# roahmlab/armour

Hardware: AMD Instinct MI355X
Metric: planning iters/s (eval_g+jac) Kinova 7-DOF, 100 timesteps × 20 obstacles (higher is better)
Workload: dtype f64

## Files before the change

armour_amd/_lib.py:

```python
import ctypes as C
import os

_HERE = os.path.dirname(os.path.abspath(__file__))
KEY128 = os.environ.get("ARMOUR_KEY128", "0") not in ("", "0")
LIB_PATH = os.environ.get("ARMOUR_HIP_LIB") or os.path.join(_HERE, "lib", "libarmour_hip_k128.so" if KEY128 else "libarmour_hip.so")

MAXJ = 9
MAXF = 8 if KEY128 else 7

OK, EINVAL, EDEVICE, ECAPACITY, ESTATE = 0, -1, -2, -3, -4


class ArmourRobot(C.Structure):
    _fields_ = [
        ("num_joints", C.c_int32), ("num_factors", C.c_int32),
        ("axes", C.c_int32 * MAXJ), ("continuous", C.c_int32 * MAXF),
        ("trans", C.c_double * ((MAXJ + 1) * 3)), ("rots", C.c_double * (MAXJ * 3)),
        ("mass", C.c_double * MAXJ), ("mass_uncertainty", C.c_double),
        ("com", C.c_double * (MAXJ * 3)),
        ("inertia", C.c_double * (MAXJ * 9)), ("inertia_uncertainty", C.c_double),
        ("friction", C.c_double * MAXJ), ("damping", C.c_double * MAXJ), ("armature", C.c_double * MAXJ),
        ("state_limits_lb", C.c_double * MAXF), ("state_limits_ub", C.c_double * MAXF),
        ("speed_limits", C.c_double * MAXF), ("torque_limits", C.c_double * MAXF),
        ("gravity", C.c_double),
        ("link_zonotope_center", C.c_double * (MAXJ * 3)), ("link_zonotope_generators", C.c_double * (MAXJ * 3)),
        ("alpha", C.c_double), ("V_m", C.c_double), ("M_max", C.c_double), ("M_min", C.c_double), ("K", C.c_double),
        ("mass_uncertainty_link", C.c_double * MAXJ), ("inertia_uncertainty_link", C.c_double * MAXJ),
    ]


class ArmourParams(C.Structure):
    _fields_ = [
        ("num_time_steps", C.c_int32), ("input_constraints_off", C.c_int32),
        ("duration", C.c_double), ("k_range", C.c_double * MAXF),
        ("simplify_threshold", C.c_double), ("t_plan", C.c_double), ("cost_scale", C.c_double),
        ("collision_violation_threshold", C.c_double), ("torque_violation_threshold", C.c_double),
    ]


class ArmourLimits(C.Structure):
    _fields_ = [
        ("max_batch", C.c_int32), ("max_obstacles", C.c_int32), ("link_monomials", C.c_int32),
        ("torque_monomials", C.c_int32), ("work_monomials", C.c_int32), ("raw_terms", C.c_int32),
    ]


class ArmourSolveOptions(C.Structure):
    _fields_ = [("max_iterations", C.c_int32), ("max_line_search", C.c_int32), ("tolerance", C.c_double),
                ("max_wall_time_s", C.c_double), ("force_host_qp", C.c_double), ("reserved", C.c_double * 3)]


class ArmourSolveResult(C.Structure):
    _fields_ = [("k_opt", C.c_double * MAXF), ("cost", C.c_double), ("max_violation", C.c_double), ("feasible", C.c_int32),
                ("iterations", C.c_int32), ("evaluations", C.c_int32), ("status", C.c_int32), ("time_ms", C.c_double)]


class ArmourTrackOptions(C.Structure):
    _fields_ = [("controller", C.c_int32), ("record_every", C.c_int32), ("steps_per_launch", C.c_int32), ("reserved0", C.c_int32),
                ("Kr", C.c_double * MAXF), ("alpha", C.c_double), ("V_max", C.c_double), ("r_norm_threshold", C.c_double),
                ("model_uncertainty", C.c_double), ("dt", C.c_double), ("t0", C.c_double), ("t1", C.c_double), ("duration", C.c_double),
                ("reserved", C.c_double * 4)]


class ArmourTrackResult(C.Structure):
    _fields_ = [("status", C.c_int32), ("steps", C.c_int32), ("limit_flags", C.c_int32), ("reserved", C.c_int32),
                ("t_end", C.c_double), ("q", C.c_double * MAXF), ("qd", C.c_double * MAXF),
                ("max_pos_error", C.c_double), ("max_vel_error", C.c_double), ("max_V", C.c_double), ("max_robust_input", C.c_double),
                ("max_torque_ratio", C.c_double), ("first_violation_t", C.c_double)]


TRACK_CTL_ROBUST, TRACK_CTL_NOMINAL, TRACK_CTL_NONE = 0, 1, 2
TRACK_LIMIT_TORQUE, TRACK_LIMIT_POSITION, TRACK_LIMIT_SPEED = 1, 2, 4


class ArmourViolation(C.Structure):
    _fields_ = [("l1_violation", C.c_double), ("worst", C.c_double), ("worst_row", C.c_int32), ("n_violated", C.c_int32),
                ("n_outside_slack", C.c_int32), ("feasible", C.c_int32)]


OPT_P1_BUILD = 1
OPT_P1_WORK_MEMORY_MB = 2
OPT_P1_KEEP_WORK_MEMORY = 3
OPT_P1_STEP_WAVES = 101
OPT_P1_STEP_FREE = 102
OPT_P1_STEP_SPLIT_FK = 103
OPT_P1_STEP_AUX3 = 104
OPT_P1_MAX_WAVES_PER_CU = 105
OPT_P1_TWO_PASS = 106
OPT_P1_STEP_PAIRS = 107
OPT_P1_STEP_QUEUE = 109
OPT_P1_STEP_TAIL_CROSS = 108
OPT_P1_STEP_TWO_CU = 123
OPT_P1_STEP_LEAN_BACK = 124
OPT_P1_TV_TAIL_CROSS = 121
OPT_P1_TV_MIN_GROUPS = 110
OPT_P1_TV_WAVES = 111
OPT_P1_TV_FREE = 112
OPT_P1_TV_SPLIT_FK = 113
OPT_P1_TV_DEDICATED = 114
OPT_P1_TV_HELP_SHIFT = 115
OPT_P1_TV_HELPERS = 116
OPT_P1_TV_HELP_MIN = 117
OPT_P1_TV_HELP_N = 118
OPT_P1_TV_AUX3 = 119
OPT_P1_FULL_PLANES = 120
OPT_P1_TV_ROW_WIDTH = 122
OPT_P2_EX = 130
OPT_STEPS_GRAPH_MIN = 131
OPT_PINNED_MODE = 132
OPT_CULL_ROWS = 133
OPT_SOLVE_SUB_TILES = 140
OPT_SOLVE_DEVICE = 141
OPT_SOLVE_CUT_TILES = 142
OPT_SOLVE_BLOCKS = 143
OPT_SOLVE_SUB_BATCH = 144
OPT_SOLVE_ROW_CAP = 145
OPT_SOLVE_HARD_CAP_S = 146
OPT_SOLVE_WAVES_PER_SIMD = 147
OPT_SOLVE_CULL = 148

EXPORTS = [
    "armour_robot_kinova_gen3_no_gripper", "armour_robot_kinova_gen3_gripper", "armour_robot_fetch", "armour_robot_fetch8", "armour_params_default", "armour_create", "armour_destroy",
    "armour_last_error", "armour_device_available", "armour_alloc_pinned", "armour_free_pinned", "armour_set_problems", "armour_set_problems_armtd", "armour_get_sizes",
    "armour_get_bounds", "armour_eval_f", "armour_eval_grad_f", "armour_eval_g_jac",
    "armour_eval_g_jac_device", "armour_eval_g_jac_device_steps", "armour_prepare_steps", "armour_eval_g_jac_device_multi", "armour_desired_trajectory", "armour_robust_controller", "armour_check_feasible", "armour_get_torque_radius",
    "armour_get_link_generators", "armour_get_link_centers", "armour_get_pz", "armour_get_table_sizes",
    "armour_solve_options_default", "armour_solve", "armour_debug_qp", "armour_debug_qp_box", "armour_debug_pz_op",
    "armour_get_hyperplanes", "armour_get_build_ms", "armour_get_build_info", "armour_p2_kernel_name", "armour_debug_load_tables",
    "armour_get_plane_skip", "armour_get_prune_margin", "armour_batch_get_prune_margin", "armour_set_option", "armour_get_option", "armour_controller_set_kernel", "armour_device_memory", "armour_abi_max_factors", "armour_eval_violations_device", "armour_eval_violations", "armour_get_row_relevance", "armour_get_solver_rows",
    "armour_batch_partition", "armour_batch_create", "armour_batch_destroy", "armour_batch_set_option", "armour_batch_set_problems",
    "armour_batch_get_sizes", "armour_batch_get_bounds", "armour_batch_eval_g_jac", "armour_batch_eval_violations", "armour_batch_solve",
    "armour_batch_get_build_ms", "armour_batch_get_build_info",
    "armour_roadmap_create", "armour_roadmap_destroy", "armour_roadmap_get_sizes", "armour_roadmap_check", "armour_roadmap_plan",
    "armour_track_options_default", "armour_track", "armour_track_auto_steps",
    "armour_path_audit", "armour_path_audit_host", "armour_path_audit_items",
]

_lib = None


def _share_hip_runtime_with_torch():
    import importlib.util
    import sys
    if "torch" in sys.modules:
        return
    try:
        spec = importlib.util.find_spec("torch")
    except (ImportError, ValueError):
        spec = None
    if spec is None or not spec.origin:
        return
    cand = os.path.join(os.path.dirname(spec.origin), "lib", "libamdhip64.so")
    if os.path.exists(cand):
        try:
            C.CDLL(cand, mode=C.RTLD_GLOBAL)
        except OSError:
            pass


def load():
    global _lib
    if _lib is not None:
        return _lib
    if not os.path.exists(LIB_PATH):
        raise OSError(
            f"{LIB_PATH} not found: build it with `make -C armour_amd/csrc` (hipcc, gfx950) or "
            "`python -c 'import __graft_entry__ as g; g.build()'`. There is no CPU path.")
    _share_hip_runtime_with_torch()
    L = C.CDLL(LIB_PATH)
    if hasattr(L, "armour_abi_max_factors") and L.armour_abi_max_factors() != MAXF:
        raise RuntimeError(f"{LIB_PATH} is built for {L.armour_abi_max_factors()} factors, this process mirrors its structs for {MAXF} (ARMOUR_KEY128)")
    dp, ip = C.POINTER(C.c_double), C.POINTER(C.c_int32)
    vp = C.c_void_p
    L.armour_robot_kinova_gen3_no_gripper.argtypes = [C.POINTER(ArmourRobot)]
    L.armour_robot_kinova_gen3_no_gripper.restype = None
    L.armour_robot_kinova_gen3_gripper.argtypes = [C.POINTER(ArmourRobot)]
    L.armour_robot_fetch.argtypes = [C.POINTER(ArmourRobot)]
    L.armour_robot_fetch.restype = None
    L.armour_robot_fetch8.argtypes = [C.POINTER(ArmourRobot)]
    L.armour_robot_fetch8.restype = C.c_int
    L.armour_robot_kinova_gen3_gripper.restype = None
    L.armour_params_default.argtypes = [C.POINTER(ArmourParams), C.c_int32]
    L.armour_params_default.restype = None
    L.armour_create.argtypes = [C.POINTER(ArmourRobot), C.POINTER(ArmourParams), C.POINTER(ArmourLimits), C.c_int32, C.POINTER(vp)]
    L.armour_destroy.argtypes = [vp]
    L.armour_destroy.restype = None
    L.armour_last_error.restype = C.c_char_p
    L.armour_alloc_pinned.argtypes = [C.c_uint64, C.POINTER(vp)]
    L.armour_free_pinned.argtypes = [vp]
    L.armour_free_pinned.restype = None
    L.armour_set_problems.argtypes = [vp, C.c_int32, C.c_int32, dp, dp, dp, dp, dp]
    L.armour_set_problems_armtd.argtypes = [vp, C.c_int32, C.c_int32, dp, dp, dp, dp, dp, dp]
    L.armour_get_sizes.argtypes = [vp, ip, ip, ip]
    L.armour_get_bounds.argtypes = [vp, dp, dp, dp, dp]
    L.armour_eval_f.argtypes = [vp, dp, dp]
    L.armour_eval_grad_f.argtypes = [vp, dp, dp]
    L.armour_eval_g_jac.argtypes = [vp, dp, dp, dp]
    L.armour_eval_g_jac_device.argtypes = [vp, vp, vp, vp, vp]
    L.armour_eval_g_jac_device_steps.argtypes = [vp, vp, C.c_int32, vp, vp, vp]
    L.armour_prepare_steps.argtypes = [vp, vp, C.c_int32, vp, vp]
    L.armour_eval_g_jac_device_multi.argtypes = [vp, vp, C.c_int32, vp, vp, vp]
    L.armour_desired_trajectory.argtypes = [C.c_int32, dp, dp, dp, dp, C.c_double, dp, C.c_double, dp, dp, dp]
    L.armour_robust_controller.argtypes = [C.POINTER(ArmourRobot), C.c_double, dp, C.c_double, C.c_double, C.c_double, C.c_int32, dp, dp, dp, dp, dp, dp, dp, dp]
    L.armour_check_feasible.argtypes = [vp, dp, ip]
    L.armour_solve_options_default.argtypes = [C.POINTER(ArmourSolveOptions)]
    L.armour_solve_options_default.restype = None
    L.armour_solve.argtypes = [vp, C.POINTER(ArmourSolveOptions), C.POINTER(ArmourSolveResult)]
    L.armour_debug_qp.argtypes = [C.c_int32, dp, dp, C.c_int32, dp, dp, dp, dp, ip]
    L.armour_debug_qp_box.argtypes = [C.c_int32, dp, dp, C.c_int32, dp, dp, dp, dp, dp, C.c_int32, dp, ip, ip, dp]
    L.armour_debug_pz_op.argtypes = [vp, C.c_int32, C.c_int32, ip, ip, C.POINTER(C.POINTER(C.c_uint64)), C.POINTER(dp), dp, dp, dp, dp,
                                     C.c_int32, C.c_int32, C.POINTER(C.c_uint64), dp, dp]
    L.armour_get_torque_radius.argtypes = [vp, dp]
    L.armour_get_link_generators.argtypes = [vp, dp]
    L.armour_get_link_centers.argtypes = [vp, dp, dp]
    L.armour_get_pz.argtypes = [vp, C.c_int32, C.c_int32, C.c_int32, C.c_int32, dp, C.POINTER(C.c_uint64), dp, C.c_int32]
    L.armour_get_table_sizes.argtypes = [vp, C.POINTER(C.c_int64)]
    L.armour_get_hyperplanes.argtypes = [vp, dp, dp, dp]
    L.armour_get_build_ms.argtypes = [vp, dp]
    L.armour_get_build_info.argtypes = [vp, ip]
    L.armour_p2_kernel_name.restype = C.c_char_p
    L.armour_debug_load_tables.argtypes = [vp, C.c_int32, C.c_int32, dp, dp, dp, dp, ip, dp, C.POINTER(C.c_uint64), dp,
                                           C.c_int32, ip, dp, C.POINTER(C.c_uint64), dp, C.c_int32, dp, dp, dp, dp]
    L.armour_get_plane_skip.argtypes = [vp, C.POINTER(C.c_uint64)]
    L.armour_get_prune_margin.argtypes = [vp, dp]
    L.armour_batch_get_prune_margin.argtypes = [vp, dp]
    L.armour_set_option.argtypes = [vp, C.c_int32, C.c_double]
    L.armour_get_option.argtypes = [vp, C.c_int32, dp]
    L.armour_device_memory.argtypes = [C.c_int32, C.POINTER(C.c_uint64), C.POINTER(C.c_uint64)]
    L.armour_controller_set_kernel.argtypes = [C.c_int32]
    L.armour_eval_violations_device.argtypes = [vp, vp, vp, vp]
    L.armour_eval_violations.argtypes = [vp, dp, C.POINTER(ArmourViolation)]
    L.armour_get_row_relevance.argtypes = [vp, C.POINTER(C.c_uint8), C.POINTER(C.c_int32), C.POINTER(C.c_double)]
    L.armour_get_solver_rows.argtypes = [vp, C.POINTER(C.c_uint8), C.POINTER(C.c_int32), C.POINTER(C.c_int32), C.POINTER(C.c_double)]
    L.armour_batch_partition.argtypes = [C.c_int32, C.c_int32, ip]
    L.armour_batch_create.argtypes = [C.POINTER(ArmourRobot), C.POINTER(ArmourParams), C.POINTER(ArmourLimits), ip, C.c_int32, C.POINTER(vp)]
    L.armour_batch_destroy.argtypes = [vp]
    L.armour_batch_destroy.restype = None
    L.armour_batch_set_option.argtypes = [vp, C.c_int32, C.c_double]
    L.armour_batch_set_problems.argtypes = [vp, C.c_int32, C.c_int32, dp, dp, dp, dp, dp]
    L.armour_batch_get_sizes.argtypes = [vp, ip, ip, ip, ip]
    L.armour_batch_get_bounds.argtypes = [vp, dp, dp, dp, dp]
    L.armour_batch_eval_g_jac.argtypes = [vp, dp, dp, dp]
    L.armour_batch_eval_violations.argtypes = [vp, dp, C.POINTER(ArmourViolation)]
    L.armour_batch_solve.argtypes = [vp, C.POINTER(ArmourSolveOptions), C.POINTER(ArmourSolveResult)]
    L.armour_batch_get_build_ms.argtypes = [vp, dp, dp]
    L.armour_batch_get_build_info.argtypes = [vp, ip]
    u8p = C.POINTER(C.c_uint8)
    L.armour_roadmap_create.argtypes = [C.POINTER(ArmourRobot), C.c_int32, dp, C.c_int32, ip, u8p, C.c_double, C.c_int32, C.POINTER(vp)]
    L.armour_roadmap_destroy.argtypes = [vp]
    L.armour_roadmap_destroy.restype = None
    L.armour_roadmap_get_sizes.argtypes = [vp, ip, ip, C.POINTER(C.c_int64)]
    L.armour_roadmap_check.argtypes = [vp, C.c_int32, C.c_int32, dp, u8p, u8p, dp, dp]
    L.armour_roadmap_plan.argtypes = [vp, C.c_int32, dp, dp, C.c_int32, C.c_int32, dp, ip]
    L.armour_track_options_default.argtypes = [C.POINTER(ArmourRobot), C.POINTER(ArmourTrackOptions)]
    L.armour_track_options_default.restype = None
    L.armour_track.argtypes = [C.POINTER(ArmourRobot), C.POINTER(ArmourTrackOptions), C.c_int32, dp, dp, dp, dp, dp, dp, dp, dp,
                               C.POINTER(ArmourTrackResult), dp, dp]
    L.armour_track_auto_steps.argtypes = [C.c_int32]
    audit = [C.POINTER(ArmourRobot), C.c_int32, C.c_int32, dp, C.c_int32, ip, dp, dp, dp, dp, dp, C.c_double, dp, dp, dp, C.c_double, ip, dp, dp]
    L.armour_path_audit.argtypes = audit + [dp]
    L.armour_path_audit_host.argtypes = audit
    L.armour_path_audit_items.argtypes = [C.POINTER(ArmourRobot), C.c_int32, dp, dp, dp, dp, dp, C.c_double, dp, dp, C.c_double, C.POINTER(C.c_int64)]
    _lib = L
    return L


class ArmourError(RuntimeError):
    def __init__(self, code, msg):
        super().__init__(f"armour error {code}: {msg}")
        self.code = code


def check(rc):
    if rc < 0:
        raise ArmourError(rc, load().armour_last_error().decode())
    return rc
```

armour_amd/csrc/api.hip:

```cpp
#include <algorithm>
#include <cmath>
#include <cstdarg>
#include <chrono>
#include <cstring>
#include <mutex>
#include <new>

#include "../../include/armour_robot_fetch.h"
#include "../../include/armour_robot_kinova.h"
#include "bezier.h"
#include "cacc.h"
#include "common.h"
#include "solver_common.h"

static thread_local char g_err[512] = "";

void armour_set_error(const char* fmt, ...) {
    va_list ap;
    va_start(ap, fmt);
    vsnprintf(g_err, sizeof(g_err), fmt, ap);
    va_end(ap);
}

extern "C" const char* armour_last_error(void) { return g_err; }

extern "C" void armour_robot_kinova_gen3_no_gripper(ArmourRobot* robot) { armour_fill_kinova_gen3_no_gripper(robot); }
extern "C" void armour_robot_kinova_gen3_gripper(ArmourRobot* robot) { armour_fill_kinova_gen3_gripper(robot); }
extern "C" void armour_robot_fetch(ArmourRobot* robot) { armour_fill_fetch(robot); }
extern "C" int armour_robot_fetch8(ArmourRobot* robot) {
#if ARMOUR_MAX_FACTORS >= 8
    if (!robot) { armour_set_error("null argument"); return ARMOUR_EINVAL; }
    armour_fill_fetch8(robot);
    return ARMOUR_OK;
#else
    (void)robot;
    armour_set_error("armour_robot_fetch8: an 8-factor robot needs the 128-bit-key library (libarmour_hip_k128.so: armour_abi_max_factors() == 8)");
    return ARMOUR_EINVAL;
#endif
}
extern "C" void armour_params_default(ArmourParams* params, int32_t T) { armour_fill_default_params(params, T); }

extern "C" int armour_device_available(void) {
    int n = 0;
    if (hipGetDeviceCount(&n) != hipSuccess) return 0;
    return n > 0 ? 1 : 0;
}

namespace {
struct PinnedRange { const char* p; size_t bytes; };
std::mutex g_pinned_mu;
std::vector<PinnedRange> g_pinned;
bool in_pinned(const void* q, size_t bytes) {
    if (!q) return true;
    const char* c = static_cast<const char*>(q);
    std::lock_guard<std::mutex> lk(g_pinned_mu);
    for (const PinnedRange& r : g_pinned)
        if (c >= r.p && c + bytes <= r.p + r.bytes) return true;
    return false;
}
}

extern "C" int armour_alloc_pinned(uint64_t bytes, void** out) {
    if (!out) { armour_set_error("null argument"); return ARMOUR_EINVAL; }
    HIPCHK(hipHostMalloc(out, bytes ? bytes : 1, hipHostMallocDefault));
    std::lock_guard<std::mutex> lk(g_pinned_mu);
    g_pinned.push_back({static_cast<const char*>(*out), (size_t)(bytes ? bytes : 1)});
    return ARMOUR_OK;
}
extern "C" void armour_free_pinned(void* p) {
    if (!p) return;
    {
        std::lock_guard<std::mutex> lk(g_pinned_mu);
        for (size_t i = 0; i < g_pinned.size(); i++)
            if (g_pinned[i].p == p) { g_pinned.erase(g_pinned.begin() + i); break; }
    }
    (void)hipHostFree(p);
}

template <class Tp>
static int dev_alloc(Tp** p, size_t count) {
    if (*p) { (void)hipFree(*p); *p = nullptr; }
    if (count == 0) count = 1;
    HIPCHK(hipMalloc((void**)p, count * sizeof(Tp)));
    return ARMOUR_OK;
}
template <class Tp>
static void dev_free(Tp** p) {
    if (*p) { (void)hipFree(*p); *p = nullptr; }
}

static int ensure_capacity(ArmourPlanner* h, int B, int O) {
    if (B <= h->allocB && O <= h->allocO) return ARMOUR_OK;
    const int nb = B > h->allocB ? B : h->allocB, no = O > h->allocO ? O : h->allocO;
    h->allocB = 0; h->allocO = 0;
    const size_t nl = (size_t)nb * h->J * h->T, nt = (size_t)nb * h->n * h->T;
    int rc;
#define TRY(x) if ((rc = (x)) != ARMOUR_OK) return rc
    TRY(dev_alloc(&h->d_link_count, nl));
    TRY(dev_alloc(&h->d_link_center, nl * 3));
    TRY(dev_alloc(&h->d_link_indep, nl * 3));
    TRY(dev_alloc(&h->d_link_keys, nl * h->lim.link_monomials));
    TRY(dev_alloc(&h->d_link_coeff, nl * h->lim.link_monomials * 3));
    TRY(dev_alloc(&h->d_tq_count, nt));
    TRY(dev_alloc(&h->d_tq_center, nt));
    TRY(dev_alloc(&h->d_tq_indep, nt));
    TRY(dev_alloc(&h->d_tq_keys, nt * h->lim.torque_monomials));
    TRY(dev_alloc(&h->d_tq_coeff, nt * h->lim.torque_monomials));
    TRY(dev_alloc(&h->d_planes, (size_t)nb * armour_planes_per_problem(h->J * h->T * no)));
    TRY(dev_alloc(&h->d_planes_ll, (size_t)nb * armour_planes_ll_per_problem(h->J * h->T)));
    TRY(dev_alloc(&h->d_obs_center, (size_t)nb * 3 * (no > 0 ? no : 1)));
    TRY(dev_alloc(&h->d_plane_skip, (size_t)nb));
    TRY(dev_alloc(&h->d_bez, (size_t)nb * 3 * h->n));
    const size_t mmax = (size_t)h->n * h->T + (size_t)h->J * h->T * no + 4 * h->n;
    TRY(dev_alloc(&h->d_k, (size_t)nb * h->n));
    TRY(dev_alloc(&h->d_g, (size_t)nb * mmax + std::max((size_t)nb * mmax * h->n, (size_t)nb * h->T * h->J * 3)));
    h->d_jac = h->d_g + (size_t)nb * mmax;
    TRY(dev_alloc(&h->d_bounds, (size_t)2 * nb * mmax));
#undef TRY
    h->allocB = nb;
    h->allocO = no;
    return ARMOUR_OK;
}

P2Tables armour_make_tables(const ArmourPlanner* h) {
    P2Tables tb;
    memset(&tb, 0, sizeof(tb));
    tb.B = h->B; tb.T = h->T; tb.J = h->J; tb.n = h->n; tb.O = h->O; tb.Q = h->Q; tb.m = h->m;
    tb.capL = h->lim.link_monomials; tb.capT = h->lim.torque_monomials;
    tb.row0 = h->row0; tb.mode = h->mode;
    tb.link_count = h->d_link_count; tb.link_center = h->d_link_center; tb.link_indep = h->d_link_indep;
    tb.link_keys = h->d_link_keys; tb.link_coeff = h->d_link_coeff;
    tb.tq_count = h->d_tq_count; tb.tq_center = h->d_tq_center; tb.tq_indep = h->d_tq_indep;
    tb.tq_keys = h->d_tq_keys; tb.tq_coeff = h->d_tq_coeff;
    tb.planes = h->d_planes; tb.planes_ll = h->d_planes_ll; tb.ll_shared = h->ll_shared;
    tb.ex_allowed = h->tune(ARMOUR_OPT_P2_EX);
    tb.obs_center = (h->d_from_center && (h->B >= 8 || !h->planes_have_d)) ? h->d_obs_center : nullptr;
    tb.plane_skip = h->d_plane_skip; tb.bez = h->d_bez;
    for (int i = 0; i < ARMOUR_MAX_FACTORS; i++) tb.k_range[i] = h->params.k_range[i];
    tb.duration = h->params.duration;
    return tb;
}

namespace {
struct TuningSpec { int option; double def, lo, hi; };
const TuningSpec kTuning[] = {
    {ARMOUR_OPT_P1_STEP_WAVES, 0, 0, 4}, {ARMOUR_OPT_P1_STEP_FREE, 1, 0, 1}, {ARMOUR_OPT_P1_STEP_SPLIT_FK, -1, -1, 1}, {ARMOUR_OPT_P1_STEP_AUX3, 1, 0, 1},
    {ARMOUR_OPT_P1_MAX_WAVES_PER_CU, 4, 1, 8}, {ARMOUR_OPT_P1_TWO_PASS, 1, 0, 1}, {ARMOUR_OPT_P1_STEP_PAIRS, 1, 0, 2}, {ARMOUR_OPT_P1_STEP_QUEUE, 1, 0, 3}, {ARMOUR_OPT_P1_STEP_TAIL_CROSS, 0, 0, 514}, {ARMOUR_OPT_P1_STEP_TWO_CU, 3, 0, 33}, {ARMOUR_OPT_P1_STEP_LEAN_BACK, 1, 0, 3}, {ARMOUR_OPT_P1_TV_TAIL_CROSS, 111, 0, 514} ,
    {ARMOUR_OPT_P1_TV_MIN_GROUPS, 31, 1, 1e6}, {ARMOUR_OPT_P1_TV_WAVES, 0, 0, 8}, {ARMOUR_OPT_P1_TV_FREE, 1, 0, 1}, {ARMOUR_OPT_P1_TV_SPLIT_FK, -1, -1, 1},
    {ARMOUR_OPT_P1_TV_DEDICATED, 1, 0, 1}, {ARMOUR_OPT_P1_TV_HELP_SHIFT, 0, 0, 3}, {ARMOUR_OPT_P1_TV_HELPERS, 1, 0, 31}, {ARMOUR_OPT_P1_TV_HELP_MIN, 192, 1, 1e6},
    {ARMOUR_OPT_P1_TV_HELP_N, 1, 0, 1}, {ARMOUR_OPT_P1_TV_AUX3, 1, 0, 1}, {ARMOUR_OPT_P1_TV_ROW_WIDTH, 0, 0, 64}, {ARMOUR_OPT_P1_FULL_PLANES, 0, 0, 1},
    {ARMOUR_OPT_P2_EX, 1, 0, 1}, {ARMOUR_OPT_STEPS_GRAPH_MIN, 2, 0, 1e6}, {ARMOUR_OPT_PINNED_MODE, 0, 0, 2}, {ARMOUR_OPT_CULL_ROWS, 0, 0, 1},
    {ARMOUR_OPT_SOLVE_SUB_TILES, 48, 1, 1e6}, {ARMOUR_OPT_SOLVE_DEVICE, 1, 0, 2}, {ARMOUR_OPT_SOLVE_CUT_TILES, 156, 1, 1e6}, {ARMOUR_OPT_SOLVE_BLOCKS, 0, 0, 1e6},
    {ARMOUR_OPT_SOLVE_SUB_BATCH, 0, 0, 1e6}, {ARMOUR_OPT_SOLVE_ROW_CAP, 0, 0, 1e7}, {ARMOUR_OPT_SOLVE_HARD_CAP_S, 0, 0, 1e6}, {ARMOUR_OPT_SOLVE_WAVES_PER_SIMD, 0, 0, 2}, {ARMOUR_OPT_SOLVE_CULL, -1, -1, 1},
};
const TuningSpec* tuning_spec(int option) {
    for (const TuningSpec& t : kTuning) if (t.option == option) return &t;
    return nullptr;
}
}
void armour_tuning_defaults(double* tuning) {
    for (int o = ARMOUR_OPT_FIRST_TUNING; o <= ARMOUR_OPT_LAST_TUNING; o++) tuning[o - ARMOUR_OPT_FIRST_TUNING] = 0.0;
    for (const TuningSpec& t : kTuning) tuning[t.option - ARMOUR_OPT_FIRST_TUNING] = t.def;
}
bool armour_trace_p1() { static const bool on = getenv("ARMOUR_P1_TRACE") != nullptr; return on; }
BuildStamps& armour_build_stamps() { static thread_local BuildStamps s; return s; }
void armour_build_stamp(const char* name) {
    if (!armour_trace_p1()) return;
    BuildStamps& s = armour_build_stamps();
    if (s.n < 12) { s.t[s.n] = std::chrono::duration<double, std::micro>(std::chrono::steady_clock::now().time_since_epoch()).count(); s.name[s.n] = name; s.n++; }
}
static void armour_build_stamps_print(const char* what) {
    if (!armour_trace_p1()) return;
    BuildStamps& s = armour_build_stamps();
    fprintf(stderr, "[%s, host side, us]", what);
    for (int i = 1; i < s.n; i++) fprintf(stderr, " %s %.1f", s.name[i], s.t[i] - s.t[i - 1]);
    if (s.n > 1) fprintf(stderr, " | total %.1f\n", s.t[s.n - 1] - s.t[0]);
}
bool armour_trace_solve() { static const bool on = getenv("ARMOUR_SOLVE_TIMING") != nullptr; return on; }

extern "C" int armour_create(const ArmourRobot* robot, const ArmourParams* params, const ArmourLimits* limits,
                             int32_t device, ArmourPlanner** out) {
    if (!robot || !params || !out) { armour_set_error("armour_create: null argument"); return ARMOUR_EINVAL; }
    if (robot->num_joints < 1 || robot->num_joints > ARMOUR_MAX_JOINTS || robot->num_factors < 1 ||
        robot->num_factors > robot->num_joints || robot->num_factors > ARMOUR_MAX_FACTORS) {
        armour_set_error("armour_create: unsupported robot (joints=%d, factors=%d; max %d joints, %d factors -- the monomial key "
                         "packs 9 bits per factor into 64, RT/PZsparse.h:8-21)", robot->num_joints, robot->num_factors,
                         ARMOUR_MAX_JOINTS, ARMOUR_MAX_FACTORS);
        return ARMOUR_EINVAL;
    }
    for (int i = 0; i < robot->num_joints; i++)
        if ((i < robot->num_factors) != (robot->axes[i] != 0)) {
            armour_set_error("armour_create: the actuated joints must come first and the fixed ones last (RT/Dynamics.cu:103-105)");
            return ARMOUR_EINVAL;
        }
    if (params->num_time_steps < 2 || (params->num_time_steps & 1)) {
        armour_set_error("armour_create: num_time_steps must be even and >= 2 (RT/Parameters.h:16)");
        return ARMOUR_EINVAL;
    }
    int ndev = 0;
    if (hipGetDeviceCount(&ndev) != hipSuccess || ndev <= 0) {
        armour_set_error("armour_create: no HIP device visible -- libarmour_hip has no CPU path");
        return ARMOUR_EDEVICE;
    }
    if (device < 0 || device >= ndev) { armour_set_error("armour_create: device %d out of range (%d visible)", device, ndev); return ARMOUR_EINVAL; }
    HIPCHK(hipSetDevice(device));
    ArmourPlanner* h = new (std::nothrow) ArmourPlanner();
    if (!h) { armour_set_error("out of host memory"); return ARMOUR_EINVAL; }
    h->robot = *robot;
    h->params = *params;
    armour_tuning_defaults(h->tuning);
    ArmourLimits lim;
    memset(&lim, 0, sizeof(lim));
    if (limits) lim = *limits;
    if (lim.max_batch <= 0) lim.max_batch = 1;
    if (lim.max_obstacles <= 0) lim.max_obstacles = 40;
    if (lim.link_monomials <= 0) lim.link_monomials = 32;
    if (lim.torque_monomials <= 0) lim.torque_monomials = 128;
    if (lim.work_monomials <= 0) lim.work_monomials = 1024;
    if (lim.raw_terms <= 0) lim.raw_terms = 4096;
    h->lim = lim;
    h->ub = armour_ultimate_bound(robot);
    h->device = device;
    h->T = params->num_time_steps; h->J = robot->num_joints; h->n = robot->num_factors;
    hipError_t e = hipStreamCreateWithFlags(&h->stream, hipStreamNonBlocking);
    if (e != hipSuccess) { armour_set_error("hipStreamCreate failed: %s", hipGetErrorString(e)); delete h; return ARMOUR_EDEVICE; }
    *out = h;
    return ARMOUR_OK;
}

double* armour_handle_pinned(ArmourPlanner* h, int slot, size_t bytes) {
    if (h->solve_pin[slot] && h->solve_pin_bytes[slot] >= bytes) return static_cast<double*>(h->solve_pin[slot]);
    if (h->solve_pin[slot]) { armour_free_pinned(h->solve_pin[slot]); h->solve_pin[slot] = nullptr; h->solve_pin_bytes[slot] = 0; }
    void* p = nullptr;
    if (armour_alloc_pinned(bytes, &p) != ARMOUR_OK) return nullptr;
    h->solve_pin[slot] = p; h->solve_pin_bytes[slot] = bytes;
    return static_cast<double*>(p);
}

static void drop_step_graphs(ArmourPlanner* h) {
    for (auto& g : h->step_graphs) (void)hipGraphExecDestroy(g.exec);
    h->step_graphs.clear();
}

extern "C" void armour_destroy(ArmourPlanner* h) {
    if (!h) return;
    (void)hipSetDevice(h->device);
    if (h->stream) (void)hipStreamSynchronize(h->stream);
    drop_step_graphs(h);
    for (void* pin : h->solve_pin) armour_free_pinned(pin);
    dev_free(&h->d_bounds); dev_free(&h->d_viol);
    armour_relevance_free(h);
    if (h->d_tr_stage) (void)hipFree(h->d_tr_stage);
    dev_free(&h->solve_dev.ctl); dev_free(&h->solve_dev.blk_word); dev_free(&h->solve_dev.blk_rows); dev_free(&h->solve_dev.qp_rows);
    dev_free(&h->solve_dev.flags);
    dev_free(&h->d_jrs);
    armour_p1_free(h);
    dev_free(&h->d_link_count); dev_free(&h->d_link_center); dev_free(&h->d_link_indep);
    dev_free(&h->d_link_keys); dev_free(&h->d_link_coeff);
    dev_free(&h->d_tq_count); dev_free(&h->d_tq_center); dev_free(&h->d_tq_indep);
    dev_free(&h->d_tq_keys); dev_free(&h->d_tq_coeff);
    dev_free(&h->d_planes); dev_free(&h->d_planes_ll); dev_free(&h->d_obs_center); dev_free(&h->d_plane_skip); dev_free(&h->d_bez);
    dev_free(&h->d_k); dev_free(&h->d_g); h->d_jac = nullptr;
    if (h->stream) (void)hipStreamDestroy(h->stream);
    delete h;
}

static int begin_problem_set(ArmourPlanner* h, int B, int O, const double* q0, const double* qd0, const double* qdd0,
                             const double* q_des, int mode = ARMOUR_MODE_ARMOUR) {
    if (!h || !q0 || !qd0 || !qdd0 || !q_des) { armour_set_error("null argument"); return ARMOUR_EINVAL; }
    if (B < 1 || O < 0) { armour_set_error("bad batch/obstacle count (B=%d, O=%d)", B, O); return ARMOUR_EINVAL; }
    {
        const double* arrs[4] = {q0, qd0, qdd0, q_des};
        for (int a = 0; a < 4; a++)
            for (size_t i = 0; i < (size_t)B * h->n; i++)
                if (!std::isfinite(arrs[a][i])) { armour_set_error("non-finite entry in the initial state / goal arrays (array %d, entry %zu)", a, i); return ARMOUR_EINVAL; }
    }
    HIPCHK(hipSetDevice(h->device));
    h->ready = false;
    h->rel_fresh = false; h->rel2_fresh = false;
    h->bounds_on_device = false; h->bounds_on_host = false;
    h->tables_from_host = false;
    h->stats_fresh = false;
    drop_step_graphs(h);
    int rc = ensure_capacity(h, B, O);
    if (rc != ARMOUR_OK) return rc;
    h->B = B; h->O = O; h->Q = h->J * h->T * O;
    h->mode = mode;
    h->row0 = h->no_torque() ? 0 : h->n * h->T;
    h->m = h->row0 + h->Q + 4 * h->n;
    h->d_jac = h->d_g + (size_t)B * h->m;
    const size_t bn = (size_t)B * h->n;
    h->h_q0.assign(q0, q0 + bn); h->h_qd0.assign(qd0, qd0 + bn);
    h->h_qdes.assign(q_des, q_des + bn);
    if (mode == ARMOUR_MODE_ARMTD) { h->h_qdd0.assign(bn, 0.0); h->h_krange.assign(qdd0, qdd0 + bn); }
    else { h->h_qdd0.assign(qdd0, qdd0 + bn); h->h_krange.clear(); }
    std::vector<double> bz((size_t)B * 3 * h->n);
    const double D = mode == ARMOUR_MODE_ARMTD ? 1.0 : h->params.duration;
    for (int b = 0; b < B; b++)
        for (int i = 0; i < h->n; i++) {
            bz[((size_t)b * 3 + 0) * h->n + i] = q0[b * h->n + i];
            bz[((size_t)b * 3 + 1) * h->n + i] = qd0[b * h->n + i] * D;
            bz[((size_t)b * 3 + 2) * h->n + i] = qdd0[b * h->n + i] * D * D;
        }
    HIPCHK(hipMemcpy(h->d_bez, bz.data(), bz.size() * sizeof(double), hipMemcpyHostToDevice));
    return ARMOUR_OK;
}

int armour_refresh_table_stats(ArmourPlanner* h) {
    if (h->stats_fresh) { h->stats_fresh = false; return ARMOUR_OK; }
    const size_t nl = (size_t)h->B * h->J * h->T, nt = (size_t)h->B * h->n * h->T;
    std::vector<int> lc(nl), tc(nt);
    HIPCHK(hipMemcpy(lc.data(), h->d_link_count, nl * sizeof(int), hipMemcpyDeviceToHost));
    HIPCHK(hipMemcpy(tc.data(), h->d_tq_count, nt * sizeof(int), hipMemcpyDeviceToHost));
    long long sl = 0, st = 0;
    int ml = 0, mt = 0;
    for (int v : lc) { sl += v; if (v > ml) ml = v; }
    for (int v : tc) { st += v; if (v > mt) mt = v; }
    h->sum_link = sl; h->sum_torque = st; h->max_link = ml; h->max_torque = mt;
    h->h_plane_skip.assign((size_t)h->B, 0ull);
    if (h->O > 0) HIPCHK(hipMemcpy(h->h_plane_skip.data(), h->d_plane_skip, (size_t)h->B * sizeof(unsigned long long), hipMemcpyDeviceToHost));
    if (h->O > 0 && armour_trace_p1()) {
        unsigned long long all_and = ~0ull, all_or = 0ull;
        for (unsigned long long v : h->h_plane_skip) { all_and &= v; all_or |= v; }
        fprintf(stderr, "[P1 planes] plane_skip of %d problem(s): AND 0x%09llx OR 0x%09llx\n", h->B, all_and & ((1ull << ARMOUR_NPLANES) - 1ull), all_or & ((1ull << ARMOUR_NPLANES) - 1ull));
    }
    return ARMOUR_OK;
}

extern "C" int armour_set_problems(ArmourPlanner* h, int32_t B, int32_t O, const double* q0, const double* qd0,
                                   const double* qdd0, const double* q_des, const double* obstacles) {
    armour_build_stamps().n = 0;
    armour_build_stamp("start");
    int rc = begin_problem_set(h, B, O, q0, qd0, qdd0, q_des);
    if (rc != ARMOUR_OK) return rc;
    if (O > 0 && !obstacles) { armour_set_error("obstacles is null but O=%d", O); return ARMOUR_EINVAL; }
    for (size_t i = 0; i < (size_t)B * O * 12; i++)
        if (!std::isfinite(obstacles[i])) { armour_set_error("non-finite obstacle entry %zu", i); return ARMOUR_EINVAL; }
    armour_build_stamp("checks+bezier-upload");
    rc = armour_p1_build(h, obstacles);
    if (rc != ARMOUR_OK) return rc;
    armour_build_stamp("copy-out");
    rc = armour_refresh_table_stats(h);
    if (rc != ARMOUR_OK) return rc;
    h->ready = true;
    armour_build_stamp("table-stats");
    armour_build_stamps_print("armour_set_problems");
    return ARMOUR_OK;
}

extern "C" int armour_set_problems_armtd(ArmourPlanner* h, int32_t B, int32_t O, const double* q0, const double* qd0, const double* q_des,
                                         const double* jrs, const double* k_range, const double* obstacles) {
    if (!jrs || !k_range) { armour_set_error("null argument"); return ARMOUR_EINVAL; }
    int rc = begin_problem_set(h, B, O, q0, qd0, k_range, q_des, ARMOUR_MODE_ARMTD);
    if (rc != ARMOUR_OK) return rc;
    if (O > 0 && !obstacles) { armour_set_error("obstacles is null but O=%d", O); return ARMOUR_EINVAL; }
    for (size_t i = 0; i < (size_t)B * O * 12; i++)
        if (!std::isfinite(obstacles[i])) { armour_set_error("non-finite obstacle entry %zu", i); return ARMOUR_EINVAL; }
    for (size_t i = 0; i < (size_t)B * h->n * 6 * h->T; i++)
        if (!std::isfinite(jrs[i])) { armour_set_error("non-finite entry %zu in the offline JRS tables", i); return ARMOUR_EINVAL; }
    const size_t cnt = (size_t)B * h->n * 6 * h->T;
    if (cnt > h->jrs_cap) {
        if ((rc = dev_alloc(&h->d_jrs, cnt)) != ARMOUR_OK) return rc;
        h->jrs_cap = cnt;
    }
    HIPCHK(hipMemcpy(h->d_jrs, jrs, cnt * sizeof(double), hipMemcpyHostToDevice));
    rc = armour_p1_build(h, obstacles);
    if (rc != ARMOUR_OK) return rc;
    rc = armour_refresh_table_stats(h);
    if (rc != ARMOUR_OK) return rc;
    h->ready = true;
    return ARMOUR_OK;
}

extern "C" int armour_debug_load_tables(ArmourPlanner* h, int32_t B, int32_t O, const double* q0, const double* qd0,
                                        const double* qdd0, const double* q_des, const int32_t* link_count,
                                        const double* link_center, const uint64_t* link_keys, const double* link_coeffs,
                                        int32_t cap_l, const int32_t* torque_count, const double* torque_center,
                                        const uint64_t* torque_keys, const double* torque_coeffs, int32_t cap_t,
                                        const double* A, const double* d, const double* delta, const double* torque_radius) {
    int rc = begin_problem_set(h, B, O, q0, qd0, qdd0, q_des);
    if (rc != ARMOUR_OK) return rc;
    h->build_ms = 0; h->build_info[0] = h->build_info[1] = h->build_info[2] = h->build_info[3] = 0;
    h->h_prune_margin.clear();
    const int J = h->J, T = h->T, n = h->n, capL = h->lim.link_monomials, capT = h->lim.torque_monomials;
    const size_t nl = (size_t)B * J * T, nt = (size_t)B * n * T;
    std::vector<double> lc(nl * 3), li(nl * 3), lco(nl * capL * 3, 0.0), tc(nt), ti(nt), tco(nt * capT, 0.0);
    std::vector<uint32_t> lk(nl * capL, 0), tk(nt * capT, 0);
    for (size_t i = 0; i < nl; i++) {
        if (link_count[i] > capL) { armour_set_error("link PZ %zu has %d monomials > capacity %d", i, link_count[i], capL); return ARMOUR_ECAPACITY; }
        for (int e = 0; e < 3; e++) { lc[i * 3 + e] = link_center[(i * 2) * 3 + e]; li[i * 3 + e] = link_center[(i * 2 + 1) * 3 + e]; }
        for (int mo = 0; mo < link_count[i]; mo++) {
            lk[i * capL + mo] = (uint32_t)link_keys[i * cap_l + mo];
            for (int e = 0; e < 3; e++) lco[(i * capL + mo) * 3 + e] = link_coeffs[(i * cap_l + mo) * 3 + e];
        }
    }
    for (size_t i = 0; i < nt; i++) {
        if (torque_count[i] > capT) { armour_set_error("torque PZ %zu has %d monomials > capacity %d", i, torque_count[i], capT); return ARMOUR_ECAPACITY; }
        tc[i] = torque_center[i * 2]; ti[i] = torque_center[i * 2 + 1];
        for (int mo = 0; mo < torque_count[i]; mo++) { tk[i * capT + mo] = (uint32_t)torque_keys[i * cap_t + mo]; tco[i * capT + mo] = torque_coeffs[i * cap_t + mo]; }
    }
    const size_t ppp = armour_planes_per_problem(h->Q);
    std::vector<double> pl((size_t)B * ppp, 0.0);
    for (int b = 0; b < B; b++)
        for (int t = 0; t < T; t++)
            for (int l = 0; l < J; l++)
                for (int o = 0; o < O; o++)
                    for (int p = 0; p < 36; p++) {
                        const size_t src = ((((size_t)b * T + t) * J + l) * O + o) * 36 + p;
                        const int q = (l * T + t) * O + o;
                        double* base = &pl[(size_t)b * ppp];
                        base[armour_plane_index(h->Q, q, p, 0)] = A[src * 3 + 0]; base[armour_plane_index(h->Q, q, p, 1)] = A[src * 3 + 1];
                        base[armour_plane_index(h->Q, q, p, 2)] = A[src * 3 + 2];
                        base[armour_plane_index(h->Q, q, p, 3)] = d[src]; base[armour_plane_index(h->Q, q, p, 4)] = delta[src];
                    }
#define UP(dst, vec) HIPCHK(hipMemcpy(dst, vec.data(), vec.size() * sizeof(vec[0]), hipMemcpyHostToDevice))
    HIPCHK(hipMemcpy(h->d_link_count, link_count, nl * sizeof(int), hipMemcpyHostToDevice));
    HIPCHK(hipMemcpy(h->d_tq_count, torque_count, nt * sizeof(int), hipMemcpyHostToDevice));
    UP(h->d_link_center, lc); UP(h->d_link_indep, li); UP(h->d_link_keys, lk); UP(h->d_link_coeff, lco);
    UP(h->d_tq_center, tc); UP(h->d_tq_indep, ti); UP(h->d_tq_keys, tk); UP(h->d_tq_coeff, tco);
    if (!pl.empty()) UP(h->d_planes, pl);
    {
        const int JT = J * T;
        std::vector<double> pll((size_t)B * armour_planes_ll_per_problem(JT), 0.0);
        bool shared = O > 0;
        for (int b = 0; b < B && O > 0; b++)
            for (int t = 0; t < T; t++)
                for (int l = 0; l < J; l++)
                    for (int p = ARMOUR_FIRST_LL_PLANE; p < 36; p++)
                        for (int o = 0; o < O; o++) {
                            const size_t src = ((((size_t)b * T + t) * J + l) * O + o) * 36 + p, src0 = ((((size_t)b * T + t) * J + l) * O) * 36 + p;
                            for (int cc = 0; cc < 3; cc++) {
                                if (o == 0) pll[(size_t)b * armour_planes_ll_per_problem(JT) + armour_plane_ll_index(JT, l * T + t, p - ARMOUR_FIRST_LL_PLANE, cc)] = A[src * 3 + cc];
                                else if (memcmp(&A[src * 3 + cc], &A[src0 * 3 + cc], sizeof(double)) != 0) shared = false;
                            }
                        }
        UP(h->d_planes_ll, pll);
        h->ll_shared = shared ? 1 : 0;
        h->d_from_center = 0;
        h->planes_lean = 0; h->planes_have_d = 1;
    }
    HIPCHK(hipMemset(h->d_plane_skip, 0, (size_t)B * sizeof(unsigned long long)));
#undef UP
    h->h_torque_radius.assign(torque_radius, torque_radius + (size_t)B * n * T);
    h->h_link_gens.assign((size_t)B * T * J * 18, 0.0);
    rc = armour_refresh_table_stats(h);
    if (rc != ARMOUR_OK) return rc;
    h->tables_from_host = true;
    h->ready = true;
    return ARMOUR_OK;
}

#define NEED_READY(h)                                                                        \
    if (!(h)) { armour_set_error("null handle"); return ARMOUR_EINVAL; }                     \
    if (!(h)->ready) { armour_set_error("no problem set: call armour_set_problems first"); return ARMOUR_ESTATE; }

extern "C" int armour_get_sizes(const ArmourPlanner* h, int32_t* B, int32_t* n, int32_t* m) {
    NEED_READY(h);
    if (B) *B = h->B;
    if (n) *n = h->n;
    if (m) *m = h->m;
    return ARMOUR_OK;
}

extern "C" int armour_get_bounds(ArmourPlanner* h, double* x_l, double* x_u, double* g_l, double* g_u) {
    NEED_READY(h);
    const int T = h->T, n = h->n;
    if (x_l) for (int i = 0; i < n; i++) x_l[i] = -1.0;
    if (x_u) for (int i = 0; i < n; i++) x_u[i] = 1.0;
    if (!g_l || !g_u) return ARMOUR_OK;
    for (int b = 0; b < h->B; b++) {
        double* gl = g_l + (size_t)b * h->m;
        double* gu = g_u + (size_t)b * h->m;
        if (!h->no_torque()) {
            const double* tr = &h->h_torque_radius[(size_t)b * n * T];
            for (int t = 0; t < T; t++)
                for (int j = 0; j < n; j++) {
                    gl[t * n + j] = -h->robot.torque_limits[j] + tr[j * T + t];
                    gu[t * n + j] = h->robot.torque_limits[j] - tr[j * T + t];
                }
        }
        size_t off = (size_t)h->row0;
        for (size_t i = off; i < off + (size_t)h->Q; i++) { gl[i] = -1e19; gu[i] = 0; }
        off += h->Q;
        for (int rep = 0; rep < 2; rep++, off += n)
            for (int i = 0; i < n; i++) { gl[off + i] = h->robot.state_limits_lb[i] + h->ub.qe; gu[off + i] = h->robot.state_limits_ub[i] - h->ub.qe; }
        for (int rep = 0; rep < 2; rep++, off += n)
            for (int i = 0; i < n; i++) { gl[off + i] = -h->robot.speed_limits[i] + h->ub.qde; gu[off + i] = h->robot.speed_limits[i] - h->ub.qde; }
    }
    return ARMOUR_OK;
}

int armour_checked_collision_rows(const ArmourPlanner* h) {
    return h->mode == ARMOUR_MODE_ARMTD ? (h->n - 1 < h->J ? h->n - 1 : h->J) * h->T * h->O : h->Q;
}

static void plan_coeffs(const ArmourPlanner* h, size_t ix, double c[3]) {
    const double D = h->params.duration;
    const bool armtd = h->mode == ARMOUR_MODE_ARMTD;
    c[0] = h->h_q0[ix];
    c[1] = armtd ? h->h_qd0[ix] : h->h_qd0[ix] * D;
    c[2] = armtd ? h->h_krange[ix] : h->h_qdd0[ix] * D * D;
}

extern "C" int armour_eval_f(ArmourPlanner* h, const double* k, double* f) {
    NEED_READY(h);
    const int n = h->n;
    for (int b = 0; b < h->B; b++) {
        double obj = 0;
        for (int pass = 0; pass < 2; pass++)
            for (int i = 0; i < n; i++) {
                if ((h->robot.continuous[i] != 0) != (pass == 0)) continue;
                const size_t ix = (size_t)b * n + i;
                double c[3];
                plan_coeffs(h, ix, c);
                const double qp = slv::plan_point(h->mode, c[0], c[1], c[2], h->params.k_range[i], k[ix], h->params.t_plan);
                const double e = h->robot.continuous[i] ? slv::wrap_to_pi(h->h_qdes[ix] - qp) : (h->h_qdes[ix] - qp);
                obj += e * e;
            }
        f[b] = obj * h->params.cost_scale;
    }
    return ARMOUR_OK;
}

extern "C" int armour_eval_grad_f(ArmourPlanner* h, const double* k, double* grad_f) {
    NEED_READY(h);
    const int n = h->n;
    const double tp = h->params.t_plan;
    for (int b = 0; b < h->B; b++)
        for (int i = 0; i < n; i++) {
            const size_t ix = (size_t)b * n + i;
            double c[3];
            plan_coeffs(h, ix, c);
            const double qp = slv::plan_point(h->mode, c[0], c[1], c[2], h->params.k_range[i], k[ix], tp);
            const double dk = slv::plan_dk(h->mode, c[2], h->params.k_range[i], tp);
            const double e = h->robot.continuous[i] ? slv::wrap_to_pi(qp - h->h_qdes[ix]) : (qp - h->h_qdes[ix]);
            grad_f[ix] = 2 * e * dk * h->params.cost_scale;
        }
    return ARMOUR_OK;
}

extern "C" int armour_desired_trajectory(int32_t n, const double* q0, const double* qd0, const double* qdd0, const double* k_range,
                                         double duration, const double* k, double t, double* q, double* qd, double* qdd) {
    if (n < 1 || !q0 || !qd0 || !qdd0 || !k_range || !k || !(duration > 0)) { armour_set_error("bad argument"); return ARMOUR_EINVAL; }
    const double D = duration, s = t / D;
    for (int i = 0; i < n; i++) {
        const double a = qd0[i] * D, b = qdd0[i] * D * D, ka = k_range[i] * k[i];
        if (q) q[i] = bez::q_des(q0[i], a, b, ka, s);
        if (qd) qd[i] = bez::qd_des(q0[i], a, b, ka, s) / D;
        if (qdd) qdd[i] = bez::qdd_des(q0[i], a, b, ka, s) / (D * D);
    }
    return ARMOUR_OK;
}

extern "C" int armour_eval_g_jac_device(ArmourPlanner* h, const double* d_k, double* d_g, double* d_jac, void* stream) {
    NEED_READY(h);
    if (!d_k) { armour_set_error("d_k is null"); return ARMOUR_EINVAL; }
    const P2Tables tb = armour_make_tables(h);
    return armour_p2_launch(tb, h->max_link, h->max_torque, h->h_plane_skip.data(), d_k, d_g, d_jac, stream ? (hipStream_t)stream : h->stream);
}

static int enqueue_steps(ArmourPlanner* h, const double* d_k, int steps, double* d_g, double* d_jac, hipStream_t st) {
    const P2Tables tb = armour_make_tables(h);
    const size_t stride = (size_t)h->B * h->n;
    for (int s = 0; s < steps; s++) {
        int rc = armour_p2_launch(tb, h->max_link, h->max_torque, h->h_plane_skip.data(), d_k + (size_t)s * stride, d_g, d_jac, st);
        if (rc != ARMOUR_OK) return rc;
    }
    return ARMOUR_OK;
}

static int steps_graph(ArmourPlanner* h, const double* d_k, int steps, double* d_g, double* d_jac, hipGraphExec_t* out) {
    h->graph_clock++;
    for (auto& g : h->step_graphs)
        if (g.d_k == d_k && g.steps == steps && g.d_g == d_g && g.d_jac == d_jac) { g.last_use = h->graph_clock; *out = g.exec; return ARMOUR_OK; }
    HIPCHK(hipSetDevice(h->device));
    HIPCHK(hipStreamSynchronize(h->stream));
    hipGraph_t graph = nullptr;
    HIPCHK(hipStreamBeginCapture(h->stream, hipStreamCaptureModeThreadLocal));
    const int rc = enqueue_steps(h, d_k, steps, d_g, d_jac, h->stream);
    const hipError_t e = hipStreamEndCapture(h->stream, &graph);
    if (rc != ARMOUR_OK) { if (graph) (void)hipGraphDestroy(graph); return rc; }
    if (e != hipSuccess) { armour_set_error("hipStreamEndCapture failed: %s", hipGetErrorString(e)); return ARMOUR_EDEVICE; }
    hipGraphExec_t exec = nullptr;
    const hipError_t ei = hipGraphInstantiate(&exec, graph, nullptr, nullptr, 0);
    (void)hipGraphDestroy(graph);
    if (ei != hipSuccess) { armour_set_error("hipGraphInstantiate failed: %s", hipGetErrorString(ei)); return ARMOUR_EDEVICE; }
    if (h->step_graphs.size() >= 4) {
        size_t lru = 0;
        for (size_t i = 1; i < h->step_graphs.size(); i++) if (h->step_graphs[i].last_use < h->step_graphs[lru].last_use) lru = i;
        (void)hipGraphExecDestroy(h->step_graphs[lru].exec);
        h->step_graphs.erase(h->step_graphs.begin() + lru);
    }
    h->step_graphs.push_back({d_k, steps, d_g, d_jac, exec, h->graph_clock});
    *out = exec;
    return ARMOUR_OK;
}

static bool steps_use_graph(const ArmourPlanner* h, int steps) {
    const int min_steps = h->tune(ARMOUR_OPT_STEPS_GRAPH_MIN);
    return min_steps > 0 && steps >= min_steps;
}

extern "C" int armour_prepare_steps(ArmourPlanner* h, const double* d_k, int32_t steps, double* d_g, double* d_jac) {
    NEED_READY(h);
    if (!d_k || steps < 0) { armour_set_error("bad argument"); return ARMOUR_EINVAL; }
    if (!steps_use_graph(h, steps)) return ARMOUR_OK;
    hipGraphExec_t exec;
    return steps_graph(h, d_k, steps, d_g, d_jac, &exec);
}

extern "C" int armour_eval_g_jac_device_steps(ArmourPlanner* h, const double* d_k, int32_t steps, double* d_g, double* d_jac,
                                              void* stream) {
    NEED_READY(h);
    if (!d_k || steps < 0) { armour_set_error("bad argument"); return ARMOUR_EINVAL; }
    if (steps == 0 || (!d_g && !d_jac)) return ARMOUR_OK;
    const hipStream_t st = stream ? (hipStream_t)stream : h->stream;
    if (steps_use_graph(h, steps))
        for (auto& g : h->step_graphs)
            if (g.d_k == d_k && g.steps == steps && g.d_g == d_g && g.d_jac == d_jac) {
                g.last_use = ++h->graph_clock;
                HIPCHK(hipGraphLaunch(g.exec, st));
                return ARMOUR_OK;
            }
    return enqueue_steps(h, d_k, steps, d_g, d_jac, st);
}

extern "C" int armour_eval_g_jac_device_multi(ArmourPlanner* h, const double* d_k, int32_t points, double* d_g, double* d_jac,
                                              void* stream) {
    NEED_READY(h);
    if (!d_k || points < 0) { armour_set_error("bad argument"); return ARMOUR_EINVAL; }
    if (points == 0) return ARMOUR_OK;
    const P2Tables tb = armour_make_tables(h);
    const long long bn = (long long)h->B * h->n, bm = (long long)h->B * h->m;
    return armour_p2_launch(tb, h->max_link, h->max_torque, h->h_plane_skip.data(), d_k, d_g, d_jac, stream ? (hipStream_t)stream : h->stream,
                            points, bn, bm, bm * h->n);
}

int armour_spin_on_stream(hipStream_t st) {
    for (;;) {
        const hipError_t q = hipStreamQuery(st);
        if (q == hipSuccess) return ARMOUR_OK;
        if (q != hipErrorNotReady) { armour_set_error("hipStreamQuery failed: %s", hipGetErrorString(q)); return ARMOUR_EDEVICE; }
    }
}

extern "C" int armour_eval_g_jac(ArmourPlanner* h, const double* k, double* g, double* jac) {
    NEED_READY(h);
    if (!k) { armour_set_error("k is null"); return ARMOUR_EINVAL; }
    HIPCHK(hipSetDevice(h->device));
    const size_t bn = (size_t)h->B * h->n, bm = (size_t)h->B * h->m;
    const P2Tables tb = armour_make_tables(h);
    const int pinned_mode = h->tune(ARMOUR_OPT_PINNED_MODE);
    const bool all_pinned = in_pinned(k, bn * sizeof(double)) && in_pinned(g, bm * sizeof(double)) && in_pinned(jac, bm * h->n * sizeof(double));
    if (all_pinned && pinned_mode == 1) {
        int rc = armour_p2_launch(tb, h->max_link, h->max_torque, h->h_plane_skip.data(), k, g, jac, h->stream);
        if (rc != ARMOUR_OK) return rc;
        return armour_spin_on_stream(h->stream);
    }
    const double* k_dev = h->d_k;
    if (all_pinned && pinned_mode == 2) k_dev = k;
    else HIPCHK(hipMemcpyAsync(h->d_k, k, bn * sizeof(double), hipMemcpyHostToDevice, h->stream));
    int rc = armour_p2_launch(tb, h->max_link, h->max_torque, h->h_plane_skip.data(), k_dev, g ? h->d_g : nullptr, jac ? h->d_jac : nullptr, h->stream);
    if (rc != ARMOUR_OK) return rc;
    if (g && jac && jac == g + bm) {
        HIPCHK(hipMemcpyAsync(g, h->d_g, bm * (1 + (size_t)h->n) * sizeof(double), hipMemcpyDeviceToHost, h->stream));
        return armour_spin_on_stream(h->stream);
    }
    if (g) HIPCHK(hipMemcpyAsync(g, h->d_g, bm * sizeof(double), hipMemcpyDeviceToHost, h->stream));
    if (jac) HIPCHK(hipMemcpyAsync(jac, h->d_jac, bm * h->n * sizeof(double), hipMemcpyDeviceToHost, h->stream));
    return armour_spin_on_stream(h->stream);
}

extern "C" int armour_check_feasible(ArmourPlanner* h, const double* g, int32_t* feasible) {
    NEED_READY(h);
    const int T = h->T, n = h->n;
    const double tt = h->params.torque_violation_threshold, ct = h->params.collision_violation_threshold;
    for (int b = 0; b < h->B; b++) {
        const double* gb = g + (size_t)b * h->m;
        bool ok = true;
        if (!h->no_torque()) {
            const double* tr = &h->h_torque_radius[(size_t)b * n * T];
            for (int t = 0; t < T && ok; t++)
                for (int j = 0; j < n; j++) {
                    const double v = gb[t * n + j];
                    if (v < -h->robot.torque_limits[j] + tr[j * T + t] - tt || v > h->robot.torque_limits[j] - tr[j * T + t] + tt) { ok = false; break; }
                }
        }
        size_t off = (size_t)h->row0;
        const size_t n_checked = (size_t)armour_checked_collision_rows(h);
        for (size_t i = 0; i < n_checked && ok; i++)
            if (gb[off + i] > ct) ok = false;
        off += h->Q;
        for (int rep = 0; rep < 2 && ok; rep++, off += n)
            for (int i = 0; i < n; i++)
                if (gb[off + i] < h->robot.state_limits_lb[i] + h->ub.qe || gb[off + i] > h->robot.state_limits_ub[i] - h->ub.qe) { ok = false; break; }
        for (int rep = 0; rep < 2 && ok; rep++, off += n)
            for (int i = 0; i < n; i++)
                if (gb[off + i] < -h->robot.speed_limits[i] + h->ub.qde || gb[off + i] > h->robot.speed_limits[i] - h->ub.qde) { ok = false; break; }
        feasible[b] = ok ? 1 : 0;
    }
    return ARMOUR_OK;
}

namespace {
struct BoundsArgs {
    int n, T, m, row0, Q, no_torque;
    double torque_limits[ARMOUR_MAX_FACTORS], lb[ARMOUR_MAX_FACTORS], ub[ARMOUR_MAX_FACTORS], speed[ARMOUR_MAX_FACTORS];
    double qe, qde;
    const double* tr;
    double* lo; double* hi;
};
__global__ __launch_bounds__(256) void armour_bounds_kernel(BoundsArgs a) {
    const int b = blockIdx.y, r = blockIdx.x * 256 + threadIdx.x;
    if (r >= a.m) return;
    double l, u;
    if (r < a.row0) {
        const int t = r / a.n, j = r - t * a.n;
        const double tr = a.tr[((size_t)b * a.n + j) * a.T + t];
        l = -a.torque_limits[j] + tr; u = a.torque_limits[j] - tr;
    } else if (r < a.row0 + a.Q) { l = -1e19; u = 0; }
    else {
        const int e = r - a.row0 - a.Q, rep = e / a.n, i = e - rep * a.n;
        if (rep < 2) { l = a.lb[i] + a.qe; u = a.ub[i] - a.qe; }
        else { l = -a.speed[i] + a.qde; u = a.speed[i] - a.qde; }
    }
    a.lo[(size_t)b * a.m + r] = l;
    a.hi[(size_t)b * a.m + r] = u;
}
}

int armour_bounds_launch(ArmourPlanner* h, const double* d_tr) {
    const size_t bm = (size_t)h->B * h->m;
    BoundsArgs a;
    a.n = h->n; a.T = h->T; a.m = h->m; a.row0 = h->row0; a.Q = h->Q; a.no_torque = h->no_torque() ? 1 : 0;
    for (int j = 0; j < ARMOUR_MAX_FACTORS; j++) {
        a.torque_limits[j] = h->robot.torque_limits[j]; a.lb[j] = h->robot.state_limits_lb[j]; a.ub[j] = h->robot.state_limits_ub[j]; a.speed[j] = h->robot.speed_limits[j];
    }
    a.qe = h->ub.qe; a.qde = h->ub.qde;
    a.lo = h->d_bounds; a.hi = h->d_bounds + bm;
    a.tr = d_tr;
    hipLaunchKernelGGL(armour_bounds_kernel, dim3((h->m + 255) / 256, h->B), dim3(256), 0, h->stream, a);
    HIPCHK(hipGetLastError());
    h->bounds_on_device = true;
    return ARMOUR_OK;
}

int armour_upload_bounds(ArmourPlanner* h) {
    if (h->bounds_on_device) return ARMOUR_OK;
    const double* d_tr = nullptr;
    if (!h->no_torque()) {
        const size_t ntr = (size_t)h->B * h->n * h->T;
        if (h->tr_stage_cap < ntr) {
            if (h->d_tr_stage) (void)hipFree(h->d_tr_stage);
            h->d_tr_stage = nullptr; h->tr_stage_cap = 0;
            HIPCHK(hipMalloc((void**)&h->d_tr_stage, ntr * sizeof(double)));
            h->tr_stage_cap = ntr;
        }
        HIPCHK(hipMemcpyAsync(h->d_tr_stage, h->h_torque_radius.data(), ntr * sizeof(double), hipMemcpyHostToDevice, h->stream));
        d_tr = h->d_tr_stage;
    }
    const int rc = armour_bounds_launch(h, d_tr);
    if (rc != ARMOUR_OK) return rc;
    HIPCHK(hipStreamSynchronize(h->stream));
    return ARMOUR_OK;
}

extern "C" int armour_set_option(ArmourPlanner* h, int32_t option, double value) {
    if (!h) { armour_set_error("null handle"); return ARMOUR_EINVAL; }
    if (option == ARMOUR_OPT_P1_BUILD && (value == 0.0 || value == 1.0 || value == 2.0)) { h->opt_p1_build = (int)value; return ARMOUR_OK; }
    if (option == ARMOUR_OPT_P1_WORK_MEMORY_MB && value >= 0.0 && value <= 1e9) { h->opt_p1_work_mb = value; return ARMOUR_OK; }
    if (option == ARMOUR_OPT_P1_KEEP_WORK_MEMORY && (value == 0.0 || value == 1.0)) { h->opt_p1_keep_work = (int)value; return ARMOUR_OK; }
    if (const TuningSpec* t = tuning_spec(option)) {
        bool ok = value >= t->lo && value <= t->hi && (option == ARMOUR_OPT_SOLVE_HARD_CAP_S || value == (double)(long long)value);
        if (ok && (option == ARMOUR_OPT_P1_STEP_TAIL_CROSS || option == ARMOUR_OPT_P1_TV_TAIL_CROSS)) {
            const int v = (int)value, lo2 = v % 100, hi2 = v / 100;
            ok = (lo2 <= 4 || (lo2 >= 10 && lo2 <= 14)) && hi2 <= 5;
        }
        if (ok && option == ARMOUR_OPT_P1_TV_ROW_WIDTH) ok = value == 0.0 || value == 50.0 || value == 64.0;
        if (ok && option == ARMOUR_OPT_P1_STEP_TWO_CU) { const int lv = (int)value % 10; ok = lv <= 3 && (value < 10.0 || lv >= 1); if (ok) h->p1_two_cu_off = false; }
        if (ok) {
            h->tuning[option - ARMOUR_OPT_FIRST_TUNING] = value;
            h->p1_step_cap_hint = 0; h->p1_tv_shape_hint = 0;
            return ARMOUR_OK;
        }
    }
    armour_set_error("armour_set_option: unknown option %d or bad value %g", option, value);
    return ARMOUR_EINVAL;
}

extern "C" int armour_abi_max_factors(void) { return ARMOUR_MAX_FACTORS; }

extern "C" int armour_device_memory(int32_t device, uint64_t* free_bytes, uint64_t* total_bytes) {
    int ndev = 0;
    if (hipGetDeviceCount(&ndev) != hipSuccess || device < 0 || device >= ndev) { (void)hipGetLastError(); armour_set_error("armour_device_memory: no such device %d", device); return ARMOUR_EDEVICE; }
    HIPCHK(hipSetDevice(device));
    size_t f = 0, t = 0;
    HIPCHK(hipMemGetInfo(&f, &t));
    if (free_bytes) *free_bytes = f;
    if (total_bytes) *total_bytes = t;
    return ARMOUR_OK;
}

extern "C" int armour_get_option(ArmourPlanner* h, int32_t option, double* value) {
    if (!h || !value) { armour_set_error("null argument"); return ARMOUR_EINVAL; }
    if (option == ARMOUR_OPT_P1_BUILD) { *value = h->opt_p1_build; return ARMOUR_OK; }
    if (option == ARMOUR_OPT_P1_WORK_MEMORY_MB) { *value = h->opt_p1_work_mb; return ARMOUR_OK; }
    if (option == ARMOUR_OPT_P1_KEEP_WORK_MEMORY) { *value = h->opt_p1_keep_work; return ARMOUR_OK; }
    if (tuning_spec(option)) { *value = h->tuning[option - ARMOUR_OPT_FIRST_TUNING]; return ARMOUR_OK; }
    armour_set_error("armour_get_option: unknown option %d", option);
    return ARMOUR_EINVAL;
}

namespace {
struct ViolArgs {
    int m, row0, Q, n_checked;
    double torque_slack, collision_slack;
    const double* g; const double* lo; const double* hi;
    ArmourViolation* out;
};
__global__ __launch_bounds__(256) void armour_violation_kernel(ViolArgs a) {
    __shared__ double s_l1[256], s_w[256];
    __shared__ int s_row[256], s_nv[256], s_no[256];
    const int b = blockIdx.x, tid = threadIdx.x;
    const double* g = a.g + (size_t)b * a.m;
    const double* lo = a.lo + (size_t)b * a.m;
    const double* hi = a.hi + (size_t)b * a.m;
    double l1 = 0.0, worst = 0.0;
    int wrow = -1, nv = 0, no = 0;
    for (int r = tid; r < a.m; r += 256) {
        const double v = g[r], l = lo[r], u = hi[r];
        const double viol = fmax(0.0, fmax(l - v, v - u));
        l1 += viol;
        if (viol > 0.0) nv++;
        if (viol > worst) { worst = viol; wrow = r; }
        bool outside;
        if (r < a.row0) outside = v < l - a.torque_slack || v > u + a.torque_slack;
        else if (r < a.row0 + a.Q) outside = (r - a.row0) < a.n_checked && v > a.collision_slack;
        else outside = v < l || v > u;
        if (outside) no++;
    }
    s_l1[tid] = l1; s_w[tid] = worst; s_row[tid] = wrow; s_nv[tid] = nv; s_no[tid] = no;
    __syncthreads();
    for (int s = 128; s > 0; s >>= 1) {
        if (tid < s) {
            s_l1[tid] += s_l1[tid + s]; s_nv[tid] += s_nv[tid + s]; s_no[tid] += s_no[tid + s];
            const double ow = s_w[tid + s];
            const int orow = s_row[tid + s];
            if (ow > s_w[tid] || (ow == s_w[tid] && orow >= 0 && (s_row[tid] < 0 || orow < s_row[tid]))) { s_w[tid] = ow; s_row[tid] = orow; }
        }
        __syncthreads();
    }
    if (tid == 0) {
        ArmourViolation o;
        o.l1_violation = s_l1[0]; o.worst = s_w[0]; o.worst_row = s_row[0]; o.n_violated = s_nv[0]; o.n_outside_slack = s_no[0];
        o.feasible = s_no[0] == 0 ? 1 : 0;
        a.out[b] = o;
    }
}
}

static int eval_violations_device_impl(ArmourPlanner* h, const double* d_k, ArmourViolation* d_out, void* stream, bool allow_cull) {
    NEED_READY(h);
    if (!d_k || !d_out) { armour_set_error("null argument"); return ARMOUR_EINVAL; }
    HIPCHK(hipSetDevice(h->device));
    int rc = armour_upload_bounds(h);
    if (rc != ARMOUR_OK) return rc;
    const hipStream_t st = stream ? (hipStream_t)stream : h->stream;
    if (allow_cull && h->tune(ARMOUR_OPT_CULL_ROWS)) return armour_eval_violations_culled(h, d_k, d_out, st);
    const P2Tables tb = armour_make_tables(h);
    rc = armour_p2_launch(tb, h->max_link, h->max_torque, h->h_plane_skip.data(), d_k, h->d_g, nullptr, st);
    if (rc != ARMOUR_OK) return rc;
    ViolArgs a;
    a.m = h->m; a.row0 = h->row0; a.Q = h->Q; a.n_checked = armour_checked_collision_rows(h);
    a.torque_slack = h->params.torque_violation_threshold; a.collision_slack = h->params.collision_violation_threshold;
    a.g = h->d_g; a.lo = h->d_bounds; a.hi = h->d_bounds + (size_t)h->B * h->m; a.out = d_out;
    hipLaunchKernelGGL(armour_violation_kernel, dim3(h->B), dim3(256), 0, st, a);
    HIPCHK(hipGetLastError());
    return ARMOUR_OK;
}

extern "C" int armour_eval_violations_device(ArmourPlanner* h, const double* d_k, ArmourViolation* d_out, void* stream) {
    return eval_violations_device_impl(h, d_k, d_out, stream, true);
}

extern "C" int armour_eval_violations(ArmourPlanner* h, const double* k, ArmourViolation* out) {
    NEED_READY(h);
    if (!k || !out) { armour_set_error("null argument"); return ARMOUR_EINVAL; }
    HIPCHK(hipSetDevice(h->device));
    const size_t bn = (size_t)h->B * h->n;
    if ((size_t)h->B > h->viol_cap) {
        dev_free(&h->d_viol); h->viol_cap = 0;
        int rc = dev_alloc(&h->d_viol, (size_t)h->B);
        if (rc != ARMOUR_OK) return rc;
        h->viol_cap = (size_t)h->B;
    }
    double* hk = armour_handle_pinned(h, 6, bn * sizeof(double));
    ArmourViolation* hv = reinterpret_cast<ArmourViolation*>(armour_handle_pinned(h, 7, (size_t)h->B * sizeof(ArmourViolation)));
    if (!hk || !hv) return ARMOUR_EDEVICE;
    memcpy(hk, k, bn * sizeof(double));
    HIPCHK(hipMemcpyAsync(h->d_k, hk, bn * sizeof(double), hipMemcpyHostToDevice, h->stream));
    bool in_box = true;
    for (size_t i = 0; i < bn && in_box; i++) in_box = fabs(k[i]) <= 1.0;
    int rc = eval_violations_device_impl(h, h->d_k, h->d_viol, h->stream, in_box);
    if (rc != ARMOUR_OK) return rc;
    HIPCHK(hipMemcpyAsync(hv, h->d_viol, (size_t)h->B * sizeof(ArmourViolation), hipMemcpyDeviceToHost, h->stream));
    rc = armour_spin_on_stream(h->stream);
    if (rc != ARMOUR_OK) return rc;
    memcpy(out, hv, (size_t)h->B * sizeof(ArmourViolation));
    return ARMOUR_OK;
}

extern "C" int armour_get_torque_radius(ArmourPlanner* h, double* out) {
    NEED_READY(h);
    memcpy(out, h->h_torque_radius.data(), h->h_torque_radius.size() * sizeof(double));
    return ARMOUR_OK;
}

extern "C" int armour_get_link_generators(ArmourPlanner* h, double* out) {
    NEED_READY(h);
    memcpy(out, h->h_link_gens.data(), h->h_link_gens.size() * sizeof(double));
    return ARMOUR_OK;
}

extern "C" int armour_get_link_centers(ArmourPlanner* h, const double* k, double* centers) {
    NEED_READY(h);
    HIPCHK(hipSetDevice(h->device));
    const size_t bn = (size_t)h->B * h->n, cnt = (size_t)h->B * h->T * h->J * 3;
    HIPCHK(hipMemcpyAsync(h->d_k, k, bn * sizeof(double), hipMemcpyHostToDevice, h->stream));
    const P2Tables tb = armour_make_tables(h);
    int rc = armour_p2_slice_links_launch(tb, h->d_k, h->d_jac, h->stream);
    if (rc != ARMOUR_OK) return rc;
    HIPCHK(hipMemcpyAsync(centers, h->d_jac, cnt * sizeof(double), hipMemcpyDeviceToHost, h->stream));
    HIPCHK(hipStreamSynchronize(h->stream));
    return ARMOUR_OK;
}

extern "C" int armour_get_pz(ArmourPlanner* h, int32_t b, int32_t which, int32_t i, int32_t t, double* center,
                             uint64_t* keys, double* coeffs, int32_t capacity) {
    NEED_READY(h);
    if (b < 0 || b >= h->B || t < 0 || t >= h->T || which < 0 || which > 1 || i < 0 || i >= (which == 0 ? h->J : h->n)) {
        armour_set_error("armour_get_pz: index out of range");
        return ARMOUR_EINVAL;
    }
    if (which == 1 && h->no_torque()) {
        if (center) center[0] = center[1] = 0.0;
        return 0;
    }
    HIPCHK(hipSetDevice(h->device));
    HIPCHK(hipStreamSynchronize(h->stream));
    const int sz = which == 0 ? 3 : 1;
    const int cap = which == 0 ? h->lim.link_monomials : h->lim.torque_monomials;
    const size_t idx = which == 0 ? ((size_t)b * h->J + i) * h->T + t : ((size_t)b * h->n + i) * h->T + t;
    int cnt = 0;
    HIPCHK(hipMemcpy(&cnt, (which == 0 ? h->d_link_count : h->d_tq_count) + idx, sizeof(int), hipMemcpyDeviceToHost));
    if (center) {
        HIPCHK(hipMemcpy(center, (which == 0 ? h->d_link_center : h->d_tq_center) + idx * sz, sz * sizeof(double), hipMemcpyDeviceToHost));
        HIPCHK(hipMemcpy(center + sz, (which == 0 ? h->d_link_indep : h->d_tq_indep) + idx * sz, sz * sizeof(double), hipMemcpyDeviceToHost));
    }
    if (keys && coeffs) {
        if (capacity < cnt) { armour_set_error("armour_get_pz: capacity %d < count %d", capacity, cnt); return ARMOUR_EINVAL; }
        std::vector<uint32_t> k32(cnt > 0 ? cnt : 1);
        if (cnt > 0) {
            HIPCHK(hipMemcpy(k32.data(), (which == 0 ? h->d_link_keys : h->d_tq_keys) + idx * cap, cnt * sizeof(uint32_t), hipMemcpyDeviceToHost));
            HIPCHK(hipMemcpy(coeffs, (which == 0 ? h->d_link_coeff : h->d_tq_coeff) + idx * cap * sz, (size_t)cnt * sz * sizeof(double), hipMemcpyDeviceToHost));
        }
        for (int mo = 0; mo < cnt; mo++) keys[mo] = k32[mo];
    }
    return cnt;
}

extern "C" int armour_get_table_sizes(ArmourPlanner* h, int64_t* out4) {
    NEED_READY(h);
    out4[0] = h->sum_link; out4[1] = h->sum_torque; out4[2] = h->max_link; out4[3] = h->max_torque;
    return ARMOUR_OK;
}

extern "C" int armour_get_hyperplanes(ArmourPlanner* h, double* A, double* d, double* delta) {
    NEED_READY(h);
    HIPCHK(hipSetDevice(h->device));
    HIPCHK(hipStreamSynchronize(h->stream));
    const int B = h->B, T = h->T, J = h->J, O = h->O;
    const size_t ppp = armour_planes_per_problem(h->Q);
    std::vector<double> pl(h->Q > 0 ? (size_t)B * ppp : 0);
    if (pl.empty()) return ARMOUR_OK;
    if (h->planes_lean) {
        double* d_full = nullptr;
        HIPCHK(hipMalloc((void**)&d_full, pl.size() * sizeof(double)));
        int rc = armour_p1_full_planes(h, d_full);
        if (rc == ARMOUR_OK && hipMemcpy(pl.data(), d_full, pl.size() * sizeof(double), hipMemcpyDeviceToHost) != hipSuccess) { armour_set_error("copy of the half-space table failed"); rc = ARMOUR_EDEVICE; }
        (void)hipFree(d_full);
        if (rc != ARMOUR_OK) return rc;
    } else
    HIPCHK(hipMemcpy(pl.data(), h->d_planes, pl.size() * sizeof(double), hipMemcpyDeviceToHost));
    for (int b = 0; b < B; b++)
        for (int t = 0; t < T; t++)
            for (int l = 0; l < J; l++)
                for (int o = 0; o < O; o++)
                    for (int p = 0; p < 36; p++) {
                        const size_t dst = ((((size_t)b * T + t) * J + l) * O + o) * 36 + p;
                        const int q = (l * T + t) * O + o;
                        const double* base = &pl[(size_t)b * ppp];
                        if (A) { A[dst * 3 + 0] = base[armour_plane_index(h->Q, q, p, 0)]; A[dst * 3 + 1] = base[armour_plane_index(h->Q, q, p, 1)]; A[dst * 3 + 2] = base[armour_plane_index(h->Q, q, p, 2)]; }
                        if (d) d[dst] = base[armour_plane_index(h->Q, q, p, 3)];
                        if (delta) delta[dst] = base[armour_plane_index(h->Q, q, p, 4)];
                    }
    return ARMOUR_OK;
}

extern "C" int armour_debug_pz_op(ArmourPlanner* h, int32_t op, int32_t nops, const int32_t* sz, const int32_t* cnt, const uint64_t* const* keys,
                                  const double* const* coef, const double* cen, const double* ind, const double* ind2, const double* consts,
                                  int32_t r, int32_t out_cap, uint64_t* out_keys, double* out_coef, double* out_misc) {
    if (!h || nops < 1 || nops > 3 || op < 0 || op > 11) { armour_set_error("armour_debug_pz_op: bad argument"); return ARMOUR_EINVAL; }
    for (int o = 0; o < nops; o++)
        if ((sz[o] != 1 && sz[o] != 3 && sz[o] != 9) || cnt[o] < 0 || cnt[o] > h->lim.work_monomials || (sz[o] == 9 && o == 1 && cnt[o] > 8)) {
            armour_set_error("armour_debug_pz_op: bad operand"); return ARMOUR_EINVAL;
        }
    return armour_p1_debug_pz_op(h, op, nops, sz, cnt, keys, coef, cen, ind, ind2, consts, r, out_cap, out_keys, out_coef, out_misc);
}

extern "C" int armour_get_plane_skip(ArmourPlanner* h, uint64_t* plane_skip) {
    NEED_READY(h);
    if (!plane_skip) { armour_set_error("null argument"); return ARMOUR_EINVAL; }
    for (int b = 0; b < h->B; b++) plane_skip[b] = (uint64_t)h->h_plane_skip[b] & ((1ull << ARMOUR_NPLANES) - 1ull);
    return ARMOUR_OK;
}

extern "C" int armour_get_prune_margin(ArmourPlanner* h, double* margin) {
    NEED_READY(h);
    if (!margin) { armour_set_error("null argument"); return ARMOUR_EINVAL; }
    if ((int)h->h_prune_margin.size() != h->B) { armour_set_error("no reach-set build on this handle (tables loaded by armour_debug_load_tables carry no prune margin)"); return ARMOUR_ESTATE; }
    for (int b = 0; b < h->B; b++) margin[b] = h->h_prune_margin[(size_t)b];
    return ARMOUR_OK;
}

extern "C" int armour_get_build_ms(ArmourPlanner* h, double* ms) {
    NEED_READY(h);
    *ms = h->build_ms;
    return ARMOUR_OK;
}

extern "C" int armour_get_build_info(ArmourPlanner* h, int32_t* out4) {
    NEED_READY(h);
    if (!out4) { armour_set_error("null argument"); return ARMOUR_EINVAL; }
    for (int i = 0; i < 4; i++) out4[i] = h->build_info[i];
    return ARMOUR_OK;
}
```

armour_amd/csrc/common.h:

```cpp
#pragma once

#include <hip/hip_runtime.h>

#include <cstdint>
#include <cstdio>
#include <string>
#include <vector>

#include "../../include/armour_hip.h"

#define ARMOUR_NPLANES 36
#define ARMOUR_PLANE_COMPONENTS 5

void armour_set_error(const char* fmt, ...);

#define ARMOUR_FIRST_LL_PLANE 21
#define ARMOUR_N_LL_PLANES 15
__host__ __device__ inline int armour_row_stride(int Q) { return (Q + 15) & ~15; }
__host__ __device__ inline size_t armour_planes_ab_offset(int Q) { (void)Q; return 0; }
__host__ __device__ inline size_t armour_planes_cd_offset(int Q) { return (size_t)2 * ARMOUR_NPLANES * armour_row_stride(Q); }
__host__ __device__ inline size_t armour_planes_dll_offset(int Q) { return (size_t)4 * ARMOUR_NPLANES * armour_row_stride(Q); }
__host__ __device__ inline size_t armour_planes_d_offset(int Q) { return (size_t)(4 * ARMOUR_NPLANES + 16) * armour_row_stride(Q); }
__host__ __device__ inline size_t armour_planes_per_problem(int Q) { return (size_t)(5 * ARMOUR_NPLANES + 16) * armour_row_stride(Q); }
__host__ __device__ inline size_t armour_plane_index(int Q, int q, int p, int c) {
    const size_t Qs = (size_t)armour_row_stride(Q);
    if (c < 2) return ((size_t)p * Qs + q) * 2 + c;
    if (c == 2) return armour_planes_cd_offset(Q) + ((size_t)p * Qs + q) * 2;
    if (c == 3) return armour_planes_d_offset(Q) + (size_t)p * Qs + q;
    if (p < ARMOUR_FIRST_LL_PLANE) return armour_planes_cd_offset(Q) + ((size_t)p * Qs + q) * 2 + 1;
    return armour_planes_dll_offset(Q) + ((size_t)((p - ARMOUR_FIRST_LL_PLANE) >> 1) * Qs + q) * 2 + ((p - ARMOUR_FIRST_LL_PLANE) & 1);
}
#define ARMOUR_RECOMPUTE_D_ROWS 32768
#define ARMOUR_LL_RECORD 48
__host__ __device__ inline size_t armour_planes_ll_per_problem(int JT) { return (size_t)ARMOUR_LL_RECORD * (size_t)JT; }
__host__ __device__ inline size_t armour_plane_ll_index(int JT, int lt, int pll, int c) { (void)JT; return (size_t)lt * ARMOUR_LL_RECORD + (size_t)pll * 3 + c; }

#define HIPCHK(expr)                                                                                     \
    do {                                                                                                 \
        hipError_t e__ = (expr);                                                                         \
        if (e__ != hipSuccess) {                                                                         \
            armour_set_error("%s failed: %s (%s:%d)", #expr, hipGetErrorString(e__), __FILE__, __LINE__); \
            return ARMOUR_EDEVICE;                                                                       \
        }                                                                                                \
    } while (0)

template <class Tp>
inline int grow(Tp** p, size_t* cap, size_t need, bool* fresh = nullptr) {
    if (need <= *cap && *p) return ARMOUR_OK;
    if (*p) (void)hipFree(*p);
    *p = nullptr;
    HIPCHK(hipMalloc((void**)p, (need ? need : 1) * sizeof(Tp)));
    *cap = need;
    if (fresh) *fresh = true;
    return ARMOUR_OK;
}

int armour_spin_on_stream(hipStream_t st);

struct P2Tables {
    int B, T, J, n, O, Q, m;
    int capL, capT;
    int row0;
    const int* link_count;
    const double* link_center;
    const double* link_indep;
    const uint32_t* link_keys;
    const double* link_coeff;
    const int* tq_count;
    const double* tq_center;
    const double* tq_indep;
    const uint32_t* tq_keys;
    const double* tq_coeff;
    const double* planes;
    const double* obs_center;
    const double* planes_ll;
    int ll_shared;
    int ex_allowed;
    int mode;
    const unsigned long long* plane_skip;
    const double* bez;
    double k_range[ARMOUR_MAX_FACTORS];
    double duration;
};

#define ARMOUR_MODE_ARMOUR 0
#define ARMOUR_MODE_ARMTD 1

struct SolveDeviceWork {
    unsigned char* ctl = nullptr; size_t ctl_cap = 0;
    unsigned char* blk_word = nullptr; size_t word_cap = 0;
    int words_clean = 0;
    unsigned char* blk_rows = nullptr; size_t blk_rows_cap = 0;
    unsigned char* qp_rows = nullptr; size_t qp_rows_cap = 0;
    unsigned char* flags = nullptr; size_t flags_cap = 0;
};

struct ArmourPlanner {
    ArmourRobot robot;
    ArmourParams params;
    ArmourLimits lim;
    ArmourUltimateBound ub;
    int device = 0;
    hipStream_t stream = nullptr;
    int T = 0, J = 0, n = 0;
    int B = 0, O = 0, Q = 0, m = 0;
    bool ready = false;
    int mode = ARMOUR_MODE_ARMOUR;
    bool no_torque() const { return mode == ARMOUR_MODE_ARMTD || params.input_constraints_off != 0; }
    int row0 = 0;
    std::vector<double> h_krange;
    double* d_jrs = nullptr;
    size_t jrs_cap = 0;
    void* solve_pin[10] = {nullptr, nullptr, nullptr, nullptr, nullptr, nullptr, nullptr, nullptr, nullptr, nullptr};
    size_t solve_pin_bytes[10] = {0, 0, 0, 0, 0, 0, 0, 0, 0, 0};
    bool stats_fresh = false;
    int opt_p1_build = 0;
    double opt_p1_work_mb = 0;
    int opt_p1_keep_work = 1;
    double tuning[ARMOUR_OPT_LAST_TUNING - ARMOUR_OPT_FIRST_TUNING + 1];
    int tune(int option) const { return (int)tuning[option - ARMOUR_OPT_FIRST_TUNING]; }
    double tune_f(int option) const { return tuning[option - ARMOUR_OPT_FIRST_TUNING]; }
    ArmourViolation* d_viol = nullptr; size_t viol_cap = 0;
    unsigned char* d_rel = nullptr; size_t rel_cap = 0;
    int* d_rel_rows = nullptr; size_t rel_rows_cap = 0;
    int* d_rel_count = nullptr; size_t rel_count_cap = 0;
    double* d_rel_packed = nullptr; size_t rel_packed_cap = 0;
    long long* d_rel_pack_off = nullptr; size_t rel_pack_off_cap = 0;
    int* d_rel_rows_res = nullptr; size_t rel_rows_res_cap = 0;
    std::vector<int> h_rel_count;
    unsigned char* d_rel2 = nullptr; size_t rel2_cap = 0;
    int* d_rel2_rows = nullptr; size_t rel2_rows_cap = 0;
    int* d_rel2_count = nullptr; size_t rel2_count_cap = 0;
    double* d_rel2_packed = nullptr; size_t rel2_packed_cap = 0;
    long long* d_rel2_pack_off = nullptr; size_t rel2_pack_off_cap = 0;
    int* d_rel2_tq_tiles = nullptr; size_t rel2_tq_tiles_cap = 0;
    std::vector<int> h_rel2_count, h_rel2_tq_count;
    bool rel2_fresh = false;
    double rel2_ms = 0;
    int rel2_max_count = 0, rel2_tq_cap = 0;
    bool rel_fresh = false;
    double rel_ms = 0;
    int rel_max_count = 0;
    SolveDeviceWork solve_dev;
    double* d_bounds = nullptr;
    bool bounds_on_device = false, bounds_on_host = false;
    bool tables_from_host = false;
    std::vector<double> h_gl, h_gu;
    std::vector<double> h_q0, h_qd0, h_qdd0, h_qdes;
    std::vector<double> h_torque_radius;
    double* d_tr_stage = nullptr; size_t tr_stage_cap = 0;
    std::vector<double> h_link_gens;
    std::vector<unsigned long long> h_plane_skip;
    std::vector<double> h_prune_margin;
    int allocB = 0, allocO = 0;
    int* d_link_count = nullptr;
    double* d_link_center = nullptr;
    double* d_link_indep = nullptr;
    uint32_t* d_link_keys = nullptr;
    double* d_link_coeff = nullptr;
    int* d_tq_count = nullptr;
    double* d_tq_center = nullptr;
    double* d_tq_indep = nullptr;
    uint32_t* d_tq_keys = nullptr;
    double* d_tq_coeff = nullptr;
    double* d_planes = nullptr;
    double* d_obs_center = nullptr;
    int d_from_center = 0;
    int planes_lean = 0;
    int planes_have_d = 1;
    double planes_ms = 0;
    double* d_planes_ll = nullptr;
    int ll_shared = 0;
    unsigned long long* d_plane_skip = nullptr;
    double* d_bez = nullptr;
    double* d_k = nullptr;
    double* d_g = nullptr;
    double* d_jac = nullptr;
    double build_ms = 0;
    int p1_step_cap_hint = 0, p1_tv_shape_hint = 0;
    bool p1_two_cu_off = false;
    int p1_hint_B = 0, p1_hint_T = 0, p1_hint_O = 0, p1_hint_builds = 0;
    int build_info[4] = {0, 0, 0, 0};
    int max_link = 0, max_torque = 0;
    long long sum_link = 0, sum_torque = 0;
    void* p1 = nullptr;
    struct StepsGraph { const double* d_k; int steps; double* d_g; double* d_jac; hipGraphExec_t exec; unsigned long long last_use; };
    std::vector<StepsGraph> step_graphs;
    unsigned long long graph_clock = 0;
};

void armour_tuning_defaults(double* tuning);
bool armour_trace_p1();
bool armour_trace_solve();

int armour_p2_launch(const P2Tables& tb, int max_link, int max_torque, const unsigned long long* h_skip, const double* d_k, double* d_g, double* d_jac, hipStream_t stream,
                     int steps = 1, long long k_stride = 0, long long g_stride = 0, long long j_stride = 0, bool skip_collision_blocks = false);
int armour_relevance_build(ArmourPlanner* h, bool for_solver);
void armour_relevance_free(ArmourPlanner* h);
int armour_eval_violations_culled(ArmourPlanner* h, const double* d_k, ArmourViolation* d_out, hipStream_t st);
int armour_refresh_table_stats(ArmourPlanner* h);
int armour_checked_collision_rows(const ArmourPlanner* h);
double* armour_handle_pinned(ArmourPlanner* h, int slot, size_t bytes);
int armour_p2_slice_links_launch(const P2Tables& tb, const double* d_k, double* d_centers, hipStream_t stream);
P2Tables armour_make_tables(const ArmourPlanner* h);
int armour_upload_bounds(ArmourPlanner* h);
struct BuildStamps { double t[12]; const char* name[12]; int n; };
BuildStamps& armour_build_stamps();
void armour_build_stamp(const char* name);
int armour_bounds_launch(ArmourPlanner* h, const double* d_torque_radius);

int armour_p1_build(ArmourPlanner* h, const double* obstacles);
void armour_p1_free(ArmourPlanner* h);
int armour_p1_full_planes(ArmourPlanner* h, double* d_full);

inline int armour_p1_auto_kernel(int B, int T, int min_groups, bool fk_only) {
    return (long long)B * T >= 50ll * (fk_only ? min_groups * 5 / 3 : min_groups) ? ARMOUR_P1_KERNEL_TIME_VECTORISED : ARMOUR_P1_KERNEL_PER_STEP;
}

int armour_p1_debug_pz_op(ArmourPlanner* h, int op, int nops, const int* sz, const int* cnt, const uint64_t* const* keys,
                          const double* const* coef, const double* cen, const double* ind, const double* ind2, const double* consts,
                          int r, int out_cap, uint64_t* out_keys, double* out_coef, double* out_misc);
```

armour_amd/csrc/p2_eval.hip:

```cpp
#include "p2_tiles.h"

using namespace p2;

namespace {

template <bool WANT_G, bool WANT_J, bool MULTI, bool DFC, bool LL, int PPW, bool EX>
__global__ __launch_bounds__(P2_BLOCK) __attribute__((amdgpu_waves_per_eu(P2_WPE(DFC, MULTI)))) void armour_p2_eval_kernel(P2Tables tb, const double* __restrict__ k_all,
                                                                  double* __restrict__ g_all, double* __restrict__ jac_all,
                                                                  P2Launch lp) {
    extern __shared__ __attribute__((aligned(16))) unsigned char smem_raw[];
    const int b = blockIdx.y, role = blockIdx.x + lp.role0;
    const int n = tb.n, m = tb.m;
    const double* k0 = k_all + (size_t)b * n;
    double* g0 = WANT_G ? g_all + (size_t)b * m : nullptr;
    double* jac0 = WANT_J ? jac_all + (size_t)b * m * n : nullptr;
    const double k_first = ((int)threadIdx.x < n) ? k0[threadIdx.x] : 0.0;
#ifdef P2_ABLATE
    if ((P2_ABLATE & 1) && role < lp.nbc) return;
    if ((P2_ABLATE & 2) && role >= lp.nbc && role < lp.nbc + lp.nbt) return;
    if ((P2_ABLATE & 4) && role >= lp.nbc + lp.nbt) return;
#endif
    if (role < lp.nbc) collision_block<WANT_G, WANT_J, MULTI, DFC, LL, PPW, EX>(tb, lp, b, role, k0, k_first, g0, jac0, smem_raw);
    else if (role < lp.nbc + lp.nbt) torque_block<WANT_G, WANT_J, MULTI, DFC, LL, PPW, EX>(tb, lp, b, role, k0, k_first, g0, jac0, smem_raw);
    else limit_block<WANT_G, WANT_J, MULTI, DFC, LL, PPW, EX>(tb, lp, b, role, k0, k_first, g0, jac0, smem_raw);
}

__global__ void armour_p2_slice_links_kernel(P2Tables tb, const double* __restrict__ k_all, double* __restrict__ centers) {
    __shared__ KPow kp;
    const int b = blockIdx.y;
    fill_kpow(kp, threadIdx.x < (unsigned)tb.n ? k_all[(size_t)b * tb.n + threadIdx.x] : 0.0, tb.n);
    __syncthreads();
    const int task = blockIdx.x * blockDim.x + threadIdx.x;
    const int JT = tb.J * tb.T;
    if (task >= JT * 3) return;
    const int lt = task / 3, e = task - lt * 3;
    const size_t idx = (size_t)b * JT + lt;
    const int cnt = tb.link_count[idx];
    double cen = tb.link_center[idx * 3 + e];
    for (int mo = 0; mo < cnt; mo++)
        cen += mono_value(kp, tb.link_keys[idx * tb.capL + mo], tb.link_coeff[(idx * tb.capL + mo) * 3 + e], tb.n);
    const int l = lt / tb.T, t = lt - l * tb.T;
    centers[(((size_t)b * tb.T + t) * tb.J + l) * 3 + e] = interval_center(cen, tb.link_indep[idx * 3 + e]);
}

}

const char* armour_p2_kernel_name(void) { return "armour_p2_eval_kernel"; }

bool armour_p2_ex_layout_ok(unsigned long long skip) {
    unsigned long long live = ~skip & ((1ull << ARMOUR_NPLANES) - 1ull);
    if (__builtin_popcountll(live) != 24) return false;
    int pl[24];
    for (int i = 0; i < 24; i++) { pl[i] = __builtin_ctzll(live); live &= live - 1ull; }
    if (pl[11] >= ARMOUR_FIRST_LL_PLANE || pl[12] < ARMOUR_FIRST_LL_PLANE) return false;
    for (int w = 2; w < 4; w++) {
        const int p0 = pl[6 * w];
        if ((p0 - ARMOUR_FIRST_LL_PLANE) & 1) return false;
        for (int i = 1; i < 6; i++) if (pl[6 * w + i] != p0 + i) return false;
    }
    return true;
}

int armour_p2_plan(const P2Tables& tb, int max_link, int max_torque, const unsigned long long* h_skip, int steps, long long k_stride,
                   long long g_stride, long long j_stride, P2Launch* lp_out, size_t* smem_out, bool* dfc_out, bool* six_out, bool* exact_out) {
    P2Launch lp;
    lp.role0 = 0;
    lp.nbc = (tb.Q + P2_ROWS - 1) / P2_ROWS;
    lp.nbt = tb.row0 == 0 ? 0 : (tb.n * tb.T + P2_TQ_ROWS - 1) / P2_TQ_ROWS;
    lp.max_pairs = tb.O > 0 ? (P2_ROWS - 1) / tb.O + 2 : 1;
    lp.strideL = max_link > 0 ? max_link : 1;
    lp.strideT = max_torque > 0 ? max_torque : 1;
    lp.skip_by_value = (tb.B == 1 && h_skip) ? 1 : 0;
    lp.skip0 = lp.skip_by_value ? h_skip[0] : 0ull;
    lp.steps = steps; lp.k_stride = k_stride; lp.g_stride = g_stride; lp.j_stride = j_stride;
    lp.magic_O = div_magic(tb.O > 0 ? tb.O : 1); lp.magic_pp3 = div_magic(3 * lp.strideL);
    if (tb.Q >= (1 << 20)) { armour_set_error("more than 2^20 collision rows per problem"); return ARMOUR_ECAPACITY; }
    if (lp.strideL * 3 > P2_BLOCK * P2_TASK_ROUNDS) { armour_set_error("link PZ with %d monomials exceeds the P2 kernel's %d", lp.strideL, P2_BLOCK * P2_TASK_ROUNDS / 3); return ARMOUR_ECAPACITY; }
    lp.pair_chunk = std::max(1, std::min(std::min(lp.max_pairs, P2_BLOCK / P2_SL), (P2_BLOCK * P2_TASK_ROUNDS) / (lp.strideL * 3)));
    if (lp.strideT > 32 * P2_TQ_ROUNDS) { armour_set_error("torque PZ with %d monomials exceeds the P2 kernel's %d", lp.strideT, 32 * P2_TQ_ROUNDS); return ARMOUR_ECAPACITY; }
    const size_t col = ((size_t)lp.max_pairs * P2_SL + (size_t)lp.pair_chunk * lp.strideL * P2_SL + 4 * 64 * 4 + 64 * ARMOUR_MAX_FACTORS) * sizeof(double) + 4 * 64 * sizeof(int);
    const size_t tq = (size_t)P2_TQ_ROWS * lp.strideT * P2_TQW * sizeof(double);
    const size_t lim = (size_t)2 * ARMOUR_MAX_FACTORS * 8 * sizeof(double);
    const size_t smem = 2 * sizeof(KPow) + std::max(std::max(col, tq), lim);
    if (smem > 64 * 1024) { armour_set_error("P2 kernel needs %zu B of LDS (link/torque monomial counts too large)", smem); return ARMOUR_ECAPACITY; }
    const bool dfc = tb.obs_center != nullptr && tb.ll_shared;
    bool six = h_skip != nullptr;
    for (int b = 0; six && b < tb.B; b++) six = __builtin_popcountll(~h_skip[b] & ((1ull << ARMOUR_NPLANES) - 1ull)) <= 24;
    bool exact = six && tb.ex_allowed && lp.max_pairs <= lp.pair_chunk;
    for (int b = 0; exact && b < tb.B; b++) exact = armour_p2_ex_layout_ok(h_skip[b]);
    *lp_out = lp; *smem_out = smem; *dfc_out = dfc; *six_out = six; *exact_out = exact;
    return ARMOUR_OK;
}

int armour_p2_launch(const P2Tables& tb, int max_link, int max_torque, const unsigned long long* h_skip, const double* d_k, double* d_g, double* d_jac,
                     hipStream_t stream, int steps, long long k_stride, long long g_stride, long long j_stride, bool skip_collision_blocks) {
    if (!d_g && !d_jac) return ARMOUR_OK;
    P2Launch lp;
    size_t smem = 0;
    bool dfc, six, exact;
    const int rc = armour_p2_plan(tb, max_link, max_torque, h_skip, steps, k_stride, g_stride, j_stride, &lp, &smem, &dfc, &six, &exact);
    if (rc != ARMOUR_OK) return rc;
    if (skip_collision_blocks) lp.role0 = lp.nbc;
    dim3 grid(lp.nbc + lp.nbt + 1 - lp.role0, tb.B), block(P2_BLOCK);
#define P2_LAUNCH_M(G, J, M)                                                                                                                      \
    do {                                                                                                                                          \
        if (dfc && exact && !(M)) hipLaunchKernelGGL((armour_p2_eval_kernel<G, J, false, true, true, 6, true>), grid, block, smem, stream, tb, d_k, d_g, d_jac, lp);      \
        else if (dfc && six) hipLaunchKernelGGL((armour_p2_eval_kernel<G, J, M, true, true, 6, false>), grid, block, smem, stream, tb, d_k, d_g, d_jac, lp);                \
        else if (dfc) hipLaunchKernelGGL((armour_p2_eval_kernel<G, J, M, true, true, 9, false>), grid, block, smem, stream, tb, d_k, d_g, d_jac, lp);              \
        else if (tb.ll_shared && exact && !(M)) hipLaunchKernelGGL((armour_p2_eval_kernel<G, J, false, false, true, 6, true>), grid, block, smem, stream, tb, d_k, d_g, d_jac, lp); \
        else if (tb.ll_shared && six) hipLaunchKernelGGL((armour_p2_eval_kernel<G, J, M, false, true, 6, false>), grid, block, smem, stream, tb, d_k, d_g, d_jac, lp); \
        else if (tb.ll_shared) hipLaunchKernelGGL((armour_p2_eval_kernel<G, J, M, false, true, 9, false>), grid, block, smem, stream, tb, d_k, d_g, d_jac, lp); \
        else hipLaunchKernelGGL((armour_p2_eval_kernel<G, J, M, false, false, 9, false>), grid, block, smem, stream, tb, d_k, d_g, d_jac, lp);             \
    } while (0)
#define P2_LAUNCH(G, J)                                                                                                     \
    do {                                                                                                                    \
        if (steps > 1) P2_LAUNCH_M(G, J, true); else P2_LAUNCH_M(G, J, false);                                                                         \
    } while (0)
    if (d_g && d_jac) P2_LAUNCH(true, true);
    else if (d_g) P2_LAUNCH(true, false);
    else P2_LAUNCH(false, true);
#undef P2_LAUNCH
#undef P2_LAUNCH_M
    HIPCHK(hipGetLastError());
    return ARMOUR_OK;
}

int armour_p2_slice_links_launch(const P2Tables& tb, const double* d_k, double* d_centers, hipStream_t stream) {
    const int tasks = tb.J * tb.T * 3;
    dim3 grid((tasks + 255) / 256, tb.B), block(256);
    hipLaunchKernelGGL(armour_p2_slice_links_kernel, grid, block, 0, stream, tb, d_k, d_centers);
    HIPCHK(hipGetLastError());
    return ARMOUR_OK;
}
```

armour_amd/csrc/p2_tiles.h:

```cpp
#pragma once
#include <algorithm>
#include <cstdlib>

#include "bezier.h"
#include "cacc.h"
#include "common.h"

#define P2_BLOCK 256
#define P2_ROWS 64
#define P2_PPW 9
#define P2_TASK_ROUNDS 2
#define P2_TQ_ROWS 8
#define P2_TQ_ROUNDS 4
#define P2_SL (3 * (1 + ARMOUR_MAX_FACTORS))
#define P2_TQW (1 + ARMOUR_MAX_FACTORS)

#define P2_WPE(DFC, MULTI) ((DFC) && !(MULTI) ? 3 : 1)

namespace p2 {


#ifdef P2_TIMELINE
#define P2_STAMP(i) do { unsigned long long t__; asm volatile("s_memrealtime %0\n\ts_waitcnt lgkmcnt(0)" : "=s"(t__) :: "memory"); stamp[i] = t__; } while (0)
#else
#define P2_STAMP(i)
#endif

struct KPow {
    double pw[ARMOUR_MAX_FACTORS][4];
    double df[ARMOUR_MAX_FACTORS][4];
};

__device__ inline void fill_kpow(KPow& kp, double x, int n) {
    const int j = threadIdx.x;
    if (j < n) {
        kp.pw[j][0] = 1.0; kp.pw[j][1] = x; kp.pw[j][2] = x * x; kp.pw[j][3] = x * x * x;
        kp.df[j][0] = 0.0; kp.df[j][1] = 1.0; kp.df[j][2] = 2.0 * x; kp.df[j][3] = 3.0 * (x * x);
    }
}

__device__ __forceinline__ void lds_barrier() {
    __builtin_amdgcn_sched_barrier(0);
    asm volatile("s_waitcnt lgkmcnt(0)\n\ts_barrier" ::: "memory");
    __builtin_amdgcn_sched_barrier(0);
}

__device__ inline double mono_value(const KPow& kp, uint32_t key, double c, int n) {
    double f[ARMOUR_MAX_FACTORS];
#pragma unroll
    for (int j = 0; j < ARMOUR_MAX_FACTORS; j++) f[j] = (j < n) ? kp.pw[j][(key >> (2 * j)) & 3u] : 1.0;
    double v = c;
#pragma unroll
    for (int j = 0; j < ARMOUR_MAX_FACTORS; j++) v *= f[j];
    return v;
}
__device__ inline double mono_grad(const KPow& kp, uint32_t key, double c, int n, int kk) {
    double f[ARMOUR_MAX_FACTORS];
#pragma unroll
    for (int j = 0; j < ARMOUR_MAX_FACTORS; j++) {
        const uint32_t d = (key >> (2 * j)) & 3u;
        f[j] = (j < n) ? (j == kk ? kp.df[j][d] : kp.pw[j][d]) : 1.0;
    }
    double v = c;
#pragma unroll
    for (int j = 0; j < ARMOUR_MAX_FACTORS; j++) v *= f[j];
    return v;
}
template <bool WANT_J>
__device__ inline void mono_all(const KPow& kp, uint32_t key, double c, int n, double* o) {
    double pw[ARMOUR_MAX_FACTORS], df[ARMOUR_MAX_FACTORS];
#pragma unroll
    for (int j = 0; j < ARMOUR_MAX_FACTORS; j++) {
        const uint32_t d = (key >> (2 * j)) & 3u;
        pw[j] = (j < n) ? kp.pw[j][d] : 1.0;
        df[j] = (j < n) ? kp.df[j][d] : 0.0;
    }
    double v = c;
#pragma unroll
    for (int j = 0; j < ARMOUR_MAX_FACTORS; j++) v *= pw[j];
    o[0] = v;
    if (WANT_J) {
#pragma unroll
        for (int kk = 0; kk < ARMOUR_MAX_FACTORS; kk++) {
            double g = c;
#pragma unroll
            for (int j = 0; j < ARMOUR_MAX_FACTORS; j++) g *= (j == kk) ? df[j] : pw[j];
            o[1 + kk] = g;
        }
    }
}
__device__ inline double interval_center(double c, double r) {
    const double lo = c - r, hi = c + r;
    return (lo + hi) * 0.5;
}

__host__ __device__ inline unsigned long long div_magic(int d) { return ((1ull << 40) + (unsigned long long)d - 1ull) / (unsigned long long)d; }
__device__ inline int fast_div(int x, unsigned long long m) { return (int)(((unsigned long long)(unsigned)x * m) >> 40); }

typedef double v2d __attribute__((ext_vector_type(2)));

struct P2Launch {
    int nbc, nbt;
    int role0;
    int max_pairs;
    int strideL;
    int strideT;
    int pair_chunk;
    int skip_by_value;
    unsigned long long skip0;
    int steps;
    long long k_stride, g_stride, j_stride;
    unsigned long long magic_O, magic_pp3;
};

struct PassRegs {
    uint32_t tkey[P2_TASK_ROUNDS];
    double tco[P2_TASK_ROUNDS];
    int tcnt[P2_TASK_ROUNDS], tdst[P2_TASK_ROUNDS];
    double rc_cen, rc_ind;
    int rc_cnt;
};

__device__ inline void load_pass(const P2Tables& tb, const P2Launch& lp, int b, int lt_first, int p0, int pc, PassRegs& pr) {
    const int tid = threadIdx.x;
    const int per_pair = lp.strideL * P2_SL, per_pair3 = lp.strideL * 3;
    const int ntask = pc * per_pair3;
#pragma unroll
    for (int r = 0; r < P2_TASK_ROUNDS; r++) {
        const int task = tid + r * P2_BLOCK;
        pr.tcnt[r] = -1; pr.tdst[r] = 0; pr.tkey[r] = 0; pr.tco[r] = 0.0;
        if (task < ntask) {
            const int pi = fast_div(task, lp.magic_pp3), rem = task - pi * per_pair3, mo = rem / 3, e = rem - mo * 3;
            const size_t idx = (size_t)b * tb.J * tb.T + (lt_first + p0 + pi);
            pr.tcnt[r] = tb.link_count[idx] - mo;
            pr.tdst[r] = pi * per_pair + mo * P2_SL + e;
            if (mo < tb.capL) {
                pr.tkey[r] = tb.link_keys[idx * tb.capL + mo];
                pr.tco[r] = tb.link_coeff[(idx * tb.capL + mo) * 3 + e];
            }
        }
    }
    pr.rc_cen = 0.0; pr.rc_ind = 0.0; pr.rc_cnt = 0;
    if (tid < pc * P2_SL) {
        const int pi = tid / P2_SL, c = tid - pi * P2_SL, e = c % 3;
        const size_t idx = (size_t)b * tb.J * tb.T + (lt_first + p0 + pi);
        pr.rc_cnt = min(tb.link_count[idx], lp.strideL);
        if (c < 3) { pr.rc_cen = tb.link_center[idx * 3 + e]; pr.rc_ind = tb.link_indep[idx * 3 + e]; }
    }
}

__device__ inline void load_pass_uncond(const P2Tables& tb, const P2Launch& lp, int b, int lt_first, int pc, PassRegs& pr) {
    const int tid = threadIdx.x;
    const int per_pair = lp.strideL * P2_SL, per_pair3 = lp.strideL * 3;
    const int ntask = pc * per_pair3;
    const size_t idx0 = (size_t)b * tb.J * tb.T + lt_first;
#pragma unroll
    for (int r = 0; r < P2_TASK_ROUNDS; r++) {
        const int task = tid + r * P2_BLOCK;
        const bool valid = task < ntask;
        const int tk = valid ? task : 0;
        const int pi = fast_div(tk, lp.magic_pp3), rem = tk - pi * per_pair3, mo = rem / 3, e = rem - mo * 3;
        const size_t idx = idx0 + pi;
        const int moc = min(mo, tb.capL - 1);
        const int cnt = tb.link_count[idx];
        pr.tkey[r] = tb.link_keys[idx * tb.capL + moc];
        pr.tco[r] = tb.link_coeff[(idx * tb.capL + moc) * 3 + e];
        pr.tcnt[r] = cnt - (valid ? mo : (1 << 20));
        pr.tdst[r] = pi * per_pair + mo * P2_SL + e;
    }
    const int tc = tid < pc * P2_SL ? tid : 0;
    const int pi = tc / P2_SL, c = tc - pi * P2_SL, e = c % 3;
    const size_t idx = idx0 + pi;
    pr.rc_cnt = min(tb.link_count[idx], lp.strideL);
    pr.rc_cen = tb.link_center[idx * 3 + e];
    pr.rc_ind = tb.link_indep[idx * 3 + e];
}

template <bool WANT_G, bool WANT_J, bool MULTI, bool DFC, bool LL, int PPW, bool EX>
__device__ __forceinline__ void collision_block(const P2Tables& tb, const P2Launch& lp, const int b, const int role, const double* __restrict__ k0,
                                   const double k_first, double* __restrict__ g0_in, double* __restrict__ jac0_in, unsigned char* smem_raw) {
    KPow* kp2 = reinterpret_cast<KPow*>(smem_raw);
    double* lds = reinterpret_cast<double*>(smem_raw + 2 * sizeof(KPow));
    const int n = tb.n, T = tb.T, O = tb.O, Q = tb.Q, m = tb.m;
    const int tid = threadIdx.x, lane = tid & 63;
    const int wv = __builtin_amdgcn_readfirstlane(tid >> 6);
    double* g0 = WANT_G ? g0_in : nullptr;
    double* jac0 = WANT_J ? jac0_in : nullptr;
    const int nsteps = MULTI ? lp.steps : 1;
    double k_next = k_first;
    (void)lane; (void)wv; (void)T; (void)O; (void)Q; (void)m; (void)kp2; (void)lds; (void)g0; (void)jac0; (void)nsteps; (void)k_next;
#ifdef P2_TIMELINE
    unsigned long long stamp[8] = {0, 0, 0, 0, 0, 0, 0, 0};
#endif
    P2_STAMP(0);
#ifdef P2_TIMELINE
    const unsigned long long cyc0 = __builtin_amdgcn_s_memtime();
#endif
    double* sx = lds;
    double* terms = sx + (size_t)lp.max_pairs * P2_SL;
    double* part = terms + (size_t)lp.pair_chunk * lp.strideL * P2_SL;
    int* pneg = reinterpret_cast<int*>(part + 4 * 64 * 4);
    double* stage = part + 4 * 64 * 4 + 4 * 64 / 2;

    const int q_begin = role * P2_ROWS;
    const int q_end = min(Q, q_begin + P2_ROWS);
    const int q = min(q_begin + lane, q_end - 1);
    const size_t Qs = (size_t)armour_row_stride(Q);
    const double* pl0 = tb.planes + (size_t)b * armour_planes_per_problem(Q);
    const v2d* plAB = reinterpret_cast<const v2d*>(pl0) + q;
    const v2d* plCD = reinterpret_cast<const v2d*>(pl0 + armour_planes_cd_offset(Q)) + q;
    const v2d* plLL = reinterpret_cast<const v2d*>(pl0 + armour_planes_dll_offset(Q)) + q;
    const double* plD = pl0 + armour_planes_d_offset(Q) + q;
    const int JT = tb.J * T;
    const int q_lt = fast_div(q, lp.magic_O), q_o = q - q_lt * O;
    const double* pll = tb.planes_ll + (size_t)b * armour_planes_ll_per_problem(JT) + (size_t)q_lt * ARMOUR_LL_RECORD;
    unsigned long long live = ~(lp.skip_by_value ? lp.skip0 : tb.plane_skip[b]) & ((1ull << ARMOUR_NPLANES) - 1ull);
    const bool plane0_live = (live & 1ull) != 0;
    const int na = __popcll(live), base = na >> 2, rem = na & 3;
    const int my_cnt = base + (wv < rem ? 1 : 0), my_start = wv * base + min(wv, rem);
    for (int s = 0; s < my_start; s++) live &= live - 1ull;
    double a0[PPW], a1[PPW], a2[PPW], dd[PPW], dl[PPW];
    const int lt_first = q_begin / O;
    const int npairs = (q_end - 1) / O - lt_first + 1;
    const bool single_pass = npairs <= lp.pair_chunk;
    PassRegs pr;
    if (EX) load_pass_uncond(tb, lp, b, lt_first, npairs, pr);
    v2d raw[EX ? 12 : 1];
    bool ll_wave = false;
    if (EX) {
        static_assert(!EX || PPW == 6, "the EX kernels hold six planes per wave");
        ll_wave = wv >= 2;
        const v2d* ra[12];
        const double* da[6];
        if (ll_wave) {
            const int pll0 = __builtin_ctzll(live) - ARMOUR_FIRST_LL_PLANE;
            const v2d* nrm = reinterpret_cast<const v2d*>(pll + (size_t)pll0 * 3);
#pragma unroll
            for (int j = 0; j < 9; j++) ra[j] = nrm + j;
#pragma unroll
            for (int j = 0; j < 3; j++) ra[9 + j] = plLL + (size_t)((pll0 >> 1) + j) * Qs;
#pragma unroll
            for (int i = 0; i < 6; i++) da[i] = plD + (size_t)(ARMOUR_FIRST_LL_PLANE + pll0 + i) * Qs;
        } else {
#pragma unroll
            for (int i = 0; i < 6; i++) {
                const size_t o = (size_t)__builtin_ctzll(live) * Qs;
                live &= live - 1ull;
                ra[2 * i] = plAB + o; ra[2 * i + 1] = plCD + o; da[i] = plD + o;
            }
        }
#pragma unroll
        for (int j = 0; j < 12; j++) raw[j] = *ra[j];
#pragma unroll
        for (int i = 0; i < 6; i++) { dd[i] = 0.0; if (!DFC) dd[i] = *da[i]; }
    } else {
#pragma unroll
    for (int i = 0; i < PPW; i++) {
        a0[i] = 0.0; a1[i] = 0.0; a2[i] = 0.0; dd[i] = 0.0; dl[i] = 0.0;
        if (i < my_cnt) {
            const int pidx = __builtin_ctzll(live);
            const size_t o = (size_t)pidx * Qs;
            live &= live - 1ull;
            if (LL && pidx >= ARMOUR_FIRST_LL_PLANE) {
                const double* al = pll + (size_t)(pidx - ARMOUR_FIRST_LL_PLANE) * 3;
                a0[i] = al[0]; a1[i] = al[1]; a2[i] = al[2];
                dl[i] = pl0[armour_plane_index(Q, q, pidx, 4)];
            } else {
                const v2d ab = plAB[o], cd = plCD[o];
                a0[i] = ab.x; a1[i] = ab.y; a2[i] = cd.x; dl[i] = cd.y;
                if (!LL && pidx >= ARMOUR_FIRST_LL_PLANE) dl[i] = pl0[armour_plane_index(Q, q, pidx, 4)];
            }
            if (!DFC) dd[i] = plD[o];
        }
#if defined(P2_ABLATE) && (P2_ABLATE & 8)
        a0[i] = 1.0 + i; a1[i] = 0.5; a2[i] = 0.25; dd[i] = 0.1; dl[i] = 0.2;
#endif
    }
    }
    double oc0 = 0.0, oc1 = 0.0, oc2 = 0.0;
    if (DFC) {
        const double* oc = tb.obs_center + (size_t)b * 3 * O + q_o;
        oc0 = oc[0]; oc1 = oc[O]; oc2 = oc[2 * (size_t)O];
    }
    P2_STAMP(1);
    const int per_pair = lp.strideL * P2_SL;
    if (MULTI && single_pass) load_pass(tb, lp, b, lt_first, 0, npairs, pr);
    const double* xs = sx + (q_lt - lt_first) * P2_SL;
    for (int s = 0; s < nsteps; s++) {
        KPow& kp = kp2[s & 1];
        const double k_cur = k_next;
        if (tid < n && s + 1 < nsteps) k_next = k0[(size_t)(s + 1) * lp.k_stride + tid];
        fill_kpow(kp, k_cur, n);
        double* g = WANT_G ? g0 + (size_t)s * lp.g_stride : nullptr;
        double* jac = WANT_J ? jac0 + (size_t)s * lp.j_stride : nullptr;
        for (int p0 = 0; p0 < npairs; p0 += lp.pair_chunk) {
            const int pc = min(lp.pair_chunk, npairs - p0);
            if (!EX && (!MULTI || !single_pass)) load_pass(tb, lp, b, lt_first, p0, pc, pr);
            if (EX) lds_barrier(); else __syncthreads();
            P2_STAMP(2);
#pragma unroll
            for (int r = 0; r < P2_TASK_ROUNDS; r++) {
                if (pr.tcnt[r] > 0) {
                    double o8[P2_TQW];
                    mono_all<WANT_J>(kp, pr.tkey[r], pr.tco[r], n, o8);
                    double* dst = terms + pr.tdst[r];
                    dst[0] = o8[0];
                    if (WANT_J) {
#pragma unroll
                        for (int kk = 0; kk < ARMOUR_MAX_FACTORS; kk++) dst[3 + kk * 3] = o8[1 + kk];
                    }
                }
            }
            if (EX) lds_barrier(); else __syncthreads();
            P2_STAMP(3);
            if (tid < pc * P2_SL) {
                const int pi = tid / P2_SL, c = tid - pi * P2_SL, out = c / 3, e2 = c - out * 3;
                double acc = (!EX || out == 0) ? pr.rc_cen : 0.0;
                const double* tp = terms + (size_t)pi * per_pair + c;
#pragma unroll 4
                for (int mo = 0; mo < pr.rc_cnt; mo++) acc += tp[mo * P2_SL];
                if (out == 0) acc = interval_center(acc, pr.rc_ind);
                sx[(p0 + pi) * P2_SL + (out == 0 ? e2 : 3 + (out - 1) * 3 + e2)] = acc;
            }
            if (EX) lds_barrier(); else __syncthreads();
        }
        P2_STAMP(4);
        const double x0 = xs[0], x1 = xs[1], x2 = xs[2];
        if (EX) {
            if (ll_wave) {
#pragma unroll
                for (int i = 0; i < 6; i++) {
                    const int e = 3 * i;
                    a0[i] = (e & 1) ? raw[e >> 1].y : raw[e >> 1].x;
                    a1[i] = ((e + 1) & 1) ? raw[(e + 1) >> 1].y : raw[(e + 1) >> 1].x;
                    a2[i] = ((e + 2) & 1) ? raw[(e + 2) >> 1].y : raw[(e + 2) >> 1].x;
                    dl[i] = (i & 1) ? raw[9 + (i >> 1)].y : raw[9 + (i >> 1)].x;
                }
            } else {
#pragma unroll
                for (int i = 0; i < 6; i++) { a0[i] = raw[2 * i].x; a1[i] = raw[2 * i].y; a2[i] = raw[2 * i + 1].x; dl[i] = raw[2 * i + 1].y; }
            }
        }
        if (DFC) {
#pragma unroll
            for (int i = 0; i < PPW; i++) dd[i] = a0[i] * oc0 + a1[i] * oc1 + a2[i] * oc2;
        }
        double max_elt = -100000000.0;
        int best = (wv == 0 && plane0_live) ? 0 : -2;
#pragma unroll
        for (int i = 0; i < PPW; i++) {
            const bool nz = (a0[i] != 0.0) | (a1[i] != 0.0) | (a2[i] != 0.0);
            const double dot = a0[i] * x0 + a1[i] * x1 + a2[i] * x2;
            const double pos_res = nz ? dot - (dd[i] + dl[i]) : -100000000.0;
            const double neg_res = nz ? -dot - (-dd[i] + dl[i]) : -100000000.0;
            const bool c1 = pos_res > max_elt;
            max_elt = c1 ? pos_res : max_elt; best = c1 ? 2 * i : best;
            const bool c2 = neg_res > max_elt;
            max_elt = c2 ? neg_res : max_elt; best = c2 ? 2 * i + 1 : best;
        }
        {
            double mA0 = 0.0, mA1 = 0.0, mA2 = 0.0;
            const int bs = best >> 1;
#pragma unroll
            for (int i = 0; i < PPW; i++) {
                const bool hit = bs == i;
                mA0 = hit ? a0[i] : mA0; mA1 = hit ? a1[i] : mA1; mA2 = hit ? a2[i] : mA2;
            }
            double* my = part + ((size_t)wv * 64 + lane) * 4;
            my[0] = max_elt; my[1] = mA0; my[2] = mA1; my[3] = mA2;
            pneg[wv * 64 + lane] = best & 1;
        }
        __syncthreads();
        P2_STAMP(5);
        {
            const double* c0 = part + (size_t)lane * 4;
            double m_elt = c0[0], mA0 = c0[1], mA1 = c0[2], mA2 = c0[3];
            int neg = pneg[lane];
#pragma unroll
            for (int w2 = 1; w2 < 4; w2++) {
                const double* o = part + ((size_t)w2 * 64 + lane) * 4;
                const double oe = o[0], o1 = o[1], o2 = o[2], o3 = o[3];
                const int on = pneg[w2 * 64 + lane];
                const bool c = oe > m_elt;
                m_elt = c ? oe : m_elt; mA0 = c ? o1 : mA0; mA1 = c ? o2 : mA1; mA2 = c ? o3 : mA2; neg = c ? on : neg;
            }
#if defined(P2_ABLATE) && (P2_ABLATE & 32)
            if (WANT_G && wv == 0 && m_elt == 12345.678) g[(size_t)tb.row0 + q_begin + lane] = -m_elt;
#else
            if (WANT_G && wv == 0 && q_begin + lane < q_end) g[(size_t)tb.row0 + q_begin + lane] = -m_elt;
#endif
            if (WANT_J) {
#pragma unroll
                for (int h = 0; h < 2; h++) {
                    const int kk = wv + 4 * h;
                    if (kk < n) {
                        const double* dx = xs + 3 + kk * 3;
                        const double dot = mA0 * dx[0] + mA1 * dx[1] + mA2 * dx[2];
                        stage[lane * n + kk] = neg ? dot : -dot;
                    }
                }
            }
        }
        if (WANT_J) {
            __syncthreads();
            const int total = (q_end - q_begin) * n;
            double* jrow = jac + ((size_t)tb.row0 + q_begin) * n;
#if defined(P2_ABLATE) && (P2_ABLATE & 32)
            for (int i = tid; i < total; i += P2_BLOCK) if (stage[i] == 12345.678) jrow[i] = stage[i];
#else
            for (int i = tid; i < total; i += P2_BLOCK) jrow[i] = stage[i];
#endif
        }
    }
#ifdef P2_TIMELINE
    P2_STAMP(6);
    stamp[7] = __builtin_amdgcn_s_memtime() - cyc0;
    if (tid == 0 && (role == 0 || role == lp.nbc / 2 || role == lp.nbc - 1)) {
        const int slot = role == 0 ? 0 : role == lp.nbc - 1 ? 2 : 1;
        for (int i2 = 0; i2 < 8; i2++) g0_in[(size_t)tb.row0 + Q + slot * 8 + i2] = (double)(stamp[i2] & 0xffffffffffffull);
    }
#endif
}

template <bool WANT_G, bool WANT_J, bool MULTI, bool DFC, bool LL, int PPW, bool EX>
__device__ __forceinline__ void torque_block(const P2Tables& tb, const P2Launch& lp, const int b, const int role, const double* __restrict__ k0,
                                   const double k_first, double* __restrict__ g0_in, double* __restrict__ jac0_in, unsigned char* smem_raw) {
    KPow* kp2 = reinterpret_cast<KPow*>(smem_raw);
    double* lds = reinterpret_cast<double*>(smem_raw + 2 * sizeof(KPow));
    const int n = tb.n, T = tb.T, O = tb.O, Q = tb.Q, m = tb.m;
    const int tid = threadIdx.x, lane = tid & 63;
    const int wv = __builtin_amdgcn_readfirstlane(tid >> 6);
    double* g0 = WANT_G ? g0_in : nullptr;
    double* jac0 = WANT_J ? jac0_in : nullptr;
    const int nsteps = MULTI ? lp.steps : 1;
    double k_next = k_first;
    (void)lane; (void)wv; (void)T; (void)O; (void)Q; (void)m; (void)kp2; (void)lds; (void)g0; (void)jac0; (void)nsteps; (void)k_next;
    double* terms = lds;
    const int r = tid >> 5, ml = tid & 31;
    const int row = (role - lp.nbc) * P2_TQ_ROWS + r;
    const bool live = row < n * T;
    int t = 0, j = 0, cnt = 0;
    size_t idx = 0;
    uint32_t tkey[P2_TQ_ROUNDS];
    double tco[P2_TQ_ROUNDS];
    double cen0 = 0.0, ind0 = 0.0;
    if (live) {
        t = row / n; j = row - t * n;
        idx = ((size_t)b * n + j) * T + t;
        cnt = min(tb.tq_count[idx], lp.strideT);
        if (ml == 0) { cen0 = tb.tq_center[idx]; ind0 = tb.tq_indep[idx]; }
#pragma unroll
        for (int rr = 0; rr < P2_TQ_ROUNDS; rr++) {
            const int mo = ml + rr * 32;
            tkey[rr] = 0; tco[rr] = 0.0;
            if (mo < lp.strideT && mo < tb.capT) { tkey[rr] = tb.tq_keys[idx * tb.capT + mo]; tco[rr] = tb.tq_coeff[idx * tb.capT + mo]; }
        }
    }
    for (int s = 0; s < nsteps; s++) {
        KPow& kp = kp2[s & 1];
        const double k_cur = k_next;
        if (tid < n && s + 1 < nsteps) k_next = k0[(size_t)(s + 1) * lp.k_stride + tid];
        fill_kpow(kp, k_cur, n);
        double* g = WANT_G ? g0 + (size_t)s * lp.g_stride : nullptr;
        double* jac = WANT_J ? jac0 + (size_t)s * lp.j_stride : nullptr;
        __syncthreads();
        if (live) {
#pragma unroll
            for (int rr = 0; rr < P2_TQ_ROUNDS; rr++) {
                const int mo = ml + rr * 32;
                if (mo < cnt) {
                    double* tp = terms + ((size_t)r * lp.strideT + mo) * P2_TQW;
                    double o8[P2_TQW];
                    mono_all<WANT_J>(kp, tkey[rr], tco[rr], n, o8);
                    tp[0] = o8[0];
                    if (WANT_J) {
#pragma unroll
                        for (int kk = 0; kk < ARMOUR_MAX_FACTORS; kk++) tp[1 + kk] = o8[1 + kk];
                    }
                }
            }
        }
        __syncthreads();
        if (live && ml <= n) {
            const double* tp = terms + (size_t)r * lp.strideT * P2_TQW + ml;
            if (ml == 0) {
                if (WANT_G) {
                    double cen = cen0;
#pragma unroll 4
                    for (int mo = 0; mo < cnt; mo++) cen += tp[mo * P2_TQW];
                    g[row] = interval_center(cen, ind0);
                }
            } else if (WANT_J) {
                double gr = 0.0;
#pragma unroll 4
                for (int mo = 0; mo < cnt; mo++) gr += tp[mo * P2_TQW];
                jac[(size_t)row * n + (ml - 1)] = gr;
            }
        }
    }
}

template <bool WANT_G, bool WANT_J, bool MULTI, bool DFC, bool LL, int PPW, bool EX>
__device__ __forceinline__ void limit_block(const P2Tables& tb, const P2Launch& lp, const int b, const int role, const double* __restrict__ k0,
                                   const double k_first, double* __restrict__ g0_in, double* __restrict__ jac0_in, unsigned char* smem_raw) {
    KPow* kp2 = reinterpret_cast<KPow*>(smem_raw);
    double* lds = reinterpret_cast<double*>(smem_raw + 2 * sizeof(KPow));
    const int n = tb.n, T = tb.T, O = tb.O, Q = tb.Q, m = tb.m;
    const int tid = threadIdx.x, lane = tid & 63;
    const int wv = __builtin_amdgcn_readfirstlane(tid >> 6);
    double* g0 = WANT_G ? g0_in : nullptr;
    double* jac0 = WANT_J ? jac0_in : nullptr;
    const int nsteps = MULTI ? lp.steps : 1;
    double k_next = k_first;
    (void)lane; (void)wv; (void)T; (void)O; (void)Q; (void)m; (void)kp2; (void)lds; (void)g0; (void)jac0; (void)nsteps; (void)k_next;
    double* pv = lds;
    const int jv = tid >> 3, piece = tid & 7;
    const double* bz = tb.bez + (size_t)b * 3 * n;
    if (tb.mode == ARMOUR_MODE_ARMTD) {
        for (int s = 0; s < nsteps; s++) {
            const double* k = k0 + (size_t)s * lp.k_stride;
            double* g = WANT_G ? g0 + (size_t)s * lp.g_stride : nullptr;
            double* jac = WANT_J ? jac0 + (size_t)s * lp.j_stride : nullptr;
            if (tid < n) {
                const cacc::Extrema e = cacc::joint_extrema(bz[tid], bz[n + tid], bz[2 * n + tid] * k[tid]);
                const cacc::Cand c4[4] = {e.q_min, e.q_max, e.qd_min, e.qd_max};
                const size_t off = (size_t)tb.row0 + Q;
                for (int r = 0; r < 4; r++) {
                    const size_t row = off + (size_t)r * n + tid;
                    if (WANT_G) g[row] = c4[r].v;
                    if (WANT_J) for (int c = 0; c < n; c++) jac[row * n + c] = (c == tid) ? c4[r].d : 0.0;
                }
            }
        }
        return;
    }
    for (int s = 0; s < nsteps; s++) {
        const double* k = k0 + (size_t)s * lp.k_stride;
        double* g = WANT_G ? g0 + (size_t)s * lp.g_stride : nullptr;
        double* jac = WANT_J ? jac0 + (size_t)s * lp.j_stride : nullptr;
        if (jv < 2 * n && piece < 6) {
            const int i = jv % n;
            const bool vel = jv >= n;
            const double q0 = bz[i], a = bz[n + i], bb = bz[2 * n + i], ka = tb.k_range[i] * k[i];
            double e2, e3, v;
            if (!vel) bez::q_stationary(a, bb, ka, &e2, &e3); else bez::qd_stationary(a, bb, ka, &e2, &e3);
            if (piece < 4) {
                const double tt = piece == 0 ? 0.0 : piece == 1 ? e2 : piece == 2 ? e3 : 1.0;
                v = vel ? bez::qd_des(q0, a, bb, ka, tt) : bez::q_des(q0, a, bb, ka, tt);
            } else {
                const int sg = piece == 4 ? +1 : -1;
                v = vel ? bez::qd_extremum_dk(q0, a, bb, ka, sg) : bez::q_extremum_dk(q0, a, bb, ka, sg);
            }
            pv[jv * 8 + piece] = v;
            if (piece == 1) pv[jv * 8 + 6] = e2;
            if (piece == 2) pv[jv * 8 + 7] = e3;
        }
        __syncthreads();
        if (tid < 2 * n) {
            const int i = tid % n;
            const bool vel = tid >= n;
            const double* v = pv + tid * 8;
            const double v1 = v[0], v2 = v[1], v3 = v[2], v4 = v[3], e2 = v[6], e3 = v[7];
            double mn, mx;
            int mnId, mxId;
            if (v1 < v4) { mn = v1; mnId = 1; mx = v4; mxId = 4; } else { mn = v4; mnId = 4; mx = v1; mxId = 1; }
            if (0 <= e2 && e2 <= 1) { if (v2 < mn) { mn = v2; mnId = 2; } if (mx < v2) { mx = v2; mxId = 2; } }
            if (0 <= e3 && e3 <= 1) { if (v3 < mn) { mn = v3; mnId = 3; } if (mx < v3) { mx = v3; mxId = 3; } }
            const double sc = vel ? tb.k_range[i] / tb.duration : tb.k_range[i];
            const double dmn = (mnId == 1 ? 0.0 : mnId == 2 ? v[4] : mnId == 3 ? v[5] : 1.0) * sc;
            const double dmx = (mxId == 1 ? 0.0 : mxId == 2 ? v[4] : mxId == 3 ? v[5] : 1.0) * sc;
            const size_t off = (size_t)tb.row0 + Q;
            const size_t r_mn = off + (vel ? 2 * n : 0) + i, r_mx = r_mn + n;
            if (WANT_G) { g[r_mn] = vel ? mn / tb.duration : mn; g[r_mx] = vel ? mx / tb.duration : mx; }
            if (WANT_J) {
                for (int c = 0; c < n; c++) {
                    jac[r_mn * n + c] = (c == i) ? dmn : 0.0;
                    jac[r_mx * n + c] = (c == i) ? dmx : 0.0;
                }
            }
        }
        __syncthreads();
    }
}

}
```

armour_amd/csrc/solver_device.hip:

```cpp
#include <algorithm>
#include <atomic>
#include <cmath>
#include <cstring>

#include "bezier.h"
#include "cacc.h"
#include "common.h"
#include "p2_tiles.h"
#include "solver_common.h"
#include "solver_device.h"

using namespace p2;
using namespace slv;

namespace {

enum { CMD_EVAL = 1, CMD_DONE = 4 };
enum { ST_AFTER_FIRST = 0, ST_AFTER_TRIAL = 1, ST_AFTER_RELIN = 2, ST_AFTER_VERDICT = 3 };
constexpr double kInf = 1e300;
#define WAVE_LDS_SYNC() do { __builtin_amdgcn_fence(__ATOMIC_SEQ_CST, "wavefront"); __builtin_amdgcn_wave_barrier(); } while (0)

__device__ inline unsigned ld_coh(const unsigned* p) { return __hip_atomic_load(p, __ATOMIC_RELAXED, __HIP_MEMORY_SCOPE_AGENT); }
__device__ inline int ld_coh(const int* p) { return __hip_atomic_load(p, __ATOMIC_RELAXED, __HIP_MEMORY_SCOPE_AGENT); }
__device__ inline long long ld_coh(const long long* p) { return __hip_atomic_load(p, __ATOMIC_RELAXED, __HIP_MEMORY_SCOPE_AGENT); }
// ... 614 lines not shown

template <int WPS>
__device__ __forceinline__ int leader_step(const SolveArgs& a, Leader& L, QpShared& QS, int b, long long viol_fx, int bad, SolveRow* cand,
                                  unsigned char* flags_g, double* x_pub, double* lds_stage) {
    const int n = a.tb.n, tid = threadIdx.x;
    const double viol = viol_from_fixed(viol_fx);
#define LSTAMP(k) do { if (a.stamps && tid == 0 && first) a.stamps[(size_t)b * 64 + 32 + (k)] = wall_clock64() - L.t_start; } while (0)
    const bool first = L.stage == ST_AFTER_FIRST;
    const double* pt = first ? L.x : L.xt;
    if (tid < n) {
        const bool cont = (a.continuous_mask >> tid) & 1;
        const double qp = plan_point(a, L.bz, tid, pt[tid]);
        const double eg = cont ? wrap_to_pi(qp - L.qdes[tid]) : (qp - L.qdes[tid]);
        L.np[tid] = 2 * eg * plan_dk(a, L.bz, tid) * a.cost_scale;
        const double e = cont ? wrap_to_pi(L.qdes[tid] - qp) : (L.qdes[tid] - qp);
        L.z[tid] = e * e;
    }
    __syncthreads();
    if (tid == 0) {
        const double fpt = cost_sum(a, L.z);
        L.stop = 0;
        if (first) {
            L.f = fpt; L.evals = 1; L.viol = viol; L.bad = bad; L.status = 0;
            for (int j = 0; j < n; j++) L.gradf[j] = L.np[j];
        } else {
            L.evals++;
            const double phi = fpt + L.mu * viol;
            if (phi <= L.phi0 + 1e-4 * L.alpha * L.dphi || L.ls == a.max_ls) {
                if (L.ls == a.max_ls && phi > L.phi0) { L.status = 4; L.stop = 1; }
                else {
                    for (int j = 0; j < n; j++) { L.x[j] = L.xt[j]; L.gradf[j] = L.np[j]; }
                    L.f = fpt; L.viol = viol; L.bad = bad; L.iters++; L.it++;
                    L.evals++;
                }
            } else {
                L.alpha *= 0.5;
                L.ls++;
                for (int j = 0; j < n; j++) L.xt[j] = L.x[j] + L.alpha * L.d[j];
                L.stop = 3;
            }
        }
        L.stage = ST_AFTER_TRIAL;
        if (L.stop == 0) {
            if (L.it >= a.max_iter) { L.status = 2; L.stop = 1; }
            else if (a.budget_ticks >= 0 && wall_clock64() - L.t_start >= a.budget_ticks) { L.status = 5; L.stop = 1; }
        }
    }
    __syncthreads();
    LSTAMP(0);
    if (L.stop == 0) {
        bool finish = false;
        if (!gather_candidates(a, L, b, cand)) {
            if (tid == 0) L.status = -1;
            finish = true;
        }
        if (!finish) {
            LSTAMP(1);
            if (tid == 0) {
                QS.first_ok = 4;
                for (int j = 0; j < NV; j++) L.invHd[j] = 1.0 / L.Hd[j];
            }
            const double* staged = nullptr;
            if (L.ncand > 64 * (WPS == 1 ? 4 : 2) - 2 * n && L.ncand <= a.lds_rows) {
                for (int i = tid; i < L.ncand; i += 256) {
                    const SolveRow& r = cand[i];
#pragma unroll
                    for (int j = 0; j < NV; j++) lds_stage[(size_t)j * a.lds_rows + i] = r.a[j];
                    lds_stage[(size_t)NV * a.lds_rows + i] = r.v;
                }
                staged = lds_stage;
            }
            __syncthreads();
            solve_qp_wave<WPS>(a, L, QS, cand, staged, flags_g);
            __syncthreads();
            if (tid == 0) {
                int k = 0;
                while (k < 3 && !QS.w[k].feasible) k++;
                const QpWave& W = QS.w[k];
                for (int j = 0; j < NV; j++) L.qx[j] = W.qx[j];
                L.max_mult = W.max_mult; L.feasible = W.feasible; L.sigma = attempt_sigma(k); L.qp_iter = W.qp_iter;
                if (a.stamps) {
                    for (int e = 0; e < 4; e++) {
                        a.stamps[(size_t)b * 64 + 44 + e] += QS.w[e].qp_iter;
                        if (QS.w[e].feasible && QS.w[e].qp_iter > a.stamps[(size_t)b * 64 + 48]) a.stamps[(size_t)b * 64 + 48] = QS.w[e].qp_iter;
                        if (QS.w[e].qp_iter > 60 && !QS.w[e].feasible) a.stamps[(size_t)b * 64 + 49] += 1;
                    }
                }
            }
            __syncthreads();
            LSTAMP(2);
            if (tid == 0 && a.stamps) { if (L.it == 0) { a.stamps[(size_t)b * 64 + 40] = L.qp_iter; a.stamps[(size_t)b * 64 + 41] = L.ncand; } a.stamps[(size_t)b * 64 + 42] += L.qp_iter; a.stamps[(size_t)b * 64 + 43] += 1; }
            if (tid == 0) {
                if (!L.feasible) { L.status = 3; L.stop = 1; }
                else {
                    double dn = 0, gd = 0;
                    for (int j = 0; j < n; j++) { L.d[j] = L.qx[j]; dn = fmax(dn, fabs(L.qx[j])); gd += L.gradf[j] * L.qx[j]; }
                    if (dn <= a.tol * 1e-2 || (dn <= a.tol && L.viol <= a.tol)) { L.status = 1; L.stop = 1; }
                    else {
                        L.mu = fmax(L.mu, 1.5 * L.max_mult + 1e-3);
                        L.phi0 = L.f + L.mu * L.viol;
                        L.dphi = gd - L.mu * (1.0 - L.sigma) * L.viol;
                        if (L.dphi > -1e-14) L.dphi = -1e-14;
                        L.alpha = 1.0;
                        L.ls = 0;
                        for (int j = 0; j < n; j++) L.xt[j] = L.x[j] + L.alpha * L.d[j];
                        L.stop = 3;
                    }
                }
            }
        }
        __syncthreads();
        if (finish && tid == 0) L.stop = 1;
        __syncthreads();
    }
    int next;
    if (L.stop == 3) {
        const int outside = a.culled && tid < n && !(fabs(L.xt[tid]) <= 1.0 + 1e-6) ? 1 : 0;
        if (__syncthreads_or(outside)) {
            if (tid == 0) a.out[b].status = -1;
            __syncthreads();
            return CMD_DONE;
        }
        if (tid < n) st_coh(x_pub + tid, L.xt[tid]);
        next = CMD_EVAL;
    } else {
        if (tid == 0) {
            ArmourSolveResult& r = a.out[b];
            if (L.status == -1) r.status = -1;
            else {
                for (int j = 0; j < NV; j++) r.k_opt[j] = j < n ? L.x[j] : 0.0;
                r.cost = L.f;
                r.max_violation = L.viol;
                r.feasible = L.bad == 0 ? 1 : 0;
                r.iterations = L.iters;
                r.evaluations = L.evals + 1;
                r.status = L.status;
                r.time_ms = (double)(wall_clock64() - L.t_start);
            }
        }
        next = CMD_DONE;
    }
    __syncthreads();
    return next;
}

template <bool LL, int PPW, int WPS>
__global__ __launch_bounds__(P2_BLOCK) __attribute__((amdgpu_waves_per_eu(WPS, WPS))) void armour_solve_kernel(const SolveArgs* __restrict__ args) {
    const SolveArgs& a = *args;
    extern __shared__ __attribute__((aligned(16))) unsigned char smem_raw[];
    __shared__ ScanShared scan_sh;
    __shared__ Leader L;
    __shared__ QpShared QS;
    __shared__ int s_cmd;
    __shared__ double s_x[NV];
    const int tid = threadIdx.x;
    const int b_local = blockIdx.x / a.nb, jb = blockIdx.x - b_local * a.nb;
    const int b = a.b0 + b_local;
    const bool leader = jb == 0;
    const int n = a.tb.n, m = a.tb.m;
    SolveCtl* c = a.ctl + b;
    TileSet ts = {0, 0, 0, 0};
    int my_tiles = a.n_tiles;
    if (a.culled) { ts = problem_tiles(a, b); my_tiles = ts.ntq + ts.nsp + 1; }
    const int t0 = (int)(((long long)jb * my_tiles) / a.nb), t1 = (int)(((long long)(jb + 1) * my_tiles) / a.nb);
    int role = 0, r0 = 0, r1 = 0, rdummy;
    if (!a.culled) {
        tile_info(a, t0, role, r0, rdummy);
        tile_info(a, t1 - 1, role, rdummy, r1);
    }
    SolveRow* my_rows = a.blk_rows + ((size_t)(b - a.b0) * a.nb + jb) * a.cap_blk;
    SolveRow* cand = a.qp_rows + (size_t)(b - a.b0) * a.cap_rows;
    unsigned char* flags_g = a.flags + (size_t)(b - a.b0) * 8 * (a.cap_rows + 2 * NV);
    double* g = a.g + (size_t)b * m;
    double* jac = a.jac + (size_t)b * m * n;
    if (leader && tid < 3 * NV) L.bz[tid] = tid < 3 * n ? a.tb.bez[(size_t)b * 3 * n + tid] : 0.0;
    if (leader && tid >= 32 && tid < 32 + NV) L.qdes[tid - 32] = tid - 32 < n ? a.q_des[(size_t)b * n + tid - 32] : 0.0;
    __syncthreads();
    if (leader && tid == 0) {
        L.t_start = wall_clock64();
        for (int j = 0; j < NV; j++) {
            L.x[j] = 0.0;
            double Hd = 1e-12;
            if (j < n) {
                const double dk = plan_dk(a, L.bz, j);
                Hd = hess_diag(a.cost_scale, dk);
            }
            L.Hd[j] = Hd;
        }
        L.mu = 1.0; L.it = 0; L.iters = 0; L.evals = 0; L.status = 0; L.stage = ST_AFTER_FIRST; L.ncand = 0; L.sigma = 0.0;
    }
    const double* my_x = s_x;
    unsigned phase = 0;
    const long long t_block = wall_clock64();
    for (;;) {
        if (tid == 0) {
            unsigned w;
            unsigned spins = 0;
            while (((w = ld_coh(&c->go)) >> 3) < phase) {
                __builtin_amdgcn_s_sleep(2);
                if ((++spins & 1023u) == 0 && wall_clock64() - t_block > a.hard_ticks) { w = (unsigned)CMD_DONE; break; }
            }
            asm volatile("" ::: "memory");
            s_cmd = (int)(w & 7u);
        }
        __syncthreads();
        const int cmd = s_cmd;
        if (cmd == CMD_DONE) {
            if (tid == 0) st_coh(&a.blk_word[(size_t)(b - a.b0) * a.nb + jb].flag, 0u);
            break;
        }
        if (tid < NV) s_x[tid] = tid < n ? ld_coh(&c->x[tid]) : 0.0;
        __syncthreads();
        const double kf = tid < n ? s_x[tid] : 0.0;
        for (int t = t0; t < t1; t++) {
            if (a.culled) {
                if (t < ts.ntq + ts.nsp) {
                    KPow& kp = *reinterpret_cast<KPow*>(smem_raw);
                    fill_kpow(kp, kf, n);
                    __syncthreads();
                    if (t < ts.ntq) {
                        const int i = t * P2_BLOCK + tid;
                        if (i < ts.cntq) sparse_torque_row(a.tb, b, a.tq_tiles[(size_t)b * a.tq_cap + i], a.lp.strideT, kp, g, jac);
                    } else {
                        const int i = (t - ts.ntq) * P2_BLOCK + tid;
                        if (i < ts.cnt2) sparse_collision_row<true>(a.tb, a.sl, b, i, kp, g, jac);
                    }
                    __syncthreads();
                    continue;
                }
                role = a.lp.nbc + a.lp.nbt;
            } else {
                int tr0, tr1;
                tile_info(a, t, role, tr0, tr1);
            }
            if (role < a.lp.nbc) {
                if constexpr (LL) {
                    if (a.tb.obs_center) collision_block<true, true, false, true, LL, PPW, false>(a.tb, a.lp, b, role, my_x, kf, g, jac, smem_raw);
                    else collision_block<true, true, false, false, LL, PPW, false>(a.tb, a.lp, b, role, my_x, kf, g, jac, smem_raw);
                } else collision_block<true, true, false, false, LL, PPW, false>(a.tb, a.lp, b, role, my_x, kf, g, jac, smem_raw);
            }
            else if (role < a.lp.nbc + a.lp.nbt) torque_block<true, true, false, false, LL, PPW, false>(a.tb, a.lp, b, role, my_x, kf, g, jac, smem_raw);
            else limit_block<true, true, false, false, LL, PPW, false>(a.tb, a.lp, b, role, my_x, kf, g, jac, smem_raw);
            __syncthreads();
        }
        __builtin_amdgcn_fence(__ATOMIC_SEQ_CST, "workgroup");
        __syncthreads();
        long long vfx = 0;
        int cnt = 0, bad = 0;
        if (a.culled) scan_tiles(a, b, ts, t0, t1, my_rows, a.cap_blk, scan_sh, vfx, cnt, bad);
        else scan_rows<3>(a, b, r0, r1, my_rows, a.cap_blk, scan_sh, vfx, cnt, bad);
        BlockWord* mine = a.blk_word + (size_t)(b - a.b0) * a.nb + jb;
        if (tid == 0) { st_coh(&mine->viol, vfx); st_coh(&mine->bad, bad); st_coh(&mine->count, cnt); }
        wait_my_memory_ops();
        __syncthreads();
        phase++;
        if (tid == 0) st_coh(&mine->flag, phase);
        if (!leader) continue;
        bool group_lost = false;
        for (unsigned spins = 0;; spins++) {
            int all = 1;
#pragma unroll
            for (int e = 0; e < 4; e++) { const int j2 = tid * 4 + e; if (j2 < a.nb && ld_coh(&a.blk_word[(size_t)(b - a.b0) * a.nb + j2].flag) < phase) all = 0; }
            if (__syncthreads_and(all)) break;
            if ((spins & 255u) == 255u && __syncthreads_or(wall_clock64() - t_block > a.hard_ticks ? 1 : 0)) { group_lost = true; break; }
        }
        asm volatile("" ::: "memory");
        if (group_lost) {
            if (tid == 0) {
                a.out[b].status = -1;
                wait_my_memory_ops();
                st_coh(&c->go, phase * 8u + (unsigned)CMD_DONE);
                st_coh(&a.blk_word[(size_t)(b - a.b0) * a.nb + jb].flag, 0u);
            }
            break;
        }
        long long viol_fx = 0;
        int nbad = 0;
        {
            long long v = 0;
            int bd = 0;
#pragma unroll
            for (int e = 0; e < 4; e++) { const int j2 = tid * 4 + e; if (j2 < a.nb) { v += ld_coh(&a.blk_word[(size_t)(b - a.b0) * a.nb + j2].viol); bd += ld_coh(&a.blk_word[(size_t)(b - a.b0) * a.nb + j2].bad); } }
            block_sum(v, bd, scan_sh.red, scan_sh.redi);
            viol_fx = v; nbad = bd;
            __syncthreads();
        }
        if (a.stamps && tid == 0 && phase <= 16) a.stamps[(size_t)b * 64 + 2 * (phase - 1)] = wall_clock64() - L.t_start;
        const int next = leader_step<WPS>(a, L, QS, b, viol_fx, nbad, cand, flags_g, c->x, reinterpret_cast<double*>(smem_raw));
        if (a.stamps && tid == 0 && phase <= 16) a.stamps[(size_t)b * 64 + 2 * (phase - 1) + 1] = wall_clock64() - L.t_start;
        wait_my_memory_ops();
        __syncthreads();
        if (tid == 0) st_coh(&c->go, phase * 8u + (unsigned)next);
        __syncthreads();
    }
}

}

int armour_solve_device_capacity(const P2Tables& tb, int max_link, int max_torque, const unsigned long long* h_skip, int device, int b_launch, int waves_per_simd, SolvePlan* plan,
                                 int n_tiles_override) {
    P2Launch lp;
    size_t smem = 0;
    bool dfc, six, exact;
    int rc = armour_p2_plan(tb, max_link, max_torque, h_skip, 1, 0, 0, 0, &lp, &smem, &dfc, &six, &exact);
    if (rc != ARMOUR_OK) return rc;
    plan->lp = lp; plan->smem = smem; plan->six = six;
    plan->n_tiles = n_tiles_override > 0 ? n_tiles_override : lp.nbt + lp.nbc + 1;
    int coop = 0;
    HIPCHK(hipDeviceGetAttribute(&coop, hipDeviceAttributeCooperativeLaunch, device));
    if (!coop) { plan->capacity = 0; return ARMOUR_OK; }
    hipDeviceProp_t prop;
    HIPCHK(hipGetDeviceProperties(&prop, device));
    const void* fn1 = !tb.ll_shared ? (const void*)armour_solve_kernel<false, 9, 1> : six ? (const void*)armour_solve_kernel<true, 6, 1> : (const void*)armour_solve_kernel<true, 9, 1>;
    const void* fn2 = !tb.ll_shared ? (const void*)armour_solve_kernel<false, 9, 2> : six ? (const void*)armour_solve_kernel<true, 6, 2> : (const void*)armour_solve_kernel<true, 9, 2>;
    const int wps_env = waves_per_simd;
    const size_t smem1 = std::max(smem, (size_t)96 * 1024), smem2 = std::max(smem, (size_t)40 * 1024);
    int per_cu = 0;
    {
        static std::atomic<unsigned long long> set1[3], set2[3];
        const int which = !tb.ll_shared ? 0 : six ? 1 : 2;
        const unsigned long long bit = 1ull << (device & 63);
        if (smem1 > 96 * 1024 || !(set1[which].load() & bit)) { HIPCHK(hipFuncSetAttribute(fn1, hipFuncAttributeMaxDynamicSharedMemorySize, (int)smem1)); set1[which].fetch_or(bit); }
        if (smem2 > 40 * 1024 || !(set2[which].load() & bit)) { HIPCHK(hipFuncSetAttribute(fn2, hipFuncAttributeMaxDynamicSharedMemorySize, (int)smem2)); set2[which].fetch_or(bit); }
    }
    HIPCHK(hipOccupancyMaxActiveBlocksPerMultiprocessor(&per_cu, fn1, P2_BLOCK, smem1));
    const int cap1 = per_cu * prop.multiProcessorCount;
    const int blocks1 = cap1 / std::max(1, b_launch);
    const bool one = wps_env ? wps_env == 1 : (blocks1 >= 1 && (n_tiles_override > 0 || (plan->n_tiles + blocks1 - 1) / blocks1 <= 24));
    const void* fn = one ? fn1 : fn2;
    plan->fn = fn;
    plan->smem = one ? smem1 : smem2;
    if (!one) HIPCHK(hipOccupancyMaxActiveBlocksPerMultiprocessor(&per_cu, fn, P2_BLOCK, smem2));
    plan->capacity = per_cu * prop.multiProcessorCount;
    int rate_khz = 0;
    HIPCHK(hipDeviceGetAttribute(&rate_khz, hipDeviceAttributeWallClockRate, device));
    plan->ticks_per_ms = rate_khz > 0 ? (double)rate_khz : 100000.0;
    return ARMOUR_OK;
}

int armour_solve_device_launch(const SolveArgs* d_args, int nb, const SolvePlan& plan, int B, hipStream_t stream) {
    const SolveArgs* p = d_args;
    void* params[1] = {&p};
    HIPCHK(hipLaunchCooperativeKernel(plan.fn, dim3((unsigned)B * (unsigned)nb), dim3(P2_BLOCK), params, (unsigned)plan.smem, stream));
    return ARMOUR_OK;
}
```

armour_amd/planner.py:

```python
import ctypes as C

import numpy as np

from . import _lib
from ._lib import ArmourLimits, ArmourParams, ArmourRobot, check


def _dp(a):
    return None if a is None else a.ctypes.data_as(C.POINTER(C.c_double))


def kinova_robot():
    r = ArmourRobot()
    _lib.load().armour_robot_kinova_gen3_no_gripper(C.byref(r))
    return r


def kinova_gripper_robot():
    r = ArmourRobot()
    _lib.load().armour_robot_kinova_gen3_gripper(C.byref(r))
    return r


def fetch_robot(payload_mass_uncertainty=0.0):
    r = ArmourRobot()
    _lib.load().armour_robot_fetch(C.byref(r))
    if payload_mass_uncertainty:
        r.mass_uncertainty_link[r.num_joints - 1] = payload_mass_uncertainty
        r.inertia_uncertainty_link[r.num_joints - 1] = payload_mass_uncertainty
    return r


def fetch8_robot(payload_mass_uncertainty=0.0):
    r = ArmourRobot()
    check(_lib.load().armour_robot_fetch8(C.byref(r)))
    if payload_mass_uncertainty:
        r.mass_uncertainty_link[r.num_joints - 1] = payload_mass_uncertainty
        r.inertia_uncertainty_link[r.num_joints - 1] = payload_mass_uncertainty
    return r


def default_params(T=128):
    p = ArmourParams()
    _lib.load().armour_params_default(C.byref(p), T)
    return p


def desired_trajectory(q0, qd0, qdd0, k, t, k_range=None, duration=1.0, t_plan=0.5, previous=None):
    q0 = np.ascontiguousarray(q0, dtype=np.float64).ravel()
    qd0 = np.ascontiguousarray(qd0, dtype=np.float64).ravel()
    qdd0 = np.ascontiguousarray(qdd0, dtype=np.float64).ravel()
    n = q0.size
    if k is None or np.any(np.isnan(np.asarray(k, dtype=np.float64))):
        if t <= t_plan and np.linalg.norm(qd0) > 1e-8 and previous is not None:
            return previous(t + t_plan)
        return q0.copy(), np.zeros(n), np.zeros(n)
    L = _lib.load()
    kr = np.full(n, np.pi / 48) if k_range is None else np.ascontiguousarray(k_range, dtype=np.float64).ravel()
    kk = np.ascontiguousarray(k, dtype=np.float64).ravel()
    q, qd, qdd = np.zeros(n), np.zeros(n), np.zeros(n)
    check(L.armour_desired_trajectory(n, _dp(q0), _dp(qd0), _dp(qdd0), _dp(kr), float(duration), _dp(kk), float(t), _dp(q), _dp(qd), _dp(qdd)))
    return q, qd, qdd


def _violation_dict(v):
    return dict(l1_violation=v.l1_violation, worst=v.worst, worst_row=v.worst_row, n_violated=v.n_violated,
                n_outside_slack=v.n_outside_slack, feasible=bool(v.feasible))


def _solve_options(L, max_iterations, tolerance, max_wall_time_s, host_qp, device_qp=False):
    opt = _lib.ArmourSolveOptions()
    L.armour_solve_options_default(C.byref(opt))
    if max_iterations is not None:
        opt.max_iterations = max_iterations
    if tolerance is not None:
        opt.tolerance = tolerance
    if max_wall_time_s is not None:
        opt.max_wall_time_s = max_wall_time_s
    if host_qp:
        opt.force_host_qp = 1.0
    elif device_qp:
        opt.force_host_qp = -1.0
    return opt


def _solve_dicts(res, n):
    return [dict(k_opt=np.array(r.k_opt[:n]), cost=r.cost, max_violation=r.max_violation, feasible=bool(r.feasible),
                 iterations=r.iterations, evaluations=r.evaluations, status=r.status, time_ms=r.time_ms) for r in res]


def batch_partition(B, n_slots):
    first = (C.c_int32 * (n_slots + 1))()
    check(_lib.load().armour_batch_partition(B, n_slots, first))
    return list(first)


class ArmourBatchNLP:

    def __init__(self, devices, robot=None, params=None, T=128, limits=None):
        self.L = _lib.load()
        self.robot = robot if robot is not None else kinova_robot()
        self.params = params if params is not None else default_params(T)
        self.T, self.J, self.n = self.params.num_time_steps, self.robot.num_joints, self.robot.num_factors
        self.limits = limits if limits is not None else ArmourLimits()
        self.devices = list(devices)
        dv = (C.c_int32 * len(self.devices))(*self.devices)
        h = C.c_void_p()
        check(self.L.armour_batch_create(C.byref(self.robot), C.byref(self.params), C.byref(self.limits), dv, len(self.devices), C.byref(h)))
        self.h = h
        self.B = self.O = self.m = 0

    def close(self):
        if getattr(self, "h", None):
            self.L.armour_batch_destroy(self.h)
            self.h = None

    def __del__(self):
        try:
            self.close()
        except Exception:
            pass

    def set_option(self, option, value):
        check(self.L.armour_batch_set_option(self.h, option, float(value)))
        return self

    def set_parameters(self, q0, qd0, qdd0, q_des, obstacles):
        q0, qd0, qdd0, q_des = [np.ascontiguousarray(np.atleast_2d(np.asarray(a, dtype=np.float64))) for a in (q0, qd0, qdd0, q_des)]
        B = q0.shape[0]
        obs = np.asarray(obstacles, dtype=np.float64)
        obs = np.ascontiguousarray(obs.reshape(B, -1, 12)) if obs.size else np.zeros((B, 0, 12))
        O = obs.shape[1]
        check(self.L.armour_batch_set_problems(self.h, B, O, _dp(q0), _dp(qd0), _dp(qdd0), _dp(q_des), _dp(obs) if O else None))
        b, n, m, g = C.c_int32(), C.c_int32(), C.c_int32(), C.c_int32()
        check(self.L.armour_batch_get_sizes(self.h, C.byref(b), C.byref(n), C.byref(m), C.byref(g)))
        self.B, self.O, self.m = b.value, O, m.value
        return self

    def _k(self, x):
        return np.ascontiguousarray(np.asarray(x, dtype=np.float64).reshape(self.B, self.n))

    def get_bounds_info(self):
        xl, xu = np.zeros(self.n), np.zeros(self.n)
        gl, gu = np.zeros((self.B, self.m)), np.zeros((self.B, self.m))
        check(self.L.armour_batch_get_bounds(self.h, _dp(xl), _dp(xu), _dp(gl), _dp(gu)))
        return xl, xu, gl, gu

    def eval_g_jac(self, x):
        g, jac = np.zeros((self.B, self.m)), np.zeros((self.B, self.m, self.n))
        check(self.L.armour_batch_eval_g_jac(self.h, _dp(self._k(x)), _dp(g), _dp(jac)))
        return g, jac

    def eval_violations(self, x):
        out = (_lib.ArmourViolation * self.B)()
        check(self.L.armour_batch_eval_violations(self.h, _dp(self._k(x)), out))
        return [_violation_dict(v) for v in out]

    def solve(self, max_iterations=None, tolerance=None, max_wall_time_s=None, host_qp=False, device_qp=False):
        opt = _solve_options(self.L, max_iterations, tolerance, max_wall_time_s, host_qp, device_qp)
        res = (_lib.ArmourSolveResult * self.B)()
        check(self.L.armour_batch_solve(self.h, C.byref(opt), res))
        return _solve_dicts(res, self.n)

    @property
    def build_ms(self):
        v = C.c_double()
        per = (C.c_double * len(self.devices))()
        check(self.L.armour_batch_get_build_ms(self.h, C.byref(v), per))
        return v.value

    def prune_margin(self):
        out = np.zeros(self.B)
        check(self.L.armour_batch_get_prune_margin(self.h, _dp(out)))
        return out

    def build_info(self):
        out = (C.c_int32 * (4 * len(self.devices)))()
        check(self.L.armour_batch_get_build_info(self.h, out))
        kn = {0: None, 1: "per_step", 2: "time_vectorised"}
        return [None if out[4 * d] == 0 else {"kernel": kn[out[4 * d]], "waves": out[4 * d + 1], "sort_entries": out[4 * d + 2], "launches": out[4 * d + 3]}
                for d in range(len(self.devices))]


class ArmourNLP:

    def __init__(self, robot=None, params=None, T=128, device=0, limits=None):
        self.L = _lib.load()
        self.robot = robot if robot is not None else kinova_robot()
        self.params = params if params is not None else default_params(T)
        self.T = self.params.num_time_steps
        self.J = self.robot.num_joints
        self.n = self.robot.num_factors
        self.limits = limits if limits is not None else ArmourLimits()
        h = C.c_void_p()
        check(self.L.armour_create(C.byref(self.robot), C.byref(self.params), C.byref(self.limits), device, C.byref(h)))
        self.h = h
        self.B = 0
        self.O = 0
        self.m = 0

    def _pinned(self, name, shape):
        cache = self.__dict__.setdefault("_pin", {})
        ent = cache.get(name)
        if ent is None or ent[1].shape != tuple(shape):
            if ent is not None:
                self.L.armour_free_pinned(ent[0])
            nbytes = int(np.prod(shape)) * 8
            ptr = C.c_void_p()
            check(self.L.armour_alloc_pinned(nbytes, C.byref(ptr)))
            arr = np.ctypeslib.as_array((C.c_double * (nbytes // 8)).from_address(ptr.value)).reshape(shape)
            ent = (ptr, arr)
            cache[name] = ent
        return ent[1]

    def close(self):
        for ptr, _ in self.__dict__.get("_pin", {}).values():
            self.L.armour_free_pinned(ptr)
        self.__dict__["_pin"] = {}
        if getattr(self, "h", None):
            self.L.armour_destroy(self.h)
            self.h = None

    def __del__(self):
        try:
            self.close()
        except Exception:
            pass

    def set_parameters(self, q0, qd0, qdd0, q_des, obstacles):
        q0, qd0, qdd0, q_des = [np.ascontiguousarray(np.atleast_2d(np.asarray(a, dtype=np.float64))) for a in (q0, qd0, qdd0, q_des)]
        obs = np.asarray(obstacles, dtype=np.float64)
        B = q0.shape[0]
        obs = np.ascontiguousarray(obs.reshape(B, -1, 12)) if obs.size else np.zeros((B, 0, 12))
        O = obs.shape[1]
        for a in (q0, qd0, qdd0, q_des):
            if a.shape != (B, self.n):
                raise ValueError(f"expected shape ({B},{self.n}), got {a.shape}")
        self._obs = obs
        check(self.L.armour_set_problems(self.h, B, O, _dp(q0), _dp(qd0), _dp(qdd0), _dp(q_des), _dp(obs) if O else None))
        self.problem = dict(q0=q0.copy(), qd0=qd0.copy(), qdd0=qdd0.copy(), q_des=q_des.copy())
        self._after_set(B, O)
        return self

    def set_parameters_armtd(self, q0, qd0, q_des, jrs, k_range, obstacles):
        q0, qd0, q_des, k_range = [np.ascontiguousarray(np.atleast_2d(np.asarray(a, dtype=np.float64))) for a in (q0, qd0, q_des, k_range)]
        B = q0.shape[0]
        jrs = np.ascontiguousarray(np.asarray(jrs, dtype=np.float64).reshape(B, self.n, 6, self.T))
        obs = np.asarray(obstacles, dtype=np.float64)
        obs = np.ascontiguousarray(obs.reshape(B, -1, 12)) if obs.size else np.zeros((B, 0, 12))
        O = obs.shape[1]
        for a in (q0, qd0, q_des, k_range):
            if a.shape != (B, self.n):
                raise ValueError(f"expected shape ({B},{self.n}), got {a.shape}")
        self._obs = obs
        self.problem = None
        check(self.L.armour_set_problems_armtd(self.h, B, O, _dp(q0), _dp(qd0), _dp(q_des), _dp(jrs), _dp(k_range), _dp(obs) if O else None))
        self._after_set(B, O)
        return self

    def _after_set(self, B, O):
        b, n, m = C.c_int32(), C.c_int32(), C.c_int32()
        check(self.L.armour_get_sizes(self.h, C.byref(b), C.byref(n), C.byref(m)))
        self.B, self.O, self.m = b.value, O, m.value

    def debug_load_tables(self, q0, qd0, qdd0, q_des, tables):
        q0, qd0, qdd0, q_des = [np.ascontiguousarray(np.atleast_2d(np.asarray(a, dtype=np.float64))) for a in (q0, qd0, qdd0, q_des)]
        t = {k: np.ascontiguousarray(v) for k, v in tables.items()}
        B, O = q0.shape[0], t["A"].shape[3]
        u64 = C.POINTER(C.c_uint64)
        i32 = C.POINTER(C.c_int32)
        check(self.L.armour_debug_load_tables(
            self.h, B, O, _dp(q0), _dp(qd0), _dp(qdd0), _dp(q_des),
            t["link_count"].ctypes.data_as(i32), _dp(t["link_center"]), t["link_keys"].ctypes.data_as(u64), _dp(t["link_coeffs"]), t["link_keys"].shape[-1],
            t["torque_count"].ctypes.data_as(i32), _dp(t["torque_center"]), t["torque_keys"].ctypes.data_as(u64), _dp(t["torque_coeffs"]), t["torque_keys"].shape[-1],
            _dp(t["A"]), _dp(t["d"]), _dp(t["delta"]), _dp(t["torque_radius"])))
        self._after_set(B, O)
        return self

    def get_nlp_info(self):
        return self.n, self.m, self.m * self.n

    def get_bounds_info(self):
        xl, xu = np.zeros(self.n), np.zeros(self.n)
        gl, gu = np.zeros((self.B, self.m)), np.zeros((self.B, self.m))
        check(self.L.armour_get_bounds(self.h, _dp(xl), _dp(xu), _dp(gl), _dp(gu)))
        return xl, xu, gl, gu

    def get_starting_point(self):
        return np.zeros((self.B, self.n))

    def _k(self, x):
        k = np.ascontiguousarray(np.asarray(x, dtype=np.float64).reshape(self.B, self.n))
        return k

    def eval_f(self, x):
        f = np.zeros(self.B)
        check(self.L.armour_eval_f(self.h, _dp(self._k(x)), _dp(f)))
        return f

    def eval_grad_f(self, x):
        gf = np.zeros((self.B, self.n))
        check(self.L.armour_eval_grad_f(self.h, _dp(self._k(x)), _dp(gf)))
        return gf

    def eval_g(self, x):
        g = np.zeros((self.B, self.m))
        check(self.L.armour_eval_g_jac(self.h, _dp(self._k(x)), _dp(g), None))
        return g

    def eval_jac_g(self, x):
        jac = np.zeros((self.B, self.m, self.n))
        check(self.L.armour_eval_g_jac(self.h, _dp(self._k(x)), None, _dp(jac)))
        return jac

    def eval_g_jac(self, x, pinned=False, out=None):
        if out is not None:
            k, (g, jac) = self._k(x), out
            assert g.dtype == np.float64 and jac.dtype == np.float64 and g.flags.c_contiguous and jac.flags.c_contiguous
            assert g.size == self.B * self.m and jac.size == self.B * self.m * self.n
        elif pinned:
            k = self._pinned("k", (self.B, self.n)); k[...] = np.asarray(x, dtype=np.float64).reshape(self.B, self.n)
            gj = self._pinned("gjac", (self.B * self.m * (1 + self.n),))
            g, jac = gj[:self.B * self.m].reshape(self.B, self.m), gj[self.B * self.m:].reshape(self.B, self.m, self.n)
        else:
            k, g, jac = self._k(x), np.zeros((self.B, self.m)), np.zeros((self.B, self.m, self.n))
        check(self.L.armour_eval_g_jac(self.h, _dp(k), _dp(g), _dp(jac)))
        return g, jac

    def eval_g_jac_device(self, d_k, d_g, d_jac, stream=0):
        check(self.L.armour_eval_g_jac_device(self.h, d_k, d_g, d_jac, stream))

    def eval_g_jac_device_steps(self, d_k, steps, d_g, d_jac, stream=0):
        check(self.L.armour_eval_g_jac_device_steps(self.h, d_k, steps, d_g, d_jac, stream))

    def prepare_steps(self, d_k, steps, d_g, d_jac):
        check(self.L.armour_prepare_steps(self.h, d_k, steps, d_g, d_jac))

    def eval_g_jac_device_multi(self, d_k, points, d_g, d_jac, stream=0):
        check(self.L.armour_eval_g_jac_device_multi(self.h, d_k, points, d_g, d_jac, stream))

    def finalize_solution(self, g):
        g = np.ascontiguousarray(np.asarray(g, dtype=np.float64).reshape(self.B, self.m))
        feas = np.zeros(self.B, dtype=np.int32)
        check(self.L.armour_check_feasible(self.h, _dp(g), feas.ctypes.data_as(C.POINTER(C.c_int32))))
        return feas.astype(bool)

    def set_option(self, option, value):
        check(self.L.armour_set_option(self.h, option, float(value)))
        return self

    def get_option(self, option):
        v = C.c_double()
        check(self.L.armour_get_option(self.h, option, C.byref(v)))
        return v.value

    def eval_violations(self, x):
        out = (_lib.ArmourViolation * self.B)()
        check(self.L.armour_eval_violations(self.h, _dp(self._k(x)), out))
        return [_violation_dict(v) for v in out]

    def row_relevance(self):
        rel = np.zeros((self.B, self.m), dtype=np.uint8)
        cnt = np.zeros(self.B, dtype=np.int32)
        ms = C.c_double()
        check(self.L.armour_get_row_relevance(self.h, rel.ctypes.data_as(C.POINTER(C.c_uint8)), cnt.ctypes.data_as(C.POINTER(C.c_int32)), C.byref(ms)))
        return rel.astype(bool), cnt, ms.value

    def solver_rows(self):
        mask = np.zeros((self.B, self.m), dtype=np.uint8)
        cnt, tq = np.zeros(self.B, dtype=np.int32), np.zeros(self.B, dtype=np.int32)
        ms = C.c_double()
        i32 = C.POINTER(C.c_int32)
        check(self.L.armour_get_solver_rows(self.h, mask.ctypes.data_as(C.POINTER(C.c_uint8)), cnt.ctypes.data_as(i32), tq.ctypes.data_as(i32), C.byref(ms)))
        return mask.astype(bool), cnt, tq, ms.value

    def eval_violations_device(self, d_k, d_out, stream=0):
        check(self.L.armour_eval_violations_device(self.h, d_k, d_out, stream))

    def solve(self, max_iterations=None, tolerance=None, max_wall_time_s=None, host_qp=False, device_qp=False):
        opt = _solve_options(self.L, max_iterations, tolerance, max_wall_time_s, host_qp, device_qp)
        res = (_lib.ArmourSolveResult * self.B)()
        check(self.L.armour_solve(self.h, C.byref(opt), res))
        return [dict(k_opt=np.array(r.k_opt[:self.n]), cost=r.cost, max_violation=r.max_violation, feasible=bool(r.feasible),
                     iterations=r.iterations, evaluations=r.evaluations, status=r.status, time_ms=r.time_ms) for r in res]

    def eval_constraint(self, k, b=0):
        x = np.zeros((self.B, self.n))
        x[b] = k
        g, jac = self.eval_g_jac(x)
        _, _, gl, gu = self.get_bounds_info()
        g, jac, gl, gu = g[b], jac[b], gl[b], gu[b]
        two_sided = gl > -1e18
        h = np.concatenate([g - gu, (gl - g)[two_sided]])
        grad_h = np.concatenate([jac, -jac[two_sided]], axis=0).T
        return h, np.zeros(0), grad_h, np.zeros((self.n, 0))

    def debug_pz_op(self, op, operands, consts=None, r=0, out_cap=4096):
        n = len(operands)
        i32 = C.c_int32 * n
        sz = i32(*[o["sz"] for o in operands])
        cnt = i32(*[len(o["keys"]) for o in operands])
        ks = [np.ascontiguousarray(o["keys"], dtype=np.uint64) if len(o["keys"]) else np.zeros(1, np.uint64) for o in operands]
        cs = [np.ascontiguousarray(o["coef"], dtype=np.float64).reshape(-1) if len(o["keys"]) else np.zeros(1) for o in operands]
        kp = (C.POINTER(C.c_uint64) * n)(*[k.ctypes.data_as(C.POINTER(C.c_uint64)) for k in ks])
        cp = (C.POINTER(C.c_double) * n)(*[_dp(c) for c in cs])
        cen, ind, ind2 = np.zeros((n, 9)), np.zeros((n, 9)), np.zeros((n, 9))
        for i, o in enumerate(operands):
            cen[i, :o["sz"]] = o["cen"]; ind[i, :o["sz"]] = o["ind"]; ind2[i, :o["sz"]] = o.get("ind2", o["ind"])
        cst = np.zeros(4) if consts is None else np.ascontiguousarray(np.concatenate([np.asarray(consts, dtype=np.float64), np.zeros(4)])[:4])
        ok, oc, misc = np.zeros(out_cap, np.uint64), np.zeros(out_cap * 9), np.zeros(64)
        check(self.L.armour_debug_pz_op(self.h, op, n, sz, cnt, kp, cp, _dp(cen), _dp(ind), _dp(ind2), _dp(cst), r, out_cap,
                                        ok.ctypes.data_as(C.POINTER(C.c_uint64)), _dp(oc), _dp(misc)))
        m, osz = int(misc[0]), int(misc[1])
        return dict(keys=ok[:m].copy(), coef=oc[:m * osz].reshape(m, osz).copy(), cen=misc[3:3 + osz].copy(), ind=misc[12:12 + osz].copy(),
                    ind2=misc[21:21 + osz].copy(), flags=int(misc[2]), cycles=float(misc[30]), raw_terms=int(misc[31]), prof=misc[32:60].copy(),
                    margin_sq=float(misc[60]), thr_sq=float(misc[61]))

    def torque_radius(self):
        out = np.zeros((self.B, self.n, self.T))
        check(self.L.armour_get_torque_radius(self.h, _dp(out)))
        return out

    def link_generators(self):
        out = np.zeros((self.B, self.T, self.J, 3, 6))
        check(self.L.armour_get_link_generators(self.h, _dp(out)))
        return out

    def link_centers(self, x):
        out = np.zeros((self.B, self.T, self.J, 3))
        check(self.L.armour_get_link_centers(self.h, _dp(self._k(x)), _dp(out)))
        return out

    def pz(self, which, i, t, b=0):
        w = {"link": 0, "torque": 1}[which]
        sz = 3 if w == 0 else 1
        cap = 4096
        cen = np.zeros(2 * sz)
        keys = np.zeros(cap, dtype=np.uint64)
        co = np.zeros((cap, sz))
        cnt = check(self.L.armour_get_pz(self.h, b, w, i, t, _dp(cen), keys.ctypes.data_as(C.POINTER(C.c_uint64)), _dp(co), cap))
        return cen[:sz], cen[sz:], keys[:cnt], co[:cnt]

    def polyzonotope(self, which, i, t, b=0):
        from . import cora
        c, ind, keys, co = self.pz(which, i, t, b=b)
        return cora.to_polyzonotope(c, ind, keys, co, self.n)

    def table_sizes(self):
        out = (C.c_int64 * 4)()
        check(self.L.armour_get_table_sizes(self.h, out))
        return dict(sum_link=out[0], sum_torque=out[1], max_link=out[2], max_torque=out[3])

    def hyperplanes(self):
        A = np.zeros((self.B, self.T, self.J, self.O, 36, 3))
        d = np.zeros((self.B, self.T, self.J, self.O, 36))
        delta = np.zeros((self.B, self.T, self.J, self.O, 36))
        check(self.L.armour_get_hyperplanes(self.h, _dp(A), _dp(d), _dp(delta)))
        return A, d, delta

    @property
    def build_ms(self):
        v = C.c_double()
        check(self.L.armour_get_build_ms(self.h, C.byref(v)))
        return v.value

    def build_info(self):
        out = (C.c_int32 * 4)()
        check(self.L.armour_get_build_info(self.h, out))
        return {"kernel": {0: None, 1: "per_step", 2: "time_vectorised"}[out[0]], "waves": out[1], "sort_entries": out[2], "launches": out[3]}

    def plane_skip(self):
        out = np.zeros(self.B, dtype=np.uint64)
        check(self.L.armour_get_plane_skip(self.h, out.ctypes.data_as(C.POINTER(C.c_uint64))))
        return out

    def prune_margin(self):
        out = np.zeros(self.B)
        check(self.L.armour_get_prune_margin(self.h, _dp(out)))
        return out

    def effective_bytes(self):
        ts = self.table_sizes()
        JT, Q, nT = self.J * self.T, self.J * self.T * self.O, self.n * self.T
        Qs = (Q + 15) // 16 * 16
        dfc = self.B >= 8 or self.B * Q >= 32768
        line = lambda nbytes: (nbytes + 127) // 128 * 128
        total = 0
        for sk in self.plane_skip():
            live = [p for p in range(36) if not (int(sk) >> p) & 1]
            lo, hi = sum(1 for p in live if p < 21), sum(1 for p in live if p >= 21)
            hi_pairs = len({(p - 21) >> 1 for p in live if p >= 21})
            per_row = 32 * lo + 16 * hi_pairs + (0 if dfc else 8 * (lo + hi))
            total += Qs * per_row + (JT * 384 if hi else 0) + (line(24 * self.O) if dfc else 0)
        total += 32 * ts["sum_link"] + 16 * ts["sum_torque"] + self.B * (JT * 52 + nT * 20)
        total += self.B * (line(8 * self.m * (1 + self.n)) + line(8 * self.n))
        return total

    def algorithmic_bytes(self):
        ts = self.table_sizes()
        return (1440 * self.T * self.J * self.O * self.B + 32 * ts["sum_link"] + 16 * ts["sum_torque"]
                + 8 * self.m * (1 + self.n) * self.B)
```

include/armour_hip.h:

```cpp
#ifndef ARMOUR_HIP_H
#define ARMOUR_HIP_H

#include <stdint.h>
#include "armour_types.h"

#ifdef __cplusplus
extern "C" {
#endif

#define ARMOUR_OK 0
#define ARMOUR_EINVAL (-1)
#define ARMOUR_EDEVICE (-2)
#define ARMOUR_ECAPACITY (-3)
#define ARMOUR_ESTATE (-4)

typedef struct ArmourPlanner ArmourPlanner;

typedef struct ArmourLimits {
    int32_t max_batch;
    int32_t max_obstacles;
    int32_t link_monomials;
    int32_t torque_monomials;
    int32_t work_monomials;
    int32_t raw_terms;
} ArmourLimits;

void armour_robot_kinova_gen3_no_gripper(ArmourRobot* robot);
void armour_robot_kinova_gen3_gripper(ArmourRobot* robot);
void armour_robot_fetch(ArmourRobot* robot);
int armour_robot_fetch8(ArmourRobot* robot);
void armour_params_default(ArmourParams* params, int32_t num_time_steps);

int armour_create(const ArmourRobot* robot, const ArmourParams* params, const ArmourLimits* limits,
                  int32_t device, ArmourPlanner** out);
void armour_destroy(ArmourPlanner* h);
const char* armour_last_error(void);
int armour_device_available(void);

int armour_alloc_pinned(uint64_t bytes, void** out);
void armour_free_pinned(void* p);

#define ARMOUR_OPT_P1_BUILD 1
#define ARMOUR_OPT_P1_WORK_MEMORY_MB 2
#define ARMOUR_OPT_P1_KEEP_WORK_MEMORY 3

#define ARMOUR_OPT_P1_STEP_WAVES 101
#define ARMOUR_OPT_P1_STEP_FREE 102
#define ARMOUR_OPT_P1_STEP_SPLIT_FK 103
#define ARMOUR_OPT_P1_STEP_AUX3 104
#define ARMOUR_OPT_P1_MAX_WAVES_PER_CU 105
#define ARMOUR_OPT_P1_TWO_PASS 106
#define ARMOUR_OPT_P1_STEP_TAIL_CROSS 108
#define ARMOUR_OPT_P1_STEP_QUEUE 109
#define ARMOUR_OPT_P1_STEP_PAIRS 107
#define ARMOUR_OPT_P1_STEP_TWO_CU 123
#define ARMOUR_OPT_P1_STEP_LEAN_BACK 124
#define ARMOUR_OPT_P1_TV_MIN_GROUPS 110
#define ARMOUR_OPT_P1_TV_WAVES 111
#define ARMOUR_OPT_P1_TV_FREE 112
#define ARMOUR_OPT_P1_TV_SPLIT_FK 113
#define ARMOUR_OPT_P1_TV_DEDICATED 114
#define ARMOUR_OPT_P1_TV_HELP_SHIFT 115
#define ARMOUR_OPT_P1_TV_HELPERS 116
#define ARMOUR_OPT_P1_TV_HELP_MIN 117
#define ARMOUR_OPT_P1_TV_HELP_N 118
#define ARMOUR_OPT_P1_TV_AUX3 119
#define ARMOUR_OPT_P1_TV_TAIL_CROSS 121
#define ARMOUR_OPT_P1_TV_ROW_WIDTH 122
#define ARMOUR_OPT_P1_FULL_PLANES 120
#define ARMOUR_OPT_P2_EX 130
#define ARMOUR_OPT_STEPS_GRAPH_MIN 131
#define ARMOUR_OPT_CULL_ROWS 133
#define ARMOUR_OPT_PINNED_MODE 132
#define ARMOUR_OPT_SOLVE_SUB_TILES 140
#define ARMOUR_OPT_SOLVE_DEVICE 141
#define ARMOUR_OPT_SOLVE_CUT_TILES 142
#define ARMOUR_OPT_SOLVE_BLOCKS 143
#define ARMOUR_OPT_SOLVE_SUB_BATCH 144
#define ARMOUR_OPT_SOLVE_ROW_CAP 145
#define ARMOUR_OPT_SOLVE_HARD_CAP_S 146
#define ARMOUR_OPT_SOLVE_WAVES_PER_SIMD 147
#define ARMOUR_OPT_SOLVE_CULL 148
#define ARMOUR_OPT_FIRST_TUNING 101
#define ARMOUR_OPT_LAST_TUNING 148
int armour_device_memory(int32_t device, uint64_t* free_bytes, uint64_t* total_bytes);
int armour_abi_max_factors(void);
int armour_set_option(ArmourPlanner* h, int32_t option, double value);
int armour_get_option(ArmourPlanner* h, int32_t option, double* value);

int armour_set_problems(ArmourPlanner* h, int32_t B, int32_t O, const double* q0, const double* qd0,
                        const double* qdd0, const double* q_des, const double* obstacles);

int armour_set_problems_armtd(ArmourPlanner* h, int32_t B, int32_t O, const double* q0, const double* qd0, const double* q_des,
                              const double* jrs, const double* k_range, const double* obstacles);

int armour_get_sizes(const ArmourPlanner* h, int32_t* B, int32_t* n, int32_t* m);

int armour_get_bounds(ArmourPlanner* h, double* x_l, double* x_u, double* g_l, double* g_u);
int armour_eval_f(ArmourPlanner* h, const double* k, double* f);
int armour_eval_grad_f(ArmourPlanner* h, const double* k, double* grad_f);
int armour_eval_g_jac(ArmourPlanner* h, const double* k, double* g, double* jac);
int armour_eval_g_jac_device(ArmourPlanner* h, const double* d_k, double* d_g, double* d_jac, void* stream);
int armour_eval_g_jac_device_steps(ArmourPlanner* h, const double* d_k, int32_t steps, double* d_g, double* d_jac,
                                   void* stream);
int armour_prepare_steps(ArmourPlanner* h, const double* d_k, int32_t steps, double* d_g, double* d_jac);
int armour_eval_g_jac_device_multi(ArmourPlanner* h, const double* d_k, int32_t points, double* d_g, double* d_jac,
                                   void* stream);
int armour_check_feasible(ArmourPlanner* h, const double* g, int32_t* feasible);

typedef struct ArmourViolation {
    double l1_violation, worst;
    int32_t worst_row, n_violated, n_outside_slack, feasible;
} ArmourViolation;
int armour_eval_violations_device(ArmourPlanner* h, const double* d_k, ArmourViolation* d_out, void* stream);
int armour_eval_violations(ArmourPlanner* h, const double* k, ArmourViolation* out);
int armour_get_row_relevance(ArmourPlanner* h, uint8_t* relevant, int32_t* n_relevant_collision_rows, double* ms);
int armour_get_solver_rows(ArmourPlanner* h, uint8_t* solver_rows, int32_t* n_collision_rows, int32_t* n_torque_rows, double* ms);

typedef struct ArmourBatch ArmourBatch;
int armour_batch_partition(int32_t B, int32_t n_slots, int32_t* first );
int armour_batch_create(const ArmourRobot* robot, const ArmourParams* params, const ArmourLimits* limits,
                        const int32_t* devices, int32_t n_devices, ArmourBatch** out);
void armour_batch_destroy(ArmourBatch* bt);
int armour_batch_set_option(ArmourBatch* bt, int32_t option, double value);
int armour_batch_set_problems(ArmourBatch* bt, int32_t B, int32_t O, const double* q0, const double* qd0, const double* qdd0,
                              const double* q_des, const double* obstacles);
int armour_batch_get_sizes(const ArmourBatch* bt, int32_t* B, int32_t* n, int32_t* m, int32_t* n_slots);
int armour_batch_get_bounds(ArmourBatch* bt, double* x_l, double* x_u, double* g_l, double* g_u);
int armour_batch_eval_g_jac(ArmourBatch* bt, const double* k, double* g, double* jac);
int armour_batch_eval_violations(ArmourBatch* bt, const double* k, ArmourViolation* out );
int armour_batch_get_prune_margin(ArmourBatch* bt, double* margin );
int armour_batch_get_build_ms(ArmourBatch* bt, double* max_ms, double* per_slot);
int armour_batch_get_build_info(ArmourBatch* bt, int32_t* info );

int armour_desired_trajectory(int32_t n, const double* q0, const double* qd0, const double* qdd0, const double* k_range,
                              double duration, const double* k, double t, double* q, double* qd, double* qdd);

int armour_robust_controller(const ArmourRobot* robot, double model_uncertainty, const double* Kr, double alpha, double V_max,
                             double r_norm_threshold, int32_t B, const double* q, const double* qd, const double* q_des,
                             const double* qd_des, const double* qdd_des, double* u, double* tau, double* v);
int armour_controller_set_kernel(int32_t which);

#define ARMOUR_TRACK_CTL_ROBUST 0
#define ARMOUR_TRACK_CTL_NOMINAL 1
#define ARMOUR_TRACK_CTL_NONE 2
#define ARMOUR_TRACK_LIMIT_TORQUE 1
#define ARMOUR_TRACK_LIMIT_POSITION 2
#define ARMOUR_TRACK_LIMIT_SPEED 4
typedef struct ArmourTrackOptions {
    int32_t controller;
    int32_t record_every;
    int32_t steps_per_launch;
    int32_t reserved0;
    double Kr[ARMOUR_MAX_FACTORS];
    double alpha, V_max, r_norm_threshold, model_uncertainty;
    double dt, t0, t1, duration;
    double reserved[4];
} ArmourTrackOptions;
typedef struct ArmourTrackResult {
    int32_t status;
    int32_t steps;
    int32_t limit_flags;
    int32_t reserved;
    double t_end, q[ARMOUR_MAX_FACTORS], qd[ARMOUR_MAX_FACTORS];
    double max_pos_error, max_vel_error, max_V, max_robust_input, max_torque_ratio;
    double first_violation_t;
} ArmourTrackResult;
void armour_track_options_default(const ArmourRobot* robot, ArmourTrackOptions* opt);
int armour_track(const ArmourRobot* robot, const ArmourTrackOptions* opt, int32_t B, const double* q0, const double* qd0, const double* qdd0,
                 const double* k, const double* k_range, const double* z0, const double* mass_scale, const double* inertia_scale,
                 ArmourTrackResult* results, double* trace, double* ms);
int armour_track_auto_steps(int32_t controller);

typedef struct ArmourSolveOptions {
    int32_t max_iterations;
    int32_t max_line_search;
    double tolerance;
    double max_wall_time_s;
    double force_host_qp;
    double reserved[3];
} ArmourSolveOptions;
typedef struct ArmourSolveResult {
    double k_opt[ARMOUR_MAX_FACTORS];
    double cost;
    double max_violation;
    int32_t feasible;
    int32_t iterations, evaluations;
    int32_t status;
    double time_ms;
} ArmourSolveResult;
void armour_solve_options_default(ArmourSolveOptions* opt);
int armour_solve(ArmourPlanner* h, const ArmourSolveOptions* opt, ArmourSolveResult* results );
int armour_batch_solve(ArmourBatch* bt, const ArmourSolveOptions* opt, ArmourSolveResult* results );
int armour_debug_qp(int32_t n, const double* Gd, const double* g0, int32_t m, const double* A, const double* lo,
                    const double* hi, double* x, int32_t* feasible);

int armour_debug_qp_box(int32_t n, const double* Gd, const double* g0, int32_t m, const double* A, const double* lo, const double* hi,
                        const double* x_lo, const double* x_hi, int32_t first_try, double* x, int32_t* feasible, int32_t* steps, double* max_mult);

int armour_get_torque_radius(ArmourPlanner* h, double* torque_radius);
int armour_get_link_generators(ArmourPlanner* h, double* gens);
int armour_get_link_centers(ArmourPlanner* h, const double* k, double* centers);

int armour_get_pz(ArmourPlanner* h, int32_t b, int32_t which, int32_t i, int32_t t, double* center,
                  uint64_t* keys, double* coeffs, int32_t capacity);
int armour_get_table_sizes(ArmourPlanner* h, int64_t* out4);
int armour_get_hyperplanes(ArmourPlanner* h, double* A, double* d, double* delta);
int armour_get_plane_skip(ArmourPlanner* h, uint64_t* plane_skip);
int armour_get_prune_margin(ArmourPlanner* h, double* margin );
int armour_get_build_ms(ArmourPlanner* h, double* ms);
#define ARMOUR_P1_KERNEL_PER_STEP 1
#define ARMOUR_P1_KERNEL_TIME_VECTORISED 2
int armour_get_build_info(ArmourPlanner* h, int32_t* out4);
const char* armour_p2_kernel_name(void);

int armour_debug_pz_op(ArmourPlanner* h, int32_t op, int32_t nops, const int32_t* sz, const int32_t* cnt, const uint64_t* const* keys,
                       const double* const* coef, const double* cen, const double* ind, const double* ind2, const double* consts,
                       int32_t r, int32_t out_cap, uint64_t* out_keys, double* out_coef, double* out_misc);

int armour_debug_load_tables(ArmourPlanner* h, int32_t B, int32_t O, const double* q0, const double* qd0,
                             const double* qdd0, const double* q_des, const int32_t* link_count,
                             const double* link_center, const uint64_t* link_keys, const double* link_coeffs,
                             int32_t cap_l, const int32_t* torque_count, const double* torque_center,
                             const uint64_t* torque_keys, const double* torque_coeffs, int32_t cap_t,
                             const double* A, const double* d, const double* delta, const double* torque_radius);

typedef struct ArmourRoadmap ArmourRoadmap;
#define ARMOUR_ROADMAP_MAX_OBSTACLES 256
int armour_roadmap_create(const ArmourRobot* robot, int32_t N, const double* nodes, int32_t E, const int32_t* edges,
                          const uint8_t* continuous, double edge_step, int32_t device, ArmourRoadmap** out);
void armour_roadmap_destroy(ArmourRoadmap* rm);
int armour_roadmap_get_sizes(const ArmourRoadmap* rm, int32_t* N, int32_t* E, int64_t* edge_samples);
int armour_roadmap_check(ArmourRoadmap* rm, int32_t W, int32_t O, const double* obstacles, uint8_t* node_free, uint8_t* edge_free,
                         double* node_clearance, double* ms);
int armour_roadmap_plan(ArmourRoadmap* rm, int32_t w, const double* q_start, const double* q_goal, int32_t connect_k,
                        int32_t max_points, double* path, int32_t* points);

int armour_path_audit(const ArmourRobot* robot, int32_t W, int32_t O, const double* obstacles, int32_t P, const int32_t* world_of_piece,
                      const double* q0, const double* qd0, const double* qdd0, const double* k, const double* k_range, double duration,
                      const double* ta, const double* tb, const double* tube, double step, int32_t* verdict, double* t_hit, double* clearance,
                      double* ms);
int armour_path_audit_host(const ArmourRobot* robot, int32_t W, int32_t O, const double* obstacles, int32_t P, const int32_t* world_of_piece,
                           const double* q0, const double* qd0, const double* qdd0, const double* k, const double* k_range, double duration,
                           const double* ta, const double* tb, const double* tube, double step, int32_t* verdict, double* t_hit,
                           double* clearance);
int armour_path_audit_items(const ArmourRobot* robot, int32_t P, const double* q0, const double* qd0, const double* qdd0, const double* k,
                            const double* k_range, double duration, const double* ta, const double* tb, double step, int64_t* items);

#ifdef __cplusplus
}
#endif
#endif
```

Before: 160,500.

## Evaluate link polynomial slices from registers in a fused P2 collision path

Adds a register-resident path for the exact single-point P2 collision kernel: each thread preloads its link monomial keys and coefficients into registers and evaluates the polynomial slice directly into shared memory. This skips the per-pass term staging array in LDS and the multi-pass term reduction. The LDS budget shrinks accordingly. It is enabled by default for small monomial counts (up to 12), with an option for up to 32. A debug API for padding link monomial counts is added for testing, and the solver path keeps the old kernel. Costs include more register pressure and two new template instantiations.

```diff
diff --git a/armour_amd/_lib.py b/armour_amd/_lib.py
--- a/armour_amd/_lib.py
+++ b/armour_amd/_lib.py
@@ -106,6 +106,7 @@
 OPT_P1_FULL_PLANES = 120
 OPT_P1_TV_ROW_WIDTH = 122
 OPT_P2_EX = 130
+OPT_P2_FUSED_SLICE = 134
 OPT_STEPS_GRAPH_MIN = 131
 OPT_PINNED_MODE = 132
 OPT_CULL_ROWS = 133
@@ -126,7 +127,7 @@
     "armour_eval_g_jac_device", "armour_eval_g_jac_device_steps", "armour_prepare_steps", "armour_eval_g_jac_device_multi", "armour_desired_trajectory", "armour_robust_controller", "armour_check_feasible", "armour_get_torque_radius",
     "armour_get_link_generators", "armour_get_link_centers", "armour_get_pz", "armour_get_table_sizes",
     "armour_solve_options_default", "armour_solve", "armour_debug_qp", "armour_debug_qp_box", "armour_debug_pz_op",
-    "armour_get_hyperplanes", "armour_get_build_ms", "armour_get_build_info", "armour_p2_kernel_name", "armour_debug_load_tables",
+    "armour_get_hyperplanes", "armour_get_build_ms", "armour_get_build_info", "armour_p2_kernel_name", "armour_debug_load_tables", "armour_debug_set_link_count",
     "armour_get_plane_skip", "armour_get_prune_margin", "armour_batch_get_prune_margin", "armour_set_option", "armour_get_option", "armour_controller_set_kernel", "armour_device_memory", "armour_abi_max_factors", "armour_eval_violations_device", "armour_eval_violations", "armour_get_row_relevance", "armour_get_solver_rows",
     "armour_batch_partition", "armour_batch_create", "armour_batch_destroy", "armour_batch_set_option", "armour_batch_set_problems",
     "armour_batch_get_sizes", "armour_batch_get_bounds", "armour_batch_eval_g_jac", "armour_batch_eval_violations", "armour_batch_solve",
@@ -219,6 +220,7 @@
     L.armour_get_build_ms.argtypes = [vp, dp]
     L.armour_get_build_info.argtypes = [vp, ip]
     L.armour_p2_kernel_name.restype = C.c_char_p
+    L.armour_debug_set_link_count.argtypes = [vp, C.c_int32]
     L.armour_debug_load_tables.argtypes = [vp, C.c_int32, C.c_int32, dp, dp, dp, dp, ip, dp, C.POINTER(C.c_uint64), dp,
                                            C.c_int32, ip, dp, C.POINTER(C.c_uint64), dp, C.c_int32, dp, dp, dp, dp]
     L.armour_get_plane_skip.argtypes = [vp, C.POINTER(C.c_uint64)]
diff --git a/armour_amd/csrc/api.hip b/armour_amd/csrc/api.hip
--- a/armour_amd/csrc/api.hip
+++ b/armour_amd/csrc/api.hip
@@ -134,6 +134,7 @@
     tb.tq_keys = h->d_tq_keys; tb.tq_coeff = h->d_tq_coeff;
     tb.planes = h->d_planes; tb.planes_ll = h->d_planes_ll; tb.ll_shared = h->ll_shared;
     tb.ex_allowed = h->tune(ARMOUR_OPT_P2_EX);
+    tb.fuse_slice = h->tune(ARMOUR_OPT_P2_FUSED_SLICE);
     tb.obs_center = (h->d_from_center && (h->B >= 8 || !h->planes_have_d)) ? h->d_obs_center : nullptr;
     tb.plane_skip = h->d_plane_skip; tb.bez = h->d_bez;
     for (int i = 0; i < ARMOUR_MAX_FACTORS; i++) tb.k_range[i] = h->params.k_range[i];
@@ -149,7 +150,7 @@
     {ARMOUR_OPT_P1_TV_MIN_GROUPS, 31, 1, 1e6}, {ARMOUR_OPT_P1_TV_WAVES, 0, 0, 8}, {ARMOUR_OPT_P1_TV_FREE, 1, 0, 1}, {ARMOUR_OPT_P1_TV_SPLIT_FK, -1, -1, 1},
     {ARMOUR_OPT_P1_TV_DEDICATED, 1, 0, 1}, {ARMOUR_OPT_P1_TV_HELP_SHIFT, 0, 0, 3}, {ARMOUR_OPT_P1_TV_HELPERS, 1, 0, 31}, {ARMOUR_OPT_P1_TV_HELP_MIN, 192, 1, 1e6},
     {ARMOUR_OPT_P1_TV_HELP_N, 1, 0, 1}, {ARMOUR_OPT_P1_TV_AUX3, 1, 0, 1}, {ARMOUR_OPT_P1_TV_ROW_WIDTH, 0, 0, 64}, {ARMOUR_OPT_P1_FULL_PLANES, 0, 0, 1},
-    {ARMOUR_OPT_P2_EX, 1, 0, 1}, {ARMOUR_OPT_STEPS_GRAPH_MIN, 2, 0, 1e6}, {ARMOUR_OPT_PINNED_MODE, 0, 0, 2}, {ARMOUR_OPT_CULL_ROWS, 0, 0, 1},
+    {ARMOUR_OPT_P2_EX, 1, 0, 1}, {ARMOUR_OPT_P2_FUSED_SLICE, 1, 0, 2}, {ARMOUR_OPT_STEPS_GRAPH_MIN, 2, 0, 1e6}, {ARMOUR_OPT_PINNED_MODE, 0, 0, 2}, {ARMOUR_OPT_CULL_ROWS, 0, 0, 1},
     {ARMOUR_OPT_SOLVE_SUB_TILES, 48, 1, 1e6}, {ARMOUR_OPT_SOLVE_DEVICE, 1, 0, 2}, {ARMOUR_OPT_SOLVE_CUT_TILES, 156, 1, 1e6}, {ARMOUR_OPT_SOLVE_BLOCKS, 0, 0, 1e6},
     {ARMOUR_OPT_SOLVE_SUB_BATCH, 0, 0, 1e6}, {ARMOUR_OPT_SOLVE_ROW_CAP, 0, 0, 1e7}, {ARMOUR_OPT_SOLVE_HARD_CAP_S, 0, 0, 1e6}, {ARMOUR_OPT_SOLVE_WAVES_PER_SIMD, 0, 0, 2}, {ARMOUR_OPT_SOLVE_CULL, -1, -1, 1},
 };
@@ -450,6 +451,37 @@
     return ARMOUR_OK;
 }
 
+extern "C" int armour_debug_set_link_count(ArmourPlanner* h, int32_t count) {
+    if (!h) { armour_set_error("null handle"); return ARMOUR_EINVAL; }
+    if (!h->ready) { armour_set_error("no problem set: call armour_set_problems first"); return ARMOUR_ESTATE; }
+    const int capL = h->lim.link_monomials;
+    if (count < 0 || count > capL) { armour_set_error("armour_debug_set_link_count: %d outside [0, %d]", count, capL); return ARMOUR_EINVAL; }
+    HIPCHK(hipSetDevice(h->device));
+    HIPCHK(hipStreamSynchronize(h->stream));
+    const size_t nl = (size_t)h->B * h->J * h->T;
+    std::vector<int> lc(nl);
+    std::vector<uint32_t> lk(nl * capL);
+    std::vector<double> lco(nl * capL * 3);
+    HIPCHK(hipMemcpy(lc.data(), h->d_link_count, nl * sizeof(int), hipMemcpyDeviceToHost));
+    HIPCHK(hipMemcpy(lk.data(), h->d_link_keys, lk.size() * sizeof(uint32_t), hipMemcpyDeviceToHost));
+    HIPCHK(hipMemcpy(lco.data(), h->d_link_coeff, lco.size() * sizeof(double), hipMemcpyDeviceToHost));
+    for (size_t i = 0; i < nl; i++) {
+        const int old = lc[i];
+        for (int mo = old; mo < count; mo++) {
+            lk[i * capL + mo] = old > 0 ? lk[i * capL + mo % old] : 0u;
+            for (int e = 0; e < 3; e++) lco[(i * capL + mo) * 3 + e] = old > 0 ? lco[(i * capL + mo % old) * 3 + e] : 0.0;
+        }
+        lc[i] = count;
+    }
+    HIPCHK(hipMemcpy(h->d_link_count, lc.data(), nl * sizeof(int), hipMemcpyHostToDevice));
+    HIPCHK(hipMemcpy(h->d_link_keys, lk.data(), lk.size() * sizeof(uint32_t), hipMemcpyHostToDevice));
+    HIPCHK(hipMemcpy(h->d_link_coeff, lco.data(), lco.size() * sizeof(double), hipMemcpyHostToDevice));
+    drop_step_graphs(h);
+    h->rel_fresh = false; h->rel2_fresh = false;
+    h->stats_fresh = false;
+    return armour_refresh_table_stats(h);
+}
+
 #define NEED_READY(h)                                                                        \
     if (!(h)) { armour_set_error("null handle"); return ARMOUR_EINVAL; }                     \
     if (!(h)->ready) { armour_set_error("no problem set: call armour_set_problems first"); return ARMOUR_ESTATE; }
@@ -780,6 +812,7 @@
         if (ok && option == ARMOUR_OPT_P1_STEP_TWO_CU) { const int lv = (int)value % 10; ok = lv <= 3 && (value < 10.0 || lv >= 1); if (ok) h->p1_two_cu_off = false; }
         if (ok) {
             h->tuning[option - ARMOUR_OPT_FIRST_TUNING] = value;
+            if (option == ARMOUR_OPT_P2_FUSED_SLICE) drop_step_graphs(h);
             h->p1_step_cap_hint = 0; h->p1_tv_shape_hint = 0;
             return ARMOUR_OK;
         }
diff --git a/armour_amd/csrc/common.h b/armour_amd/csrc/common.h
--- a/armour_amd/csrc/common.h
+++ b/armour_amd/csrc/common.h
@@ -76,6 +76,7 @@
     const double* planes_ll;
     int ll_shared;
     int ex_allowed;
+    int fuse_slice;
     int mode;
     const unsigned long long* plane_skip;
     const double* bez;
diff --git a/armour_amd/csrc/p2_eval.hip b/armour_amd/csrc/p2_eval.hip
--- a/armour_amd/csrc/p2_eval.hip
+++ b/armour_amd/csrc/p2_eval.hip
@@ -4,7 +4,7 @@
 
 namespace {
 
-template <bool WANT_G, bool WANT_J, bool MULTI, bool DFC, bool LL, int PPW, bool EX>
+template <bool WANT_G, bool WANT_J, bool MULTI, bool DFC, bool LL, int PPW, bool EX, int FS = 0>
 __global__ __launch_bounds__(P2_BLOCK) __attribute__((amdgpu_waves_per_eu(P2_WPE(DFC, MULTI)))) void armour_p2_eval_kernel(P2Tables tb, const double* __restrict__ k_all,
                                                                   double* __restrict__ g_all, double* __restrict__ jac_all,
                                                                   P2Launch lp) {
@@ -20,7 +20,7 @@
     if ((P2_ABLATE & 2) && role >= lp.nbc && role < lp.nbc + lp.nbt) return;
     if ((P2_ABLATE & 4) && role >= lp.nbc + lp.nbt) return;
 #endif
-    if (role < lp.nbc) collision_block<WANT_G, WANT_J, MULTI, DFC, LL, PPW, EX>(tb, lp, b, role, k0, k_first, g0, jac0, smem_raw);
+    if (role < lp.nbc) collision_block<WANT_G, WANT_J, MULTI, DFC, LL, PPW, EX, FS>(tb, lp, b, role, k0, k_first, g0, jac0, smem_raw);
     else if (role < lp.nbc + lp.nbt) torque_block<WANT_G, WANT_J, MULTI, DFC, LL, PPW, EX>(tb, lp, b, role, k0, k_first, g0, jac0, smem_raw);
     else limit_block<WANT_G, WANT_J, MULTI, DFC, LL, PPW, EX>(tb, lp, b, role, k0, k_first, g0, jac0, smem_raw);
 }
@@ -61,6 +61,10 @@
     return true;
 }
 
+#define P2_FS_SMALL 12
+#define P2_FS_LARGE 32
+#define P2_FS_THRESHOLD 12
+
 int armour_p2_plan(const P2Tables& tb, int max_link, int max_torque, const unsigned long long* h_skip, int steps, long long k_stride,
                    long long g_stride, long long j_stride, P2Launch* lp_out, size_t* smem_out, bool* dfc_out, bool* six_out, bool* exact_out) {
     P2Launch lp;
@@ -78,16 +82,20 @@
     if (lp.strideL * 3 > P2_BLOCK * P2_TASK_ROUNDS) { armour_set_error("link PZ with %d monomials exceeds the P2 kernel's %d", lp.strideL, P2_BLOCK * P2_TASK_ROUNDS / 3); return ARMOUR_ECAPACITY; }
     lp.pair_chunk = std::max(1, std::min(std::min(lp.max_pairs, P2_BLOCK / P2_SL), (P2_BLOCK * P2_TASK_ROUNDS) / (lp.strideL * 3)));
     if (lp.strideT > 32 * P2_TQ_ROUNDS) { armour_set_error("torque PZ with %d monomials exceeds the P2 kernel's %d", lp.strideT, 32 * P2_TQ_ROUNDS); return ARMOUR_ECAPACITY; }
-    const size_t col = ((size_t)lp.max_pairs * P2_SL + (size_t)lp.pair_chunk * lp.strideL * P2_SL + 4 * 64 * 4 + 64 * ARMOUR_MAX_FACTORS) * sizeof(double) + 4 * 64 * sizeof(int);
-    const size_t tq = (size_t)P2_TQ_ROWS * lp.strideT * P2_TQW * sizeof(double);
-    const size_t lim = (size_t)2 * ARMOUR_MAX_FACTORS * 8 * sizeof(double);
-    const size_t smem = 2 * sizeof(KPow) + std::max(std::max(col, tq), lim);
-    if (smem > 64 * 1024) { armour_set_error("P2 kernel needs %zu B of LDS (link/torque monomial counts too large)", smem); return ARMOUR_ECAPACITY; }
     const bool dfc = tb.obs_center != nullptr && tb.ll_shared;
     bool six = h_skip != nullptr;
     for (int b = 0; six && b < tb.B; b++) six = __builtin_popcountll(~h_skip[b] & ((1ull << ARMOUR_NPLANES) - 1ull)) <= 24;
     bool exact = six && tb.ex_allowed && lp.max_pairs <= lp.pair_chunk;
     for (int b = 0; exact && b < tb.B; b++) exact = armour_p2_ex_layout_ok(h_skip[b]);
+    lp.fs_slots = 0;
+    if (exact && !dfc && tb.ll_shared && steps <= 1 && tb.fuse_slice != 0 && lp.strideL <= (tb.fuse_slice == 2 ? P2_FS_LARGE : P2_FS_THRESHOLD))
+        lp.fs_slots = lp.strideL <= P2_FS_SMALL ? P2_FS_SMALL : P2_FS_LARGE;
+    const size_t n_terms = lp.fs_slots > 0 ? 0 : (size_t)lp.pair_chunk * lp.strideL * P2_SL;
+    const size_t col = ((size_t)lp.max_pairs * P2_SL + n_terms + 4 * 64 * 4 + 64 * ARMOUR_MAX_FACTORS) * sizeof(double) + 4 * 64 * sizeof(int);
+    const size_t tq = (size_t)P2_TQ_ROWS * lp.strideT * P2_TQW * sizeof(double);
+    const size_t lim = (size_t)2 * ARMOUR_MAX_FACTORS * 8 * sizeof(double);
+    const size_t smem = 2 * sizeof(KPow) + std::max(std::max(col, tq), lim);
+    if (smem > 64 * 1024) { armour_set_error("P2 kernel needs %zu B of LDS (link/torque monomial counts too large)", smem); return ARMOUR_ECAPACITY; }
     *lp_out = lp; *smem_out = smem; *dfc_out = dfc; *six_out = six; *exact_out = exact;
     return ARMOUR_OK;
 }
@@ -107,6 +115,8 @@
         if (dfc && exact && !(M)) hipLaunchKernelGGL((armour_p2_eval_kernel<G, J, false, true, true, 6, true>), grid, block, smem, stream, tb, d_k, d_g, d_jac, lp);      \
         else if (dfc && six) hipLaunchKernelGGL((armour_p2_eval_kernel<G, J, M, true, true, 6, false>), grid, block, smem, stream, tb, d_k, d_g, d_jac, lp);                \
         else if (dfc) hipLaunchKernelGGL((armour_p2_eval_kernel<G, J, M, true, true, 9, false>), grid, block, smem, stream, tb, d_k, d_g, d_jac, lp);              \
+        else if (tb.ll_shared && exact && !(M) && lp.fs_slots == P2_FS_SMALL) hipLaunchKernelGGL((armour_p2_eval_kernel<G, J, false, false, true, 6, true, P2_FS_SMALL>), grid, block, smem, stream, tb, d_k, d_g, d_jac, lp); \
+        else if (tb.ll_shared && exact && !(M) && lp.fs_slots == P2_FS_LARGE) hipLaunchKernelGGL((armour_p2_eval_kernel<G, J, false, false, true, 6, true, P2_FS_LARGE>), grid, block, smem, stream, tb, d_k, d_g, d_jac, lp); \
         else if (tb.ll_shared && exact && !(M)) hipLaunchKernelGGL((armour_p2_eval_kernel<G, J, false, false, true, 6, true>), grid, block, smem, stream, tb, d_k, d_g, d_jac, lp); \
         else if (tb.ll_shared && six) hipLaunchKernelGGL((armour_p2_eval_kernel<G, J, M, false, true, 6, false>), grid, block, smem, stream, tb, d_k, d_g, d_jac, lp); \
         else if (tb.ll_shared) hipLaunchKernelGGL((armour_p2_eval_kernel<G, J, M, false, true, 9, false>), grid, block, smem, stream, tb, d_k, d_g, d_jac, lp); \
diff --git a/armour_amd/csrc/p2_tiles.h b/armour_amd/csrc/p2_tiles.h
--- a/armour_amd/csrc/p2_tiles.h
+++ b/armour_amd/csrc/p2_tiles.h
@@ -1,5 +1,6 @@
 #pragma once
 #include <algorithm>
+#include <cstddef>
 #include <cstdlib>
 
 #include "bezier.h"
@@ -88,6 +89,22 @@
             o[1 + kk] = g;
         }
     }
+}
+__device__ inline double mono_one(const KPow& kp, uint32_t key, double c, int n, int kk) {
+    static_assert(offsetof(KPow, df) == sizeof(double) * 4 * ARMOUR_MAX_FACTORS, "df follows pw");
+    const double* tab = &kp.pw[0][0];
+    double f[ARMOUR_MAX_FACTORS];
+#pragma unroll
+    for (int j = 0; j < ARMOUR_MAX_FACTORS; j++) {
+        const uint32_t d = (key >> (2 * j)) & 3u;
+        const bool dj = j == kk;
+        const double t = tab[(dj ? 4 * ARMOUR_MAX_FACTORS : 0) + j * 4 + (int)d];
+        f[j] = (j < n) ? t : (dj ? 0.0 : 1.0);
+    }
+    double v = c;
+#pragma unroll
+    for (int j = 0; j < ARMOUR_MAX_FACTORS; j++) v *= f[j];
+    return v;
 }
 __device__ inline double interval_center(double c, double r) {
     const double lo = c - r, hi = c + r;
@@ -109,6 +126,7 @@
     int skip_by_value;
     unsigned long long skip0;
     int steps;
+    int fs_slots;
     long long k_stride, g_stride, j_stride;
     unsigned long long magic_O, magic_pp3;
 };
@@ -176,7 +194,33 @@
     pr.rc_ind = tb.link_indep[idx * 3 + e];
 }
 
-template <bool WANT_G, bool WANT_J, bool MULTI, bool DFC, bool LL, int PPW, bool EX>
+template <int FS>
+struct FusedRegs {
+    uint32_t key[FS > 0 ? FS : 1];
+    double co[FS > 0 ? FS : 1];
+    double cen, ind;
+    int cnt;
+};
+template <int FS>
+__device__ __forceinline__ void load_fused(const P2Tables& tb, int b, int lt_first, int pc, FusedRegs<FS>& fr) {
+    const int tid = threadIdx.x;
+    const int tc = tid < pc * P2_SL ? tid : 0;
+    const int pi = tc / P2_SL, c = tc - pi * P2_SL, e = c % 3;
+    const size_t idx = (size_t)b * tb.J * tb.T + lt_first + pi;
+    fr.cnt = tb.link_count[idx];
+    fr.cen = tb.link_center[idx * 3 + e];
+    fr.ind = tb.link_indep[idx * 3 + e];
+    const uint32_t* kq = tb.link_keys + idx * tb.capL;
+    const double* cq = tb.link_coeff + idx * tb.capL * 3 + e;
+#pragma unroll
+    for (int mo = 0; mo < FS; mo++) {
+        const int moc = min(mo, tb.capL - 1);
+        fr.key[mo] = kq[moc];
+        fr.co[mo] = cq[(size_t)moc * 3];
+    }
+}
+
+template <bool WANT_G, bool WANT_J, bool MULTI, bool DFC, bool LL, int PPW, bool EX, int FS = 0>
 __device__ __forceinline__ void collision_block(const P2Tables& tb, const P2Launch& lp, const int b, const int role, const double* __restrict__ k0,
                                    const double k_first, double* __restrict__ g0_in, double* __restrict__ jac0_in, unsigned char* smem_raw) {
     KPow* kp2 = reinterpret_cast<KPow*>(smem_raw);
@@ -197,8 +241,9 @@
     const unsigned long long cyc0 = __builtin_amdgcn_s_memtime();
 #endif
     double* sx = lds;
+    static_assert(FS == 0 || (EX && !MULTI), "register slicing is built for the one-point EX kernels");
     double* terms = sx + (size_t)lp.max_pairs * P2_SL;
-    double* part = terms + (size_t)lp.pair_chunk * lp.strideL * P2_SL;
+    double* part = terms + (FS > 0 ? 0 : (size_t)lp.pair_chunk * lp.strideL * P2_SL);
     int* pneg = reinterpret_cast<int*>(part + 4 * 64 * 4);
     double* stage = part + 4 * 64 * 4 + 4 * 64 / 2;
 
@@ -224,7 +269,9 @@
     const int npairs = (q_end - 1) / O - lt_first + 1;
     const bool single_pass = npairs <= lp.pair_chunk;
     PassRegs pr;
-    if (EX) load_pass_uncond(tb, lp, b, lt_first, npairs, pr);
+    FusedRegs<FS> fr;
+    if (FS > 0) load_fused<FS>(tb, b, lt_first, npairs, fr);
+    else if (EX) load_pass_uncond(tb, lp, b, lt_first, npairs, pr);
     v2d raw[EX ? 12 : 1];
     bool ll_wave = false;
     if (EX) {
@@ -293,6 +340,27 @@
         fill_kpow(kp, k_cur, n);
         double* g = WANT_G ? g0 + (size_t)s * lp.g_stride : nullptr;
         double* jac = WANT_J ? jac0 + (size_t)s * lp.j_stride : nullptr;
+        if (FS > 0) {
+            lds_barrier();
+            P2_STAMP(2);
+            if (tid < npairs * P2_SL) {
+                const int out = (tid % P2_SL) / 3;
+                if (WANT_J || out == 0) {
+                    double acc = out == 0 ? fr.cen : 0.0;
+#pragma unroll
+                    for (int mo = 0; mo < FS; mo++) {
+                        if (mo < lp.strideL) {
+                            const double t = mono_one(kp, fr.key[mo], fr.co[mo], n, out - 1);
+                            acc = mo < fr.cnt ? acc + t : acc;
+                        }
+                    }
+                    if (out == 0) acc = interval_center(acc, fr.ind);
+                    sx[tid] = acc;
+                }
+            }
+            P2_STAMP(3);
+            lds_barrier();
+        } else
         for (int p0 = 0; p0 < npairs; p0 += lp.pair_chunk) {
             const int pc = min(lp.pair_chunk, npairs - p0);
             if (!EX && (!MULTI || !single_pass)) load_pass(tb, lp, b, lt_first, p0, pc, pr);
diff --git a/armour_amd/csrc/solver_device.hip b/armour_amd/csrc/solver_device.hip
--- a/armour_amd/csrc/solver_device.hip
+++ b/armour_amd/csrc/solver_device.hip
@@ -940,7 +940,9 @@
     P2Launch lp;
     size_t smem = 0;
     bool dfc, six, exact;
-    int rc = armour_p2_plan(tb, max_link, max_torque, h_skip, 1, 0, 0, 0, &lp, &smem, &dfc, &six, &exact);
+    P2Tables tb2 = tb;
+    tb2.fuse_slice = 0;
+    int rc = armour_p2_plan(tb2, max_link, max_torque, h_skip, 1, 0, 0, 0, &lp, &smem, &dfc, &six, &exact);
     if (rc != ARMOUR_OK) return rc;
     plan->lp = lp; plan->smem = smem; plan->six = six;
     plan->n_tiles = n_tiles_override > 0 ? n_tiles_override : lp.nbt + lp.nbc + 1;
diff --git a/armour_amd/planner.py b/armour_amd/planner.py
--- a/armour_amd/planner.py
+++ b/armour_amd/planner.py
@@ -275,6 +275,10 @@
             t["torque_count"].ctypes.data_as(i32), _dp(t["torque_center"]), t["torque_keys"].ctypes.data_as(u64), _dp(t["torque_coeffs"]), t["torque_keys"].shape[-1],
             _dp(t["A"]), _dp(t["d"]), _dp(t["delta"]), _dp(t["torque_radius"])))
         self._after_set(B, O)
+        return self
+
+    def debug_set_link_count(self, count):
+        check(self.L.armour_debug_set_link_count(self.h, int(count)))
         return self
 
     def get_nlp_info(self):
diff --git a/include/armour_hip.h b/include/armour_hip.h
--- a/include/armour_hip.h
+++ b/include/armour_hip.h
@@ -69,6 +69,7 @@
 #define ARMOUR_OPT_P1_TV_ROW_WIDTH 122
 #define ARMOUR_OPT_P1_FULL_PLANES 120
 #define ARMOUR_OPT_P2_EX 130
+#define ARMOUR_OPT_P2_FUSED_SLICE 134
 #define ARMOUR_OPT_STEPS_GRAPH_MIN 131
 #define ARMOUR_OPT_CULL_ROWS 133
 #define ARMOUR_OPT_PINNED_MODE 132
@@ -218,6 +219,8 @@
                        const double* const* coef, const double* cen, const double* ind, const double* ind2, const double* consts,
                        int32_t r, int32_t out_cap, uint64_t* out_keys, double* out_coef, double* out_misc);
 
+int armour_debug_set_link_count(ArmourPlanner* h, int32_t count);
+
 int armour_debug_load_tables(ArmourPlanner* h, int32_t B, int32_t O, const double* q0, const double* qd0,
                              const double* qdd0, const double* q_des, const int32_t* link_count,
                              const double* link_center, const uint64_t* link_keys, const double* link_coeffs,
```

Measured after the change: 133,800. 16.7% lower.
